# hey-yahei/Quantization.MXNet

Measured on AMD Instinct MI355X. Metric: images/sec int8-sim MobileNet1.0 (per-layer W8A8, online input quant), higher is better.
Workload: dtype f32

## Files before the change

### include/fakequant.h

```cpp
#ifndef FAKEQUANT_H_
#define FAKEQUANT_H_

#include <stddef.h>
#include <stdint.h>

#ifdef __cplusplus
extern "C" {
#endif

#define FQ_OK 0
#define FQ_ERR_INVALID 1
#define FQ_ERR_HIP 2

typedef void* fqStream_t;

#define FQ_ACT_SIGNED 1u
#define FQ_ACT_LO_NEG_MAX 2u
#define FQ_ACT_NO_ABS 4u
#define FQ_ACT_NO_EPS 8u

#define FQ_CODES_INT8 0
#define FQ_CODES_UINT8 1
#define FQ_CODES_RANGE 2
#define FQ_CODES_SCALE 3
// ... 47 lines not shown
int fq_fake_quant_online_prestat(const float* x, float* y, int64_t n, int64_t inner, const float* stat, int width,
                                 unsigned flags, float* out_current_max, int32_t* codes, fqStream_t stream);

#define FQ_ACT_NONE 0
#define FQ_ACT_RELU 1
#define FQ_ACT_RELU6 2
#define FQ_STAT_PREZEROED 0x100
int fq_bn_act_stat(const float* x, float* y, int64_t n, int64_t c, int64_t hw, const float* scale,
                   const float* shift, int act, float* stat_out, fqStream_t stream);
int fq_bn_act_maxpool_stat(const float* x, float* y, int64_t n, int64_t c, int64_t h, int64_t w, const float* scale,
                           const float* shift, int act, float* stat_out, fqStream_t stream);

int fq_add_act_stat(const float* a, const float* b, float* y, int64_t n, int64_t inner, int act, float* stat_out,
                    fqStream_t stream);

int fq_bn_act_stat_hist(const float* x, float* y, int64_t n, int64_t c, int64_t hw, const float* scale,
                        const float* shift, int act, float* stat_out, const float* hist_max, int bins, uint64_t* hist,
                        uint32_t* neg_count, fqStream_t stream);
int fq_add_act_stat_hist(const float* a, const float* b, float* y, int64_t n, int64_t inner, int act, float* stat_out,
                         const float* hist_max, int bins, uint64_t* hist, uint32_t* neg_count, fqStream_t stream);

int fq_bn_add_act_stat(const float* x, const float* residual, float* y, int64_t n, int64_t c, int64_t hw, const float* scale,
                       const float* shift, int act, float* stat_out, fqStream_t stream);
int fq_bn_add_act_stat_hist(const float* x, const float* residual, float* y, int64_t n, int64_t c, int64_t hw,
                            const float* scale, const float* shift, int act, float* stat_out, const float* hist_max, int bins,
                            uint64_t* hist, uint32_t* neg_count, fqStream_t stream);

int fq_global_avg_pool_stat(const float* x, float* y, int64_t n, int64_t c, int64_t hw, int flags, float* stat_out,
                            fqStream_t stream);

int fq_gemm_i8_codes(const int8_t* xcodes, const int8_t* wcodes, const int32_t* wsum, int32_t* out, int64_t n,
                     int64_t l, int64_t k_pad, int64_t cout, int zoff, fqStream_t stream);

int fq_eval_counters(const float* logits, const int64_t* labels, int64_t n, int64_t classes, float* counters,
                     fqStream_t stream);

int fq_stem_conv3x3s2(const float* x, const float* w_tap_major, const float* bias, float* y, int64_t n, int64_t cin,
                      int64_t cout, int64_t h, int64_t w, const float* bn_scale, const float* bn_shift, int act,
                      float* stat_out, fqStream_t stream);
int fq_stem_conv3x3s2_c16(const float* x, const float* w_tap_major, const float* bias, void* y16, int64_t n, int64_t cin,
                          int64_t cout, int64_t h, int64_t w, const float* bn_scale, const float* bn_shift, int act,
                          float* stat_out, const float* out_thr, int out_width, unsigned out_flags, fqStream_t stream);
int fq_stem_conv7x7s2(const float* x, const float* w_tap_major, const float* bias, float* y, int64_t n, int64_t cin,
                      int64_t cout, int64_t h, int64_t w, const float* bn_scale, const float* bn_shift, int act,
                      float* stat_out, fqStream_t stream);
int fq_stem_conv7x7s2_pool_supported(int64_t h, int64_t w);
int fq_stem_conv7x7s2_pool(const float* x, const float* w_tap_major, const float* bias, float* y, int64_t n, int64_t cin,
                           int64_t cout, int64_t h, int64_t w, const float* bn_scale, const float* bn_shift, int act,
                           float* stat_out, fqStream_t stream);

int fq_dwconv3x3(const float* x, const float* w, const float* bias, float* y, int64_t n, int64_t c, int64_t h,
                 int64_t wdt, int stride, const float* in_stat, const float* in_thr, int in_width, unsigned in_flags,
                 float* out_current_max, const float* bn_scale, const float* bn_shift, int act, float* stat_out,
                 fqStream_t stream);

int fq_weight_codes(const float* w, int64_t rows, int64_t row_len, int rows_per_scale, int width, int64_t row_pad,
                    int64_t rows_pad, int8_t* codes, float* scales, int32_t* rowsum, void* ws, fqStream_t stream);
#define FQ_PW_FORM(f) ((f) << 12)
size_t fq_pwconv_workspace_bytes(int64_t n, int64_t cin_pad, int64_t hw);
int fq_pwconv_i8(const float* x, const int8_t* wcodes, const float* wscale, const int32_t* wsum, const float* bias,
                 float* y, int64_t n, int64_t cin, int64_t cin_pad, int64_t cout, int64_t hw, const float* in_stat,
                 const float* in_thr, int in_width, unsigned in_flags, float* out_current_max,
                 const float* bn_scale, const float* bn_shift, int act, float* stat_out, void* ws,
                 fqStream_t stream);

size_t fq_dense_i8_eval_workspace_bytes(int64_t n, int64_t cout);
int fq_dense_i8_eval(const float* x, const int8_t* wcodes, const float* wscale, const int32_t* wsum, const float* bias,
                     float* y, int64_t n, int64_t cin, int64_t cin_pad, int64_t cout, const float* in_stat,
                     const float* in_thr, int in_width, unsigned in_flags, float* out_current_max,
                     const int64_t* labels, float* counters, void* eval_ws, void* ws, fqStream_t stream);

int fq_pwconv_i8_strided(const float* x, const int8_t* wcodes, const float* wscale, const int32_t* wsum,
                         const float* bias, float* y, int64_t n, int64_t cin, int64_t cin_pad, int64_t cout, int64_t h,
                         int64_t w, int stride, const float* in_stat, const float* in_thr, int in_width,
                         unsigned in_flags, float* out_current_max, const float* bn_scale, const float* bn_shift,
                         int act, float* stat_out, const float* residual, void* ws, fqStream_t stream);

int fq_pwconv_i8_sub2_supported(int64_t cin, int64_t cout);
int fq_pwconv_i8_sub2(const float* x, const int8_t* wcodes, const float* wscale, const int32_t* wsum, const float* bias,
                      float* y, int64_t n, int64_t cin, int64_t cin_pad, int64_t cout, int64_t h, int64_t w,
                      const float* in_stat, const float* in_thr, int in_width, unsigned in_flags, float* out_current_max,
                      const float* bn_scale, const float* bn_shift, int act, float* stat_out, const float* residual, void* ws,
                      fqStream_t stream);

int fq_pwconv_i8_shortcut_supported(int64_t cin, int64_t cin2, int64_t cout);
int fq_pwconv_i8_shortcut(const float* x, const int8_t* wcodes, const float* wscale, const int32_t* wsum, const float* bias,
                          float* y, int64_t n, int64_t cin, int64_t cin_pad, int64_t cout, int64_t hw, const float* in_stat,
                          const float* in_thr, int in_width, unsigned in_flags, float* out_current_max, const float* bn_scale,
                          const float* bn_shift, int act, float* stat_out, const float* x2, const int8_t* wcodes2,
                          const float* wscale2, const int32_t* wsum2, int64_t cin2, int64_t cin2_pad, const float* in_stat2,
                          const float* in_thr2, int in_width2, unsigned in_flags2, float* out_current_max2,
                          const float* bn_scale2, const float* bn_shift2, fqStream_t stream);

int fq_pwconv_i8_shortcut_c16(const void* x, const int8_t* wcodes, const float* wscale, const int32_t* wsum, const float* bias,
                              float* y, void* y16, int64_t n, int64_t cin, int64_t cin_pad, int64_t cout, int64_t hw,
                              const float* in_stat, const float* in_thr, int in_width, unsigned in_flags, float* out_current_max,
                              const float* bn_scale, const float* bn_shift, int act, float* stat_out, const void* x2, int x2_is_c16,
                              const int8_t* wcodes2, const float* wscale2, const int32_t* wsum2, int64_t cin2, int64_t cin2_pad,
                              const float* in_stat2, const float* in_thr2, int in_width2, unsigned in_flags2,
                              float* out_current_max2, const float* bn_scale2, const float* bn_shift2, const float* out_thr,
                              int out_width, unsigned out_flags, fqStream_t stream);

int fq_pwconv_i8_gap_supported(int64_t n, int64_t cin, int64_t cout, int64_t hw, int has_residual);
int fq_pwconv_i8_gap(const float* x, const int8_t* wcodes, const float* wscale, const int32_t* wsum, const float* bias,
                     float* y, int64_t n, int64_t cin, int64_t cin_pad, int64_t cout, int64_t hw, const float* in_stat,
                     const float* in_thr, int in_width, unsigned in_flags, float* out_current_max, const float* bn_scale,
                     const float* bn_shift, int act, float* stat_out, const float* residual, void* ws, fqStream_t stream);

int fq_pwconv_i8_stat_supported(int64_t n, int64_t cin, int64_t cout, int64_t hw);
int fq_pwconv_i8_stat(const float* x, const int8_t* wcodes, const float* wscale, const int32_t* wsum, const float* bias,
                      int64_t n, int64_t cin, int64_t cin_pad, int64_t cout_pad, int64_t cout, int64_t hw,
                      const float* in_stat, const float* in_thr, int in_width, unsigned in_flags, float* out_current_max,
                      const float* bn_scale, const float* bn_shift, int act, float* stat_out, void* x_codes_out,
                      fqStream_t stream);
int fq_pwdw_fused_supported(int64_t n, int64_t cin, int64_t cout, int64_t h, int64_t w, int stride);
int fq_debug_fast_quotient(const float* c, int64_t n, const float* d, float* out, int* took_fast_path, fqStream_t stream);
int fq_pwdw_fused(const float* x, const int8_t* wcodes, const float* wscale, const int32_t* wsum, const float* pw_bias,
                  int64_t n, int64_t cin, int64_t cin_pad, int64_t cout_pad, int64_t cout, int64_t h, int64_t w,
                  const float* in_stat, const float* in_thr, int in_width, unsigned in_flags, const float* pw_bn_scale,
                  const float* pw_bn_shift, int pw_act, const float* mid_stat, const float* mid_thr, int mid_width,
                  unsigned mid_flags, float* mid_current_max, const float* dw_w, const float* dw_bias, int dw_stride,
                  const float* dw_bn_scale, const float* dw_bn_shift, int dw_act, float* y, float* stat_out,
                  const void* x_codes, fqStream_t stream);

int fq_pwconv_i8_c16(const void* x, int x_is_c16, const int8_t* wcodes, const float* wscale, const int32_t* wsum,
                     const float* bias, void* y, int64_t n, int64_t cin, int64_t cin_pad, int64_t cout, int64_t h, int64_t w,
                     int stride, const float* in_stat, const float* in_thr, int in_width, unsigned in_flags,
                     float* out_current_max, const float* bn_scale, const float* bn_shift, int act, float* stat_out,
                     const float* residual, const float* out_thr, int out_width, unsigned out_flags, void* ws,
                     fqStream_t stream);

int fq_pwconv_i8_c16_dual(const void* x, const int8_t* wcodes, const float* wscale, const int32_t* wsum, const float* bias,
                          float* y, void* y16, int64_t n, int64_t cin, int64_t cin_pad, int64_t cout, int64_t h, int64_t w,
                          const float* in_stat, const float* in_thr, int in_width, unsigned in_flags, float* out_current_max,
                          const float* bn_scale, const float* bn_shift, int act, float* stat_out, const float* residual,
                          const float* out_thr, int out_width, unsigned out_flags, void* ws, fqStream_t stream);
int fq_pwconv_i8_c16_dual_sub2(const void* x, const int8_t* wcodes, const float* wscale, const int32_t* wsum, const float* bias,
                               float* y, void* y16, int64_t n, int64_t cin, int64_t cin_pad, int64_t cout, int64_t h, int64_t w,
                               const float* in_stat, const float* in_thr, int in_width, unsigned in_flags,
                               float* out_current_max, const float* bn_scale, const float* bn_shift, int act, float* stat_out,
                               const float* residual, const float* out_thr, int out_width, unsigned out_flags, void* ws,
                               fqStream_t stream);

int fq_conv3x3_i8(const float* x, const int8_t* wcodes, const float* wscale, const int32_t* wsum, const float* bias,
                  float* y, int64_t n, int64_t cin, int64_t cout, int64_t h, int64_t w, const float* in_stat,
                  const float* in_thr, int in_width, unsigned in_flags, float* out_current_max, const float* bn_scale,
                  const float* bn_shift, int act, float* stat_out, fqStream_t stream);

int fq_conv3x3_i8_c16(const void* x, int x_is_c16, const int8_t* wcodes, const float* wscale, const int32_t* wsum,
                      const float* bias, void* y, int64_t n, int64_t cin, int64_t cout, int64_t h, int64_t w,
                      const float* in_stat, const float* in_thr, int in_width, unsigned in_flags, float* out_current_max,
                      const float* bn_scale, const float* bn_shift, int act, float* stat_out, const float* out_thr,
                      int out_width, unsigned out_flags, fqStream_t stream);

int fq_dwconv3x3_c16(const void* x, const float* w, const float* bias, void* y, int64_t n, int64_t c, int64_t h, int64_t wdt,
                     int stride, const float* in_stat, const float* in_thr, int in_width, unsigned in_flags,
                     float* out_current_max, const float* bn_scale, const float* bn_shift, int act, float* stat_out,
                     const float* out_thr, int out_width, unsigned out_flags, fqStream_t stream);

int fq_weight_slices(const float* w, int64_t rows, int64_t row_len, int64_t row_pad, int64_t rows_pad, int8_t* codes,
                     float* pscale, int32_t* rowsum, void* ws, fqStream_t stream);
int fq_conv3x3_i8_sliced(const float* x, const int8_t* wslices, const float* pscale, const int32_t* wsum, const float* bias,
                         float* y, int64_t n, int64_t cin, int64_t cout, int64_t h, int64_t w, const float* in_stat,
                         const float* in_thr, int in_width, unsigned in_flags, float* out_current_max,
                         const float* bn_scale, const float* bn_shift, int act, float* stat_out, fqStream_t stream);

int fq_ste_forward(const float* x, float* y, int64_t rows, int64_t row_len, const float* scales, int has_clip,
// ... 54 lines not shown
```

### quantization/mxnet_amd/_lib.py

```python
import ctypes
import os

__all__ = ["LIB", "check_call", "load", "library_path", "FakeQuantError", "EXPORTS"]

_HERE = os.path.dirname(os.path.abspath(__file__))
_LIB_PATH = os.environ.get("FQ_LIB_PATH") or os.path.join(_HERE, "csrc", "libfakequant.so")

c_f32p = ctypes.POINTER(ctypes.c_float)
c_i32p = ctypes.POINTER(ctypes.c_int32)
c_u32p = ctypes.POINTER(ctypes.c_uint32)
c_u64p = ctypes.POINTER(ctypes.c_uint64)
_vp, _i64, _int, _uint, _f32 = ctypes.c_void_p, ctypes.c_int64, ctypes.c_int, ctypes.c_uint, ctypes.c_float

EXPORTS = {
    "fq_last_error": (ctypes.c_char_p, []),
    "fq_version": (_int, []),
    "fq_build_id": (ctypes.c_char_p, []),
    "fq_device_info": (_int, [ctypes.c_char_p, _int, ctypes.POINTER(_int), ctypes.POINTER(_int)]),
    "fq_profile_enable": (_int, [_int]),
    "fq_profile_reset": (_int, []),
    "fq_profile_read": (_int, [_int, ctypes.POINTER(ctypes.c_double), ctypes.POINTER(_i64),
                               ctypes.POINTER(ctypes.c_double)]),
    "fq_profile_read_moved": (_int, [_int, ctypes.POINTER(ctypes.c_double)]),
    "fq_profile_calibrate": (_int, [_vp, _int, ctypes.POINTER(ctypes.c_double), ctypes.POINTER(ctypes.c_double), _vp]),
    "fq_profile_launch_overhead": (_int, [_vp, _int, ctypes.c_double, ctypes.POINTER(ctypes.c_double),
                                          ctypes.POINTER(ctypes.c_double), _vp]),
    "fq_act_workspace_bytes": (ctypes.c_size_t, [_i64]),
    "fq_absmax_per_sample": (_int, [_vp, _i64, _i64, _uint, _vp, _vp]),
    "fq_batch_mean": (_int, [_vp, _i64, _vp, _vp]),
    "fq_batch_mean_gathered": (_int, [_vp, _int, _i64, _vp, _vp]),
    "fq_stat_rows_sum": (_int, [_vp, _i64, _i64, _i64, _vp, _vp]),
    "fq_mean_from_sums": (_int, [_vp, _i64, _vp, _vp]),
    "fq_batch_mean_rows": (_int, [_vp, _i64, _i64, _i64, _vp, _vp]),
    "fq_fake_quant_online": (_int, [_vp, _vp, _i64, _i64, _int, _uint, _vp, _vp, _vp, _vp]),
    "fq_fake_quant_online_prestat": (_int, [_vp, _vp, _i64, _i64, _vp, _int, _uint, _vp, _vp, _vp]),
    "fq_bn_act_stat": (_int, [_vp, _vp, _i64, _i64, _i64, _vp, _vp, _int, _vp, _vp]),
    "fq_bn_act_maxpool_stat": (_int, [_vp, _vp, _i64, _i64, _i64, _i64, _vp, _vp, _int, _vp, _vp]),
    "fq_add_act_stat": (_int, [_vp, _vp, _vp, _i64, _i64, _int, _vp, _vp]),
    "fq_bn_act_stat_hist": (_int, [_vp, _vp, _i64, _i64, _i64, _vp, _vp, _int, _vp, _vp, _int, _vp, _vp, _vp]),
    "fq_add_act_stat_hist": (_int, [_vp, _vp, _vp, _i64, _i64, _int, _vp, _vp, _int, _vp, _vp, _vp]),
    "fq_bn_add_act_stat": (_int, [_vp, _vp, _vp, _i64, _i64, _i64, _vp, _vp, _int, _vp, _vp]),
    "fq_bn_add_act_stat_hist": (_int, [_vp, _vp, _vp, _i64, _i64, _i64, _vp, _vp, _int, _vp, _vp, _int, _vp, _vp, _vp]),
    "fq_global_avg_pool_stat": (_int, [_vp, _vp, _i64, _i64, _i64, _int, _vp, _vp]),
    "fq_gemm_i8_codes": (_int, [_vp, _vp, _vp, _vp, _i64, _i64, _i64, _i64, _int, _vp]),
    "fq_eval_counters": (_int, [_vp, _vp, _i64, _i64, _vp, _vp]),
    "fq_stem_conv3x3s2": (_int, [_vp, _vp, _vp, _vp, _i64, _i64, _i64, _i64, _i64, _vp, _vp, _int, _vp, _vp]),
    "fq_stem_conv7x7s2": (_int, [_vp, _vp, _vp, _vp, _i64, _i64, _i64, _i64, _i64, _vp, _vp, _int, _vp, _vp]),
    "fq_stem_conv7x7s2_pool": (_int, [_vp, _vp, _vp, _vp, _i64, _i64, _i64, _i64, _i64, _vp, _vp, _int, _vp, _vp]),
    "fq_stem_conv7x7s2_pool_supported": (_int, [_i64, _i64]),
    "fq_stem_conv3x3s2_c16": (_int, [_vp, _vp, _vp, _vp, _i64, _i64, _i64, _i64, _i64, _vp, _vp, _int, _vp, _vp, _int, _uint, _vp]),
    "fq_dwconv3x3": (_int, [_vp, _vp, _vp, _vp, _i64, _i64, _i64, _i64, _int, _vp, _vp, _int, _uint, _vp, _vp, _vp, _int,
                            _vp, _vp]),
    "fq_dwconv3x3_c16": (_int, [_vp, _vp, _vp, _vp, _i64, _i64, _i64, _i64, _int, _vp, _vp, _int, _uint, _vp, _vp, _vp, _int,
                                _vp, _vp, _int, _uint, _vp]),
    "fq_weight_codes": (_int, [_vp, _i64, _i64, _int, _int, _i64, _i64, _vp, _vp, _vp, _vp, _vp]),
    "fq_pwconv_workspace_bytes": (ctypes.c_size_t, [_i64, _i64, _i64]),
    "fq_pwconv_i8": (_int, [_vp, _vp, _vp, _vp, _vp, _vp, _i64, _i64, _i64, _i64, _i64, _vp, _vp, _int, _uint, _vp, _vp,
                            _vp, _int, _vp, _vp, _vp]),
    "fq_pwconv_i8_stat_supported": (_int, [_i64, _i64, _i64, _i64]),
    "fq_pwconv_i8_stat": (_int, [_vp, _vp, _vp, _vp, _vp, _i64, _i64, _i64, _i64, _i64, _i64, _vp, _vp, _int, _uint, _vp, _vp,
                                 _vp, _int, _vp, _vp, _vp]),
    "fq_pwdw_fused_supported": (_int, [_i64, _i64, _i64, _i64, _i64, _int]),
    "fq_pwdw_fused": (_int, [_vp, _vp, _vp, _vp, _vp, _i64, _i64, _i64, _i64, _i64, _i64, _i64, _vp, _vp, _int, _uint, _vp,
                             _vp, _int, _vp, _vp, _int, _uint, _vp, _vp, _vp, _int, _vp, _vp, _int, _vp, _vp, _vp, _vp]),
    "fq_debug_fast_quotient": (_int, [_vp, _i64, _vp, _vp, _vp, _vp]),
    "fq_dense_i8_eval_workspace_bytes": (ctypes.c_size_t, [_i64, _i64]),
    "fq_dense_i8_eval": (_int, [_vp, _vp, _vp, _vp, _vp, _vp, _i64, _i64, _i64, _i64, _vp, _vp, _int, _uint, _vp, _vp, _vp,
                                _vp, _vp, _vp]),
    "fq_pwconv_i8_strided": (_int, [_vp, _vp, _vp, _vp, _vp, _vp, _i64, _i64, _i64, _i64, _i64, _i64, _int, _vp, _vp, _int,
                                    _uint, _vp, _vp, _vp, _int, _vp, _vp, _vp, _vp]),
    "fq_pwconv_i8_shortcut_supported": (_int, [_i64, _i64, _i64]),
    "fq_pwconv_i8_shortcut": (_int, [_vp, _vp, _vp, _vp, _vp, _vp, _i64, _i64, _i64, _i64, _i64, _vp, _vp, _int, _uint, _vp, _vp,
                                     _vp, _int, _vp, _vp, _vp, _vp, _vp, _i64, _i64, _vp, _vp, _int, _uint, _vp, _vp, _vp, _vp]),
    "fq_pwconv_i8_shortcut_c16": (_int, [_vp, _vp, _vp, _vp, _vp, _vp, _vp, _i64, _i64, _i64, _i64, _i64, _vp, _vp, _int, _uint, _vp,
                                         _vp, _vp, _int, _vp, _vp, _int, _vp, _vp, _vp, _i64, _i64, _vp, _vp, _int, _uint, _vp, _vp,
                                         _vp, _vp, _int, _uint, _vp]),
    "fq_pwconv_i8_gap_supported": (_int, [_i64, _i64, _i64, _i64, _int]),
    "fq_pwconv_i8_gap": (_int, [_vp, _vp, _vp, _vp, _vp, _vp, _i64, _i64, _i64, _i64, _i64, _vp, _vp, _int, _uint, _vp, _vp, _vp,
                                _int, _vp, _vp, _vp, _vp]),
    "fq_pwconv_i8_sub2_supported": (_int, [_i64, _i64]),
    "fq_pwconv_i8_sub2": (_int, [_vp, _vp, _vp, _vp, _vp, _vp, _i64, _i64, _i64, _i64, _i64, _i64, _vp, _vp, _int,
                                 _uint, _vp, _vp, _vp, _int, _vp, _vp, _vp, _vp]),
    "fq_pwconv_i8_c16": (_int, [_vp, _int, _vp, _vp, _vp, _vp, _vp, _i64, _i64, _i64, _i64, _i64, _i64, _int, _vp, _vp, _int,
                                _uint, _vp, _vp, _vp, _int, _vp, _vp, _vp, _int, _uint, _vp, _vp]),
    "fq_pwconv_i8_c16_dual": (_int, [_vp, _vp, _vp, _vp, _vp, _vp, _vp, _i64, _i64, _i64, _i64, _i64, _i64, _vp, _vp, _int,
                                     _uint, _vp, _vp, _vp, _int, _vp, _vp, _vp, _int, _uint, _vp, _vp]),
    "fq_pwconv_i8_c16_dual_sub2": (_int, [_vp, _vp, _vp, _vp, _vp, _vp, _vp, _i64, _i64, _i64, _i64, _i64, _i64, _vp, _vp, _int,
                                          _uint, _vp, _vp, _vp, _int, _vp, _vp, _vp, _int, _uint, _vp, _vp]),
    "fq_conv3x3_i8": (_int, [_vp, _vp, _vp, _vp, _vp, _vp, _i64, _i64, _i64, _i64, _i64, _vp, _vp, _int, _uint, _vp, _vp,
                             _vp, _int, _vp, _vp]),
    "fq_conv3x3_i8_c16": (_int, [_vp, _int, _vp, _vp, _vp, _vp, _vp, _i64, _i64, _i64, _i64, _i64, _vp, _vp, _int, _uint, _vp,
                                 _vp, _vp, _int, _vp, _vp, _int, _uint, _vp]),
    "fq_conv3x3_i8_sliced": (_int, [_vp, _vp, _vp, _vp, _vp, _vp, _i64, _i64, _i64, _i64, _i64, _vp, _vp, _int, _uint, _vp,
                                    _vp, _vp, _int, _vp, _vp]),
    "fq_weight_slices": (_int, [_vp, _i64, _i64, _i64, _i64, _vp, _vp, _vp, _vp, _vp]),
    "fq_fake_quant_offline": (_int, [_vp, _vp, _i64, _i64, _vp, _int, _uint, _vp, _vp, _vp, _vp]),
    "fq_ste_forward": (_int, [_vp, _vp, _i64, _i64, _vp, _int, _f32, _f32, _f32, _vp]),
    "fq_weight_workspace_bytes": (ctypes.c_size_t, [_i64]),
    "fq_weight_fake_quant": (_int, [_vp, _vp, _i64, _i64, _int, _vp, _vp, _vp]),
    "fq_wino_weight_fake_quant": (_int, [_vp, _vp, _i64, _i64, _int, c_f32p, c_f32p, c_f32p, _int, _vp, _vp, _vp]),
    "fq_comm_unique_id": (_int, [_vp]),
    "fq_comm_init": (_int, [_int, _int, _vp]),
    "fq_comm_world": (_int, []),
    "fq_allreduce_f32": (_int, [_vp, _i64, _int, _vp]),
    "fq_allreduce_f64": (_int, [_vp, _i64, _int, _vp]),
    "fq_allreduce_i64": (_int, [_vp, _i64, _int, _vp]),
    "fq_comm_destroy": (_int, []),
    "fq_ema_update": (_int, [_vp, _vp, _i64, ctypes.c_double, _vp]),
    "fq_global_max": (_int, [_vp, _i64, _vp, _vp]),
    "fq_histogram_accumulate": (_int, [_vp, _i64, _vp, _int, _vp, _vp, _vp]),
    "fq_hist_to_float": (_int, [_vp, _vp, _i64, _vp]),
    "fq_kl_workspace_bytes": (ctypes.c_size_t, [_i64, _int]),
    "fq_kl_search": (_int, [_vp, _i64, _int, _int, _int, _vp, _vp, _vp]),
    "fq_quantize_codes": (_int, [_vp, _vp, _i64, _int, _vp, _vp, _vp]),
# ... 56 lines not shown
```

### quantization/mxnet_amd/csrc/fq_common.h

```cpp
#ifndef FQ_COMMON_H_
#define FQ_COMMON_H_

#include <hip/hip_runtime.h>
#include <type_traits>

#include <algorithm>
#include <cmath>
#include <cstdarg>
#include <cstdint>
#include <cstdio>
#include <cstdlib>
#include <cstring>
#include <mutex>
#include <vector>

#include "fakequant.h"

namespace fqi {

int fail(int code, const char* fmt, ...);
int num_cu();
int max_lds_bytes();
int env_int(const char* name, int dflt);
int stream_policy(int kernel_id, int64_t numel);
// ... 492 lines not shown
    f.sh = k - 32;
  }
  return f;
}

template <bool NT>
__device__ __forceinline__ f4 ld4(const f4* p) {
  if (NT) return __builtin_nontemporal_load(p);
  return *p;
}
template <bool NT>
__device__ __forceinline__ void st4(f4* p, f4 v) {
  if (NT)
    __builtin_nontemporal_store(v, p);
  else
    *p = v;
}
__device__ __forceinline__ f4 fq_code4(f4 v, const QParams& q) {
  f4 k;
  k.x = fq_code(v.x, q);
  k.y = fq_code(v.y, q);
  k.z = fq_code(v.z, q);
  k.w = fq_code(v.w, q);
  return k;
}

template <bool USE_ABS>
__device__ __forceinline__ float stat4(f4 v) {
  return fmaxf(fmaxf(stat_of<USE_ABS>(v.x), stat_of<USE_ABS>(v.y)), fmaxf(stat_of<USE_ABS>(v.z), stat_of<USE_ABS>(v.w)));
}

struct ChunkRange {
  int64_t begin, end;
};
__device__ __forceinline__ ChunkRange block_range(int64_t total_chunks) {
  const int64_t per = (total_chunks + gridDim.x - 1) / gridDim.x;
  ChunkRange r;
  r.begin = (int64_t)blockIdx.x * per;
  r.end = r.begin + per < total_chunks ? r.begin + per : total_chunks;
  return r;
}

__device__ __forceinline__ float act_rt(float v, int act) {
  if (act == FQ_ACT_RELU) v = fmaxf(v, 0.0f);
  if (act == FQ_ACT_RELU6) v = fminf(fmaxf(v, 0.0f), 6.0f);
  return v;
}

__device__ __forceinline__ float lane_prev(float v) {
  return __builtin_bit_cast(float, __builtin_amdgcn_update_dpp(0, __builtin_bit_cast(int, v), 0x138, 0xF, 0xF, false));
}
__device__ __forceinline__ float lane_next(float v) {
  return __builtin_bit_cast(float, __builtin_amdgcn_update_dpp(0, __builtin_bit_cast(int, v), 0x130, 0xF, 0xF, false));
}

constexpr int kEpiRuntime = 0, kEpiBnRelu = 1, kEpiBnRelu6 = 2;
constexpr int kActBiasMul = 0x10;
template <int EPI, bool ACT = true>
__device__ __forceinline__ float dw_finish(float acc, bool has_bias, float bch, bool has_bn, float bsc, float bsh, int act) {
  if (EPI == kEpiRuntime) {
    if (has_bias) acc = (act & kActBiasMul) ? acc * bch : acc + bch;
    if (has_bn) {
      acc = acc * bsc;
      acc = acc + bsh;
    }
    return act_rt(acc, act & 15);
  }
  acc = acc * bsc;
  acc = acc + bsh;
  if (!ACT) return acc;
  acc = fmaxf(acc, 0.0f);
  return EPI == kEpiBnRelu6 ? fminf(acc, 6.0f) : acc;
}

#ifdef FQ_PW_TRACE
__device__ unsigned long long* g_pw_trace = nullptr;
__device__ int g_pw_dbg = 0;
#define PW_STAMP(i)                                                                       \
  do {                                                                                    \
    if (threadIdx.x == 0 && g_pw_trace != nullptr) g_pw_trace[(size_t)blockIdx.x * 8 + (i)] = wall_clock64(); \
  } while (0)
#else
#define PW_STAMP(i) do { } while (0)
#endif

template <bool WANT_MIN, bool USE_ABS>
__global__ __launch_bounds__(kBlock) void minmax_kernel(const float* __restrict__ x, int64_t numel, int vec_ok,
                                                        float* __restrict__ out_min, float* __restrict__ out_max) {
  __shared__ float red[4];
  float mx = USE_ABS ? 0.0f : -INFINITY, mn = INFINITY;
  auto take = [&](float v) {
    mx = fmaxf(mx, stat_of<USE_ABS>(v));
    if (WANT_MIN) mn = fminf(mn, v);
  };
  const int64_t chunks = (numel + kChunk - 1) / kChunk;
  const ChunkRange rg = block_range(chunks);
  for (int64_t c = rg.begin; c < rg.end; ++c) {
    const int64_t base = c * (int64_t)kChunk;
    const int64_t rem = numel - base;
    if (vec_ok && rem >= kChunk) {
      const f4* p = reinterpret_cast<const f4*>(x + base);
      f4 v[kUnroll];
#pragma unroll
      for (int u = 0; u < kUnroll; ++u) v[u] = p[threadIdx.x + u * kBlock];
#pragma unroll
      for (int u = 0; u < kUnroll; ++u) {
// ... 22 lines not shown
```

### quantization/mxnet_amd/csrc/fq_dwconv.hip

```cpp
#include "fq_common.h"

namespace {

typedef float f2 __attribute__((ext_vector_type(2)));
__device__ __forceinline__ f2 splat2(float v) { return (f2){v, v}; }

__device__ __forceinline__ float dw_taps(float w00, float w01, float w02, float w10, float w11, float w12, float w20,
                                         float w21, float w22, float a0, float a1, float a2, float b0, float b1, float b2,
                                         float c0, float c1, float c2) {
  float acc = 0.0f;
  acc = fmaf(w00, a0, acc);
  acc = fmaf(w01, a1, acc);
  acc = fmaf(w02, a2, acc);
  acc = fmaf(w10, b0, acc);
  acc = fmaf(w11, b1, acc);
  acc = fmaf(w12, b2, acc);
  acc = fmaf(w20, c0, acc);
  acc = fmaf(w21, c1, acc);
  acc = fmaf(w22, c2, acc);
  return acc;
}
__device__ __forceinline__ f2 dw_taps2(float w00, float w01, float w02, float w10, float w11, float w12, float w20, float w21,
                                       float w22, f2 a0, f2 a1, f2 a2, f2 b0, f2 b1, f2 b2, f2 c0, f2 c1, f2 c2) {
  f2 acc = {0.f, 0.f};
  acc = __builtin_elementwise_fma(splat2(w00), a0, acc);
  acc = __builtin_elementwise_fma(splat2(w01), a1, acc);
  acc = __builtin_elementwise_fma(splat2(w02), a2, acc);
  acc = __builtin_elementwise_fma(splat2(w10), b0, acc);
  acc = __builtin_elementwise_fma(splat2(w11), b1, acc);
  acc = __builtin_elementwise_fma(splat2(w12), b2, acc);
  acc = __builtin_elementwise_fma(splat2(w20), c0, acc);
  acc = __builtin_elementwise_fma(splat2(w21), c1, acc);
  acc = __builtin_elementwise_fma(splat2(w22), c2, acc);
  return acc;
}

template <bool ONLINE>
__device__ __forceinline__ QParams dw_qparams(const float* in_stat, int n, const float* in_thr,
                                              float levels, int lo_neg_max, float eps, float* cur_max_out) {
  const float max_ = input_threshold(in_stat, n, ONLINE ? nullptr : in_thr, cur_max_out, blockIdx.x == 0);
  return make_qparams_rt(max_, levels, lo_neg_max, eps, in_thr);
}
template <bool ONLINE>
__device__ __forceinline__ QParams dw_qparams_finish(const ThresholdReq& treq, const float* in_stat, int n,
                                                     const float* in_thr, float levels, int lo_neg_max, float eps,
                                                     float* cur_max_out) {
  const float max_ = threshold_finish(treq, in_stat, n, ONLINE ? nullptr : in_thr, cur_max_out, blockIdx.x == 0);
  return make_qparams_rt(max_, levels, lo_neg_max, eps, in_thr);
}

struct DwBlkRange {
  unsigned begin, end;
  unsigned n_samples;
  unsigned s_base;
};
__device__ __forceinline__ DwBlkRange dw_block_range(unsigned nblk, unsigned tsegs, unsigned segs_per_block, unsigned nsegx,
                                                     unsigned C) {
  DwBlkRange r;
  r.begin = (unsigned)((uint64_t)nblk * blockIdx.x / gridDim.x);
  r.end = (unsigned)((uint64_t)nblk * (blockIdx.x + 1) / gridDim.x);
  r.n_samples = tsegs / nsegx / C;
  const unsigned seg0 = r.begin * segs_per_block;
  r.s_base = (seg0 < tsegs ? seg0 : tsegs - 1) / nsegx / C;
  return r;
}

constexpr int kStatSlots = 16;
template <class SampleT>
__device__ __forceinline__ void dw_stat_update(unsigned* k_stat, unsigned s_base, SampleT sample, bool is_out, float m,
                                               int lane, float* stat_out) {
  const unsigned s0 = (unsigned)__builtin_amdgcn_readfirstlane((int)sample);
  const bool wave_uniform = __all(!is_out || (unsigned)sample == s0);
  if (wave_uniform) {
    const float wm = wave_max_nonneg(is_out ? m : 0.0f);
// ... 705 lines not shown
          for (int r = 0; r < H; ++r) {
            float c0 = 0.f, c1 = 0.f, c2 = 0.f;
            if (r + 1 < H) {
              c1 = lp[(r + 1) * W];
              c0 = left_of(c1, first);
              c2 = right_of(c1, last);
            }
            lp[r * W] = window(a0, a1, a2, b0, b1, b2, c0, c1, c2);
            a0 = b0; a1 = b1; a2 = b2;
            b0 = c0; b1 = c1; b2 = c2;
          }
        } else {
          const float* lp = my_tile + j * IN + pos * 2;
          float* op = my_out + j * OUT + pos;
          float a0 = 0.f, a1 = 0.f, a2 = 0.f;
#pragma unroll
          for (int r = 0; r < HO; ++r) {
            const f2 vb = *reinterpret_cast<const f2*>(lp + (2 * r) * W);
            const float b0 = left_of(vb.y, first);
            float c0 = 0.f, c1 = 0.f, c2 = 0.f;
            if (2 * r + 1 < H) {
              const f2 vc = *reinterpret_cast<const f2*>(lp + (2 * r + 1) * W);
              c1 = vc.x;
              c2 = vc.y;
              c0 = left_of(vc.y, first);
            }
            op[r * WO] = window(a0, a1, a2, b0, vb.x, vb.y, c0, c1, c2);
            a0 = c0; a1 = c1; a2 = c2;
          }
        }
      }
    }
    FQ_DWF_PHASE();
    {
      f4 ov[NLO];
#pragma unroll
      for (int i = 0; i < NLO; ++i) ov[i] = DOWN ? otile[wave][lane + 64 * i] : tile[wave][lane + 64 * i];
#pragma unroll
      for (int i = 0; i < NLO; ++i)
        buf_st_v4f_unguarded(ry, (lane + 64u * i) < lim_out ? lane * 16u : kOob, base * (OUT * 4u) + 1024u * i, ov[i]);
      hold_store_data(ov);
    }
    if (has_stat) {
      const unsigned sample = fast_div(base + (is_out ? j : 0u), g.by_c);
      dw_stat_update(k_stat, s_base, sample, is_out, m, (int)lane, stat_out);
    }
    __builtin_amdgcn_wave_barrier();
  }
  PW_STAMP(3);
  if (has_stat) dw_stat_flush(k_stat, s_base, n_samples, stat_out);
  PW_STAMP(5);
}

template <int S, bool QUANT, bool ONLINE, bool NT, int EPI>
__global__ __launch_bounds__(kBlock) void dwconv3x3_cols4_kernel(
    const float* __restrict__ x, const float* __restrict__ wgt, const float* __restrict__ bias,
    float* __restrict__ y, DwColGeom g, int64_t total_segs, const float* __restrict__ in_stat, int n,
    const float* __restrict__ in_thr, float levels, int lo_neg_max, float eps, float* __restrict__ cur_max_out,
    const float* __restrict__ bn_scale, const float* __restrict__ bn_shift, int act, float* __restrict__ stat_out) {
  constexpr int D = (S == 1) ? 4 : 2;
  __shared__ unsigned k_stat[kStatSlots];
  if (threadIdx.x < kStatSlots) k_stat[threadIdx.x] = 0u;
  QParams q = {};
  if (QUANT) q = dw_qparams<ONLINE>(in_stat, n, in_thr, levels, lo_neg_max, eps, cur_max_out);
  const int lane = threadIdx.x & 63, wave = threadIdx.x >> 6;
  const int seg_in_wave = lane / g.SEG;
  const int pos = lane - seg_in_wave * g.SEG;
  const bool lane_used = seg_in_wave < g.segs;
  const int64_t segs_per_block = (int64_t)g.segs * (kBlock / 64);
  const int64_t nblk = (total_segs + segs_per_block - 1) / segs_per_block;
  const bool has_bn = bn_scale != nullptr, has_stat = stat_out != nullptr;
  const int plane_in = g.H * g.W, plane_out = g.Ho * g.Wo;
  const int last_row = g.H - 1;
  const unsigned tsegs = (unsigned)total_segs, nsegx = (unsigned)g.nsegx, C_u = (unsigned)g.C;
  const DwBlkRange rg = dw_block_range((unsigned)nblk, tsegs, (unsigned)segs_per_block, nsegx, C_u);
  __syncthreads();
  for (unsigned blk = rg.begin; blk < rg.end; ++blk) {
    const unsigned seg = blk * (unsigned)segs_per_block + (unsigned)wave * (unsigned)g.segs + (unsigned)seg_in_wave;
    const bool seg_ok = lane_used && seg < tsegs;
    const unsigned plane = seg_ok ? seg / nsegx : 0u;
    const int sx = seg_ok ? (int)(seg - plane * nsegx) : 0;
    const unsigned sample_u = plane / C_u;
    const int ch = (int)(plane - sample_u * C_u);
    const int sample = (int)sample_u;
    const int ic0 = (sx * g.sw + pos - 1) * 4;
    const bool ld_ok = seg_ok && ic0 >= 0 && ic0 < g.W;
    const int oc = S == 1 ? ic0 : ic0 / 2;
    const bool is_out = seg_ok && pos >= 1 && pos <= g.sw && oc < g.Wo;
    const f4* xs = reinterpret_cast<const f4*>(ld_ok ? x + plane * (int64_t)plane_in + ic0 : x);
    float* yp = y + plane * (int64_t)plane_out + oc;
    const int rowq = g.W / 4;
    const float* wk = wgt + ch * 9;
    const float w00 = wk[0], w01 = wk[1], w02 = wk[2], w10 = wk[3], w11 = wk[4], w12 = wk[5], w20 = wk[6],
                w21 = wk[7], w22 = wk[8];
    const float bch = bias != nullptr ? bias[ch] : 0.0f;
    const float bsc = has_bn ? bn_scale[ch] : 1.0f, bsh = has_bn ? bn_shift[ch] : 0.0f;
    float m = 0.0f;
    auto ldrow = [&](int row) -> f4 {
      const int rc = row < last_row ? row : last_row;
      return keep4(ld4<NT>(xs + (int64_t)rc * rowq), ld_ok && row <= last_row);
    };
    auto quant4 = [&](f4 v) -> f4 { return QUANT ? fq_code4(v, q) * q.scale : v; };
    auto finish = [&](float acc) -> float { return dw_finish<EPI>(acc, bias != nullptr, bch, has_bn, bsc, bsh, act); };

    if (S == 1) {
      float a[6] = {0.f, 0.f, 0.f, 0.f, 0.f, 0.f}, b[6];
      f4 raw[D];
#pragma unroll
      for (int k = 0; k < D; ++k) raw[k] = ldrow(1 + k);
      {
        const f4 v = quant4(ldrow(0));
        b[0] = lane_prev(v.w);
        b[1] = v.x; b[2] = v.y; b[3] = v.z; b[4] = v.w;
        b[5] = lane_next(v.x);
      }
      auto emit = [&](int r, f4 craw) {
        const f4 v = quant4(craw);
        float c[6];
        c[0] = lane_prev(v.w);
        c[1] = v.x; c[2] = v.y; c[3] = v.z; c[4] = v.w;
        c[5] = lane_next(v.x);
        float o[4];
#pragma unroll
        for (int k = 0; k < 4; ++k) {
          o[k] = finish(dw_taps(w00, w01, w02, w10, w11, w12, w20, w21, w22, a[k], a[k + 1], a[k + 2], b[k], b[k + 1],
                                b[k + 2], c[k], c[k + 1], c[k + 2]));
        }
        const float mm = fmaxf(fmaxf(fabsf(o[0]), fabsf(o[1])), fmaxf(fabsf(o[2]), fabsf(o[3])));
        m = fmaxf(m, keep(mm, is_out));
        if (is_out) {
          if (g.nts) __builtin_nontemporal_store((f4){o[0], o[1], o[2], o[3]}, reinterpret_cast<f4*>(yp + (int64_t)r * g.Wo));
          else *reinterpret_cast<f4*>(yp + (int64_t)r * g.Wo) = (f4){o[0], o[1], o[2], o[3]};
        }
#pragma unroll
        for (int k = 0; k < 6; ++k) {
          a[k] = b[k];
          b[k] = c[k];
        }
      };
      int r0 = 0;
      for (; r0 + D <= g.Ho; r0 += D) {
        f4 nxt[D];
#pragma unroll
        for (int k = 0; k < D; ++k) nxt[k] = ldrow(r0 + k + 1 + D);
#pragma unroll
        for (int k = 0; k < D; ++k) emit(r0 + k, raw[k]);
#pragma unroll
        for (int k = 0; k < D; ++k) raw[k] = nxt[k];
      }
#pragma unroll
      for (int k = 0; k < D; ++k)
        if (r0 + k < g.Ho) emit(r0 + k, raw[k]);
    } else {
      float a[5] = {0.f, 0.f, 0.f, 0.f, 0.f};
      f4 rb[D], rc[D];
#pragma unroll
      for (int k = 0; k < D; ++k) {
        rb[k] = ldrow(2 * k);
        rc[k] = ldrow(2 * k + 1);
      }
      auto emit2 = [&](int r, f4 braw, f4 craw) {
        const f4 vb = quant4(braw), vc = quant4(craw);
        const float b[5] = {lane_prev(vb.w), vb.x, vb.y, vb.z, vb.w};
        const float c[5] = {lane_prev(vc.w), vc.x, vc.y, vc.z, vc.w};
        float o[2];
#pragma unroll
        for (int k = 0; k < 2; ++k) {
          o[k] = finish(dw_taps(w00, w01, w02, w10, w11, w12, w20, w21, w22, a[2 * k], a[2 * k + 1], a[2 * k + 2], b[2 * k],
                                b[2 * k + 1], b[2 * k + 2], c[2 * k], c[2 * k + 1], c[2 * k + 2]));
        }
        m = fmaxf(m, keep(fmaxf(fabsf(o[0]), fabsf(o[1])), is_out));
        if (is_out) {
          typedef float f2v __attribute__((ext_vector_type(2)));
          if (g.nts) __builtin_nontemporal_store((f2v){o[0], o[1]}, reinterpret_cast<f2v*>(yp + (int64_t)r * g.Wo));
          else *reinterpret_cast<float2*>(yp + (int64_t)r * g.Wo) = make_float2(o[0], o[1]);
        }
#pragma unroll
        for (int k = 0; k < 5; ++k) a[k] = c[k];
      };
      int r0 = 0;
      for (; r0 + D <= g.Ho; r0 += D) {
        f4 nb[D], nc[D];
#pragma unroll
        for (int k = 0; k < D; ++k) {
          nb[k] = ldrow(2 * (r0 + k + D));
          nc[k] = ldrow(2 * (r0 + k + D) + 1);
        }
#pragma unroll
        for (int k = 0; k < D; ++k) emit2(r0 + k, rb[k], rc[k]);
#pragma unroll
        for (int k = 0; k < D; ++k) {
          rb[k] = nb[k];
          rc[k] = nc[k];
        }
      }
#pragma unroll
      for (int k = 0; k < D; ++k)
        if (r0 + k < g.Ho) emit2(r0 + k, rb[k], rc[k]);
    }
    if (has_stat) dw_stat_update(k_stat, rg.s_base, sample, is_out, m, lane, stat_out);
  }
  if (has_stat) dw_stat_flush(k_stat, rg.s_base, rg.n_samples, stat_out);
}

}

constexpr unsigned kFlagRangeRecord = 0x100u;
constexpr unsigned kFlagBiasMultiplies = 0x200u;

namespace {

struct DwCall {
  const float *x, *w, *bias;
  float* y;
  int64_t n, c, h, wdt;
  int stride;
  const float *in_stat, *in_thr;
  float* out_current_max;
  const float *bn_scale, *bn_shift;
  int act;
  float* stat_out;
  hipStream_t st;
  bool quant, online, prezeroed;
  int epi;
  float levels, eps;
  int lo_neg;
  int64_t ho, wo;
};

template <class KernelFor, class... Geom>
int dw_launch(const DwCall& d, int grid, size_t lds, KernelFor kernel_for, Geom... geom) {
  using std::integral_constant;
  if (d.stat_out && !d.prezeroed) FQ_HIP(hipMemsetAsync(d.stat_out, 0, d.n * sizeof(float), d.st));
  ProfScope prof(FQ_KERNEL_DWCONV, 4.0 * ((double)d.n * d.c * d.h * d.wdt + (double)d.n * d.c * d.ho * d.wo), d.st);
  auto launch = [&](auto kernel) {
    hipLaunchKernelGGL(kernel, dim3(grid), dim3(kBlock), lds, d.st, d.x, d.w, d.bias, d.y, geom..., d.in_stat, (int)d.n,
                       d.in_thr, d.levels, d.lo_neg, d.eps, d.out_current_max, d.bn_scale, d.bn_shift, d.act, d.stat_out);
  };
  auto with_epi = [&](auto quant_c, auto online_c) {
    if (d.epi == kEpiBnRelu) launch(kernel_for(quant_c, online_c, integral_constant<int, kEpiBnRelu>{}));
    else if (d.epi == kEpiBnRelu6) launch(kernel_for(quant_c, online_c, integral_constant<int, kEpiBnRelu6>{}));
    else launch(kernel_for(quant_c, online_c, integral_constant<int, kEpiRuntime>{}));
  };
  if (!d.quant) with_epi(std::false_type{}, std::false_type{});
  else if (d.online) with_epi(std::true_type{}, std::true_type{});
  else with_epi(std::true_type{}, std::false_type{});
  FQ_LAUNCH_CHECK();
  return FQ_OK;
}
template <int V>
using dw_int = std::integral_constant<int, V>;

int64_t dw_blocks(int64_t total_segs, int segs) {
  const int64_t per_block = (int64_t)segs * (kBlock / 64);
  return (total_segs + per_block - 1) / per_block;
}
int dw_grid(int64_t nblk, int wg_per_cu) {
  const int64_t cap = (int64_t)num_cu() * wg_per_cu;
  return (int)(nblk < cap ? nblk : cap);
}

DwColGeom dw_col_geom(const DwCall& d, int units, int halo) {
  DwColGeom cg = {};
  cg.C = (int)d.c;
  cg.H = (int)d.h;
  cg.W = (int)d.wdt;
  cg.Ho = (int)d.ho;
  cg.Wo = (int)d.wo;
  const int max_sw = 64 - halo;
  cg.nsegx = (units + max_sw - 1) / max_sw;
  cg.sw = (units + cg.nsegx - 1) / cg.nsegx;
  cg.SEG = cg.sw + halo;
  cg.segs = 64 / cg.SEG;
  return cg;
}

int dw_flat_kind(const DwCall& d) {
  return (d.h == 14 && d.wdt == 14) ? (d.stride == 1 ? 0 : 1)
         : (d.h == 7 && d.wdt == 7 && d.stride == 1) ? 2
         : (d.h == 28 && d.wdt == 28) ? (d.stride == 1 ? 3 : 4) : -1;
}
int dw_flat_planes(int kind) { return kind == 0 ? 9 : kind >= 3 ? 4 : 8; }
bool dw_flat_applies(const DwCall& d, int form) {
  static const int flat_on = env_int("FQ_DW_FLAT", 31) & 31;
  const int kind = dw_flat_kind(d);
  const bool whole = kind == 0 || kind >= 3 || (d.n * d.c) % dw_flat_planes(kind) == 0;
  return kind >= 0 && (form == 5 || (form == 0 && ((flat_on >> kind) & 1))) && whole && aligned16(d.x) && aligned16(d.y) &&
         d.n * d.c * d.h * d.wdt * 4 < (1ll << 31);
}
// ... 1 lines not shown
  const int kind = dw_flat_kind(d);
  DwFlatGeom fg;
  fg.C = (int)d.c;
  fg.planes = (unsigned)(d.n * d.c);
  fg.by_c = fast_div_for((unsigned)d.c);
  const int64_t nblk = dw_blocks(d.n * d.c, dw_flat_planes(kind));
  static const int fl_tune = env_int("FQ_DW_FLAT_WG_PER_CU", 0);
  const int grid = dw_grid(nblk, fl_tune > 0 ? fl_tune : 3);
  fg.per = (unsigned)(nblk / grid);
  fg.rem = (unsigned)(nblk % grid);
  auto go = [&](auto s, auto hw) {
    return dw_launch(d, grid, 0, [](auto q, auto o, auto e) {
      return dwconv3x3_flat_kernel<decltype(s)::value, q(), o(), decltype(hw)::value, decltype(hw)::value, e()>;
    }, fg);
  };
  return kind == 0 ? go(dw_int<1>{}, dw_int<14>{}) : kind == 1 ? go(dw_int<2>{}, dw_int<14>{})
         : kind == 2 ? go(dw_int<1>{}, dw_int<7>{}) : kind == 4 ? go(dw_int<2>{}, dw_int<28>{})
                     : go(dw_int<1>{}, dw_int<28>{});
}

bool dw_planes_two_cols(const DwCall& d) {
  static const int planes_cpl = env_int("FQ_DW_PLANES_CPL", 2);
  const bool al8 = ((((uintptr_t)d.x) | ((uintptr_t)d.y)) & 7) == 0;
  return d.wdt % 2 == 0 && al8 && (d.stride == 2 || planes_cpl == 2);
}
bool dw_planes_applies(const DwCall& d, int form) {
  static const int planes_on = env_int("FQ_DW_PLANES", 1);
  const bool can_planes = (d.h == 14 || d.h == 7) && d.wdt <= 64 && (d.stride == 1 || (dw_planes_two_cols(d) && d.h == 14)) &&
                          d.n * d.c * d.h * d.wdt * 4 < (1ll << 31);
  return (form == 4 || (form == 0 && planes_on)) && can_planes;
}
int dw_run_planes(const DwCall& d) {
  const bool two_cols = dw_planes_two_cols(d);
  DwColGeom cg = dw_col_geom(d, (int)(d.stride == 2 ? d.wo : (two_cols ? d.wdt / 2 : d.wdt)), 0);
  cg.sw = cg.Wo;
  const int64_t total_segs = d.n * d.c;
  static const int pl_wg_per_cu = env_int("FQ_DW_PLANES_WG_PER_CU", 5);
  const int grid = dw_grid(dw_blocks(total_segs, cg.segs), pl_wg_per_cu);
  auto go = [&](auto s, auto h, auto cpl) {
    return dw_launch(d, grid, 0, [](auto q, auto o, auto e) {
      return dwconv3x3_planes_kernel<decltype(s)::value, q(), o(), decltype(h)::value, decltype(cpl)::value, e()>;
    }, cg, total_segs);
  };
  if (d.stride == 2) return go(dw_int<2>{}, dw_int<14>{}, dw_int<2>{});
  if (d.h == 14) return two_cols ? go(dw_int<1>{}, dw_int<14>{}, dw_int<2>{}) : go(dw_int<1>{}, dw_int<14>{}, dw_int<1>{});
  return two_cols ? go(dw_int<1>{}, dw_int<7>{}, dw_int<2>{}) : go(dw_int<1>{}, dw_int<7>{}, dw_int<1>{});
}

int dw_cols_grid(int64_t total_segs, const DwColGeom& cg) {
  static const int dw_wg_per_cu = env_int("FQ_DW_WG_PER_CU", 6);
  return dw_grid(dw_blocks(total_segs, cg.segs), dw_wg_per_cu);
}
bool dw_cols4_applies(const DwCall& d, int form) {
  const bool can4 = (d.wdt % 4 == 0) && aligned16(d.x) && aligned16(d.y) && ((d.h * d.wdt) % 4 == 0) &&
                    (d.stride == 1 || ((d.wdt / 2) % 2 == 0));
  return (form == 3 || form == 0) && can4;
}
int dw_run_cols4(const DwCall& d) {
  DwColGeom cg = dw_col_geom(d, (int)(d.wdt / 4), d.stride == 1 ? 2 : 1);
  const int64_t total_segs = d.n * d.c * cg.nsegx;
  FQ_REQUIRE(total_segs < (1ll << 31) - 1024, "fq_dwconv3x3: tensor too large for 32-bit segment indices");
  const int grid = dw_cols_grid(total_segs, cg);
  static const int dw_nt_mb = env_int("FQ_DW_NT_MB", 200);
  const bool nt = 4.0 * (double)d.n * d.c * d.h * d.wdt > 1e6 * dw_nt_mb;
  static const int dw_nts_mb = env_int("FQ_DW_NTS_MB", 1 << 30);
  cg.nts = 4.0 * (double)d.n * d.c * cg.Ho * cg.Wo >= 1e6 * dw_nts_mb ? 1 : 0;
  auto go = [&](auto s, auto nt_c) {
    return dw_launch(d, grid, 0, [](auto q, auto o, auto e) {
      return dwconv3x3_cols4_kernel<decltype(s)::value, q(), o(), decltype(nt_c)::value, e()>;
    }, cg, total_segs);
  };
  if (d.stride == 1) return nt ? go(dw_int<1>{}, std::true_type{}) : go(dw_int<1>{}, std::false_type{});
  return nt ? go(dw_int<2>{}, std::true_type{}) : go(dw_int<2>{}, std::false_type{});
}
bool dw_cols_applies(const DwCall& d, int form) {
  return form == 2 || ((form == 0 || form == 3) && d.wdt >= 14);
}
int dw_run_cols(const DwCall& d) {
  const DwColGeom cg = dw_col_geom(d, (int)d.wo, d.stride == 1 ? 2 : 1);
  const int64_t total_segs = d.n * d.c * cg.nsegx;
  FQ_REQUIRE(total_segs < (1ll << 31) - 1024, "fq_dwconv3x3: tensor too large for 32-bit segment indices");
  const int grid = dw_cols_grid(total_segs, cg);
  auto go = [&](auto s) {
    return dw_launch(d, grid, 0, [](auto q, auto o, auto e) {
      return dwconv3x3_cols_kernel<decltype(s)::value, q(), o(), e()>;
    }, cg, total_segs);
  };
  return d.stride == 1 ? go(dw_int<1>{}) : go(dw_int<2>{});
}

int dw_run_tiles(const DwCall& d) {
  const int stride = d.stride;
  DwGeom g;
  g.C = (int)d.c;
  g.H = (int)d.h;
  g.W = (int)d.wdt;
  g.Ho = (int)d.ho;
  g.Wo = (int)d.wo;
  g.WS = g.W + 2;
  if ((g.WS & 1) == 0) g.WS += 1;
  const int lds_budget = 8192;
  const int plane_in = g.H * g.W;
  if (plane_in <= 4096 && (g.H + 2) * g.WS <= lds_budget) {
    g.TR = g.Ho;
    g.strips = 1;
    g.IR = g.H + 2;
    g.P = 1;
    for (int p = (int)(d.c < 64 ? d.c : 64); p >= 1; --p)
      if (d.c % p == 0 && p * g.IR * g.WS <= lds_budget) {
        g.P = p;
        break;
      }
  } else {
    g.P = 1;
    int tr = (lds_budget / g.WS - 2) / stride;
    FQ_REQUIRE(tr >= 1, "fq_dwconv3x3: rows of %d floats do not fit the LDS tile", g.W);
    g.strips = (g.Ho + tr - 1) / tr;
    g.TR = (g.Ho + g.strips - 1) / g.strips;
    g.IR = g.TR * stride + 2;
  }
  {
    const int per_seg = g.P * g.Wo;
    int nseg = (2 * kBlock + per_seg - 1) / per_seg;
    if (nseg < 1) nseg = 1;
    if (nseg > g.TR) nseg = g.TR;
    g.RS = (g.TR + nseg - 1) / nseg;
    g.nseg = (g.TR + g.RS - 1) / g.RS;
  }
  const bool base_ok = aligned16(d.x);
  if (g.P > 1 || g.strips == 1)
    g.vec_in = base_ok && (((int64_t)g.P * plane_in) % 4 == 0) && (plane_in % 4 == 0 || g.P % 4 == 0);
  else
    g.vec_in = base_ok && (g.W % 4 == 0) && (plane_in % 4 == 0);
  const int64_t tiles = (d.n * d.c / g.P) * g.strips;
  const size_t lds = (size_t)((g.P * g.IR * g.WS + 3) / 4 * 4 + 16) * sizeof(float);
  auto go = [&](auto s) {
    return dw_launch(d, grid_for(tiles), lds, [](auto q, auto o, auto) {
      return dwconv3x3_kernel<decltype(s)::value, q(), o()>;
    }, g, tiles);
  };
  return stride == 1 ? go(dw_int<1>{}) : go(dw_int<2>{});
}

}

static int dwconv3x3_impl(const float* x, const float* w, const float* bias, float* y, int64_t n, int64_t c, int64_t h,
                          int64_t wdt, int stride, const float* in_stat, const float* in_thr, int in_width, unsigned in_flags,
                          float* out_current_max, const float* bn_scale, const float* bn_shift, int act, float* stat_out,
                          fqStream_t stream) {
  FQ_REQUIRE(x && w && y, "fq_dwconv3x3: null pointer");
  FQ_REQUIRE(n > 0 && c > 0 && h > 0 && wdt > 0 && n * c < (1ll << 31) && h * wdt < (1ll << 28),
             "fq_dwconv3x3: bad shape (n=%lld c=%lld h=%lld w=%lld)", (long long)n, (long long)c, (long long)h,
             (long long)wdt);
  FQ_REQUIRE(stride == 1 || stride == 2, "fq_dwconv3x3: stride must be 1 or 2, got %d", stride);
  FQ_REQUIRE((bn_scale == nullptr) == (bn_shift == nullptr), "fq_dwconv3x3: bn_scale and bn_shift go together");
  const bool prezeroed = (act & FQ_STAT_PREZEROED) != 0;
  act &= ~FQ_STAT_PREZEROED;
  FQ_REQUIRE(act >= FQ_ACT_NONE && act <= FQ_ACT_RELU6, "fq_dwconv3x3: unknown activation %d", act);
  const bool quant = in_stat != nullptr || in_thr != nullptr;
  if (quant) FQ_REQUIRE(in_width >= 2 && in_width <= 16, "fq_dwconv3x3: width %d out of range", in_width);
  if (in_flags & kFlagBiasMultiplies) act |= kActBiasMul;
  static const int epi_on = env_int("FQ_DW_EPI", 1);

  DwCall d = {};
  d.x = x; d.w = w; d.bias = bias; d.y = y;
  d.n = n, d.c = c, d.h = h, d.wdt = wdt, d.stride = stride;
  d.in_stat = in_stat, d.in_thr = in_thr, d.out_current_max = out_current_max;
  d.bn_scale = bn_scale, d.bn_shift = bn_shift, d.act = act, d.stat_out = stat_out;
  d.st = (hipStream_t)stream;
  d.quant = quant, d.online = quant && in_thr == nullptr, d.prezeroed = prezeroed;
  d.epi = (epi_on && bn_scale != nullptr && bias == nullptr)
              ? (act == FQ_ACT_RELU ? kEpiBnRelu : act == FQ_ACT_RELU6 ? kEpiBnRelu6 : kEpiRuntime)
              : kEpiRuntime;
  d.levels = act_levels(in_width, in_flags);
  d.lo_neg = (in_flags & kFlagRangeRecord) ? kRangeMode : ((in_flags & FQ_ACT_LO_NEG_MAX) ? 1 : 0);
  d.eps = (in_flags & FQ_ACT_NO_EPS) ? 0.0f : kEps;
  d.ho = (h - 1) / stride + 1, d.wo = (wdt - 1) / stride + 1;

  static const int form = env_int("FQ_DW_FORM", 0);
  if (dw_flat_applies(d, form)) return dw_run_flat(d);
  if (dw_planes_applies(d, form)) return dw_run_planes(d);
  if (dw_cols4_applies(d, form)) return dw_run_cols4(d);
  if (dw_cols_applies(d, form)) return dw_run_cols(d);
  return dw_run_tiles(d);
}

namespace fqi {
int dw_range_call(const float* x, const float* wcodes_f32, float* y, int64_t n, int64_t c, int64_t h, int64_t wdt, int stride,
                  const float* rec, const float* svec, const float* bn_scale, const float* bn_shift, int act,
                  float* stat_out, hipStream_t st) {
  return dwconv3x3_impl(x, wcodes_f32, svec, y, n, c, h, wdt, stride, nullptr, rec, 8, kFlagRangeRecord | kFlagBiasMultiplies,
                        nullptr, bn_scale, bn_shift, act, stat_out, (fqStream_t)st);
}
}

extern "C" {

int fq_dwconv3x3(const float* x, const float* w, const float* bias, float* y, int64_t n, int64_t c, int64_t h,
                 int64_t wdt, int stride, const float* in_stat, const float* in_thr, int in_width, unsigned in_flags,
                 float* out_current_max, const float* bn_scale, const float* bn_shift, int act, float* stat_out,
                 fqStream_t stream) {
  FQ_REQUIRE(!(in_flags & ~(FQ_ACT_SIGNED | FQ_ACT_LO_NEG_MAX | FQ_ACT_NO_ABS | FQ_ACT_NO_EPS)), "fq_dwconv3x3: unknown flags");
  return dwconv3x3_impl(x, w, bias, y, n, c, h, wdt, stride, in_stat, in_thr, in_width, in_flags, out_current_max, bn_scale,
                        bn_shift, act, stat_out, stream);
}

}
```

### quantization/mxnet_amd/csrc/fq_pw.h

```cpp
#ifndef FQ_PW_H_
#define FQ_PW_H_

#include "fq_common.h"

namespace fqi {

struct PwCall {
  const float* x;
  const int8_t* wcodes;
  const float* wscale;
  const int32_t* wsum;
  const float* bias;
  float* y;
  int64_t n, cin, cin_pad, cout, hw;
  int stride;
  int64_t h_in, w_in, w_out;
  const float* in_stat;
  const float* in_thr;
  float levels;
  int lo_neg, zoff;
  float* out_current_max;
  const float* bn_scale;
  const float* bn_shift;
  int act;
  float* stat_out;
  const float* residual;
  bool prezeroed;
  void* ws;
  hipStream_t st;
  int form;
  bool in_c16 = false;
  const float* out_thr = nullptr;
  float out_levels = 0.0f;
  int out_lo_neg = 0, out_zoff = 0;
  void* y16 = nullptr;
  const float* dual_thr = nullptr;
  bool sub = false;
  bool gap = false;
  const long long* eval_labels = nullptr;
  float* eval_counters = nullptr;
  void* eval_ws = nullptr;
  void* x_codes_out = nullptr;
};

bool pw_stat_shape_ok(int64_t n, int64_t cin, int64_t cout, int64_t hw);
int pw_stat_launch(const PwCall& c);
bool pw_short_shape_ok(int64_t cin, int64_t cin2, int64_t cout);
int pw_short_launch(const PwCall& a, const PwCall& b);
int pw_try_stream(const PwCall& c, bool* taken);
bool pw_stream_shape_ok(const PwCall& c);
bool pw_stream_thin_takes(const PwCall& c);
int pw_try_split(const PwCall& c, bool* taken);
int pw_split16_launch(const PwCall& a, const void* geom, int kt, int cw, int64_t grid, size_t lds, const int8_t* wfrag,
                      bool* launched, int nw = 4);
bool pw_split_sub_shape_ok(int64_t cin_pad, int64_t cout);
int pw_split_sub_launch(const PwCall& a, const void* geom, int kt, int64_t grid, size_t lds, const int8_t* wfrag, bool* launched);
int pw_try_sample(const PwCall& c, bool* taken);
bool pw_sample_gap_shape_ok(int64_t n, int64_t cin, int64_t cout, int64_t hw, bool residual);
int pw_try_rows(const PwCall& c, bool* taken);
size_t pw_rows_eval_ws_bytes(int64_t n, int64_t cout);
int pw_two_kernels(const PwCall& c);

inline int pw_zero_stat(const PwCall& c) {
  if (c.stat_out && !c.prezeroed) {
    hipError_t e = hipMemsetAsync(c.stat_out, 0, c.n * sizeof(float), c.st);
    if (e != hipSuccess) return fail(FQ_ERR_HIP, "hipMemsetAsync(stat_out): %s", hipGetErrorString(e));
  }
  return FQ_OK;
}

}

#endif
```

### quantization/mxnet_amd/csrc/fq_pwconv.hip

```cpp
#include "fq_pw.h"

namespace {

__global__ __launch_bounds__(kBlock) void weight_codes_kernel(const float* __restrict__ w, int rows, int row_len,
                                                              int rows_per_scale, float levels, int row_pad,
                                                              const float* __restrict__ gmax,
                                                              int8_t* __restrict__ codes, float* __restrict__ scales,
                                                              int* __restrict__ rowsum, int8_t* __restrict__ frag) {
  __shared__ int red[4];
  const int r = blockIdx.x;
  int8_t* dst = codes + (int64_t)r * row_pad;
  const int kts = row_pad >> 5;
  auto frag_at = [&](int i) -> int8_t* {
    const int kt = i >> 5, hs = (i >> 4) & 1, b = i & 15;
    return frag + ((((int64_t)(r >> 5) * kts + kt) << 6) + (r & 31) + 32 * hs) * 16 + b;
  };
  if (r >= rows) {
    for (int i = threadIdx.x; i < row_pad; i += kBlock) {
      dst[i] = 0;
      *frag_at(i) = 0;
    }
    return;
  }
  const float s = gmax[r / rows_per_scale] / levels;
// ... 141 lines not shown
    FQ_REQUIRE(c.form == 0 || c.form == 7, "fq_pwconv_i8_gap: only the sample form pools");
    if (int rc = pw_try_sample(c, &taken)) return rc;
    FQ_REQUIRE(taken, "fq_pwconv_i8_gap: shape not taken (see fq_pwconv_i8_gap_supported)");
    return FQ_OK;
  }
  if (sub) {
    FQ_REQUIRE(c.form == 0 || c.form == 6, "fq_pwconv_i8_sub2: only the split form stores a subsampled output");
    if (int rc = pw_try_split(c, &taken)) return rc;
    FQ_REQUIRE(taken, "fq_pwconv_i8_sub2: shape not taken (see fq_pwconv_i8_sub2_supported)");
    return FQ_OK;
  }
  if (hw == 1 && !(in_c16 || out_thr) && !range) {
    if (int rc = pw_try_rows(c, &taken)) return rc;
    if (taken) return FQ_OK;
  }
  FQ_REQUIRE(c.form != 8, "fq_pwconv_i8: the rows form takes planes of one pixel");
  if (!(in_c16 || out_thr)) {
    if (int rc = pw_try_sample(c, &taken)) return rc;
    if (taken) return FQ_OK;
  } else if (out_thr && !in_c16) {
    if (int rc = pw_try_stream(c, &taken)) return rc;
    if (taken) return FQ_OK;
  }
  if (!taken && pw_stream_thin_takes(c)) {
    if (int rc = pw_try_stream(c, &taken)) return rc;
    if (taken) return FQ_OK;
  }
  FQ_REQUIRE(c.form != 7, "fq_pwconv_i8: the sample form takes stride 1, no residual, Cout a multiple of 256 and planes that "
             "cut into blocks of 96..128 pixels (Cin 128 ... 1024; a residual operand with 512 channels per workgroup) or whole planes "
             "of 45..64 pixels (Cin 512 / 1024, no residual)");
  if (int rc = pw_try_split(c, &taken)) return rc;
  if (taken) return FQ_OK;
  if (int rc = pw_try_stream(c, &taken)) return rc;
  if (taken) return FQ_OK;
  FQ_REQUIRE(residual == nullptr, "fq_pwconv_i8_strided: a residual operand needs a shape the split or the streaming "
             "form takes");
  if (range) {
    *range_taken = false;
    prof.cancel();
    return FQ_OK;
  }
  return pw_two_kernels(c);
}

int fq_pwconv_i8(const float* x, const int8_t* wcodes, const float* wscale, const int32_t* wsum, const float* bias,
                 float* y, int64_t n, int64_t cin, int64_t cin_pad, int64_t cout, int64_t hw, const float* in_stat,
                 const float* in_thr, int in_width, unsigned in_flags, float* out_current_max,
                 const float* bn_scale, const float* bn_shift, int act, float* stat_out, void* ws,
                 fqStream_t stream) {
  return pwconv_dispatch(x, wcodes, wscale, wsum, bias, y, n, cin, cin_pad, cout, hw, 1, 0, 0, 0, in_stat, in_thr,
                         in_width, in_flags, out_current_max, bn_scale, bn_shift, act, stat_out, nullptr, ws, stream);
}

int fq_pwconv_i8_stat_supported(int64_t n, int64_t cin, int64_t cout, int64_t hw) {
  return pw_stat_shape_ok(n, cin, cout, hw) ? 1 : 0;
}

int fq_pwconv_i8_stat(const float* x, const int8_t* wcodes, const float* wscale, const int32_t* wsum, const float* bias,
                      int64_t n, int64_t cin, int64_t cin_pad, int64_t cout_pad, int64_t cout, int64_t hw,
                      const float* in_stat, const float* in_thr, int in_width, unsigned in_flags, float* out_current_max,
                      const float* bn_scale, const float* bn_shift, int act, float* stat_out, void* x_codes_out,
                      fqStream_t stream) {
  FQ_REQUIRE(x && wcodes && wscale && wsum && stat_out, "fq_pwconv_i8_stat: null pointer");
  FQ_REQUIRE(pw_stat_shape_ok(n, cin, cout, hw), "fq_pwconv_i8_stat: shape not taken (n=%lld cin=%lld cout=%lld hw=%lld): see "
             "fq_pwconv_i8_stat_supported", (long long)n, (long long)cin, (long long)cout, (long long)hw);
  FQ_REQUIRE(cin_pad >= cin && cin_pad % 64 == 0 && cin_pad <= 8192 && cout_pad >= cout && cout_pad % 32 == 0,
             "fq_pwconv_i8_stat: cin_pad / cout_pad must be those of fq_weight_codes");
  FQ_REQUIRE(in_stat != nullptr || in_thr != nullptr, "fq_pwconv_i8_stat: give in_stat (online), in_thr (offline) or both");
  FQ_REQUIRE(in_width >= 2 && in_width <= 8, "fq_pwconv_i8_stat: input width %d does not fit int8 codes", in_width);
  FQ_REQUIRE(!(in_flags & (FQ_ACT_NO_ABS | FQ_ACT_NO_EPS)), "fq_pwconv_i8_stat: unsupported activation flags");
  FQ_REQUIRE((bn_scale == nullptr) == (bn_shift == nullptr), "fq_pwconv_i8_stat: bn_scale and bn_shift go together");
  PwCall c;
  c.prezeroed = (act & FQ_STAT_PREZEROED) != 0;
  act &= ~FQ_STAT_PREZEROED;
  FQ_REQUIRE(act >= FQ_ACT_NONE && act <= FQ_ACT_RELU6, "fq_pwconv_i8_stat: unknown activation %d", act);
  FQ_REQUIRE(aligned16(wcodes) && aligned16(x) && aligned16(x_codes_out),
             "fq_pwconv_i8_stat: x, wcodes and x_codes_out must be 16-byte aligned");
  c.x = x; c.wcodes = wcodes + cout_pad * cin_pad; c.wscale = wscale; c.wsum = wsum; c.bias = bias; c.y = nullptr;
  c.n = n; c.cin = cin; c.cin_pad = cin_pad; c.cout = cout; c.hw = hw; c.stride = 1; c.h_in = c.w_in = c.w_out = 0;
  c.in_stat = in_stat; c.in_thr = in_thr;
  c.levels = act_levels(in_width, in_flags);
  c.lo_neg = (in_flags & FQ_ACT_LO_NEG_MAX) ? 1 : 0;
  c.zoff = (in_flags & FQ_ACT_SIGNED) ? 0 : 128;
  c.out_current_max = out_current_max; c.bn_scale = bn_scale; c.bn_shift = bn_shift; c.act = act;
  c.stat_out = stat_out; c.residual = nullptr; c.ws = nullptr; c.st = (hipStream_t)stream; c.form = 0;
  c.x_codes_out = x_codes_out;
  const double in_elems = (double)n * cin * hw, out_elems = (double)n * cout * hw;
  const double code_bytes = x_codes_out ? 32.0 * (double)((cin + 31) / 32) * n * hw : 0.0;
  ProfScope prof(FQ_KERNEL_PWCONV, 4.0 * (in_elems + out_elems), c.st, 4.0 * in_elems + code_bytes);
  return pw_stat_launch(c);
}

int fq_pwconv_i8_strided(const float* x, const int8_t* wcodes, const float* wscale, const int32_t* wsum,
                         const float* bias, float* y, int64_t n, int64_t cin, int64_t cin_pad, int64_t cout, int64_t h,
                         int64_t w, int stride, const float* in_stat, const float* in_thr, int in_width,
                         unsigned in_flags, float* out_current_max, const float* bn_scale, const float* bn_shift,
                         int act, float* stat_out, const float* residual, void* ws, fqStream_t stream) {
  FQ_REQUIRE(h > 0 && w > 0 && (stride == 1 || stride == 2), "fq_pwconv_i8_strided: bad plane %lld x %lld or stride %d",
             (long long)h, (long long)w, stride);
  const int64_t ho = (h - 1) / stride + 1, wo = (w - 1) / stride + 1;
  return pwconv_dispatch(x, wcodes, wscale, wsum, bias, y, n, cin, cin_pad, cout, ho * wo, stride, h, w, wo, in_stat,
                         in_thr, in_width, in_flags, out_current_max, bn_scale, bn_shift, act, stat_out, residual, ws,
                         stream);
}

int fq_pwconv_i8_sub2_supported(int64_t cin, int64_t cout) {
  return pw_split_sub_shape_ok((cin + 63) / 64 * 64, cout) ? 1 : 0;
}

int fq_pwconv_i8_sub2(const float* x, const int8_t* wcodes, const float* wscale, const int32_t* wsum, const float* bias,
                      float* y, int64_t n, int64_t cin, int64_t cin_pad, int64_t cout, int64_t h, int64_t w,
                      const float* in_stat, const float* in_thr, int in_width, unsigned in_flags, float* out_current_max,
                      const float* bn_scale, const float* bn_shift, int act, float* stat_out, const float* residual, void* ws,
                      fqStream_t stream) {
  FQ_REQUIRE(h > 0 && w > 0, "fq_pwconv_i8_sub2: bad plane %lld x %lld", (long long)h, (long long)w);
  FQ_REQUIRE(pw_split_sub_shape_ok(cin_pad, cout), "fq_pwconv_i8_sub2: built for 64 / 128 / 256 / 512 (padded) input channels "
             "and more than 128 output channels (got cin_pad=%lld cout=%lld)", (long long)cin_pad, (long long)cout);
  return pwconv_dispatch(x, wcodes, wscale, wsum, bias, y, n, cin, cin_pad, cout, h * w, 1, h, w, w, in_stat, in_thr,
                         in_width, in_flags, out_current_max, bn_scale, bn_shift, act, stat_out, residual, ws, stream, false,
                         nullptr, 8, 0, nullptr, nullptr, nullptr, nullptr, nullptr, true);
}

int fq_pwconv_i8_gap_supported(int64_t n, int64_t cin, int64_t cout, int64_t hw, int has_residual) {
  return pw_sample_gap_shape_ok(n, cin, cout, hw, has_residual != 0) ? 1 : 0;
}

int fq_pwconv_i8_gap(const float* x, const int8_t* wcodes, const float* wscale, const int32_t* wsum, const float* bias,
                     float* y, int64_t n, int64_t cin, int64_t cin_pad, int64_t cout, int64_t hw, const float* in_stat,
                     const float* in_thr, int in_width, unsigned in_flags, float* out_current_max, const float* bn_scale,
                     const float* bn_shift, int act, float* stat_out, const float* residual, void* ws, fqStream_t stream) {
  FQ_REQUIRE(cin == cin_pad && pw_sample_gap_shape_ok(n, cin, cout, hw, residual != nullptr),
             "fq_pwconv_i8_gap: shape not taken (n=%lld cin=%lld cout=%lld hw=%lld%s): see fq_pwconv_i8_gap_supported",
             (long long)n, (long long)cin, (long long)cout, (long long)hw, residual ? ", residual" : "");
  return pwconv_dispatch(x, wcodes, wscale, wsum, bias, y, n, cin, cin_pad, cout, hw, 1, 0, 0, 0, in_stat, in_thr, in_width,
                         in_flags, out_current_max, bn_scale, bn_shift, act, stat_out, residual, ws, stream, false, nullptr, 8, 0,
                         nullptr, nullptr, nullptr, nullptr, nullptr, false, true);
}

int fq_pwconv_i8_shortcut_supported(int64_t cin, int64_t cin2, int64_t cout) {
  return pw_short_shape_ok(cin, cin2, cout) ? 1 : 0;
}

// ... 194 lines not shown
```

### quantization/mxnet_amd/csrc/fq_pwdw.hip

```cpp
#include "fq_pw.h"

#include <climits>

namespace {

struct PwDwGeom {
  int Cin, KTS, Cout, H, W, Ho, Wo;
  int strips, ctg, bands, RB;
  int zoff, pitch;
  int vw;
  FastDiv qv;
};

constexpr int kRowSlack = 8;

template <int KT, int S> struct PwDwRing {
  static constexpr int NB = S == 1 ? 2 : (KT <= 2 ? 3 : 4);
  static constexpr int NR = 2;
};

template <int KT, int CW, int S, int LZ, int FAST, int CODES>
__global__ __launch_bounds__(512) void pwdw_kernel(
    const float* __restrict__ x, const int8_t* __restrict__ xc, const int8_t* __restrict__ wfrag, const float* __restrict__ wscale,
    const int* __restrict__ wsum, const float* __restrict__ bias1, PwDwGeom g, const float* __restrict__ in_stat, int n,
// ... 324 lines not shown
            const float* src = rbuf + c * g.pitch + 2 * qd;
            const float2 v = make_float2(src[0], src[1]);
            m = fmaxf(m, fmaxf(fabsf(v.x), fabsf(v.y)));
            *reinterpret_cast<float2*>(yr + (int64_t)c * g.Ho * g.Wo + 2 * qd) = v;
          } else {
            const float v = rbuf[c * g.pitch + qd];
            m = fmaxf(m, fabsf(v));
            yr[(int64_t)c * g.Ho * g.Wo + qd] = v;
          }
        }
      }
    };
    constexpr int U = CODES ? NR : ((KT % NB == 0) ? 1 : ((2 * KT) % NB == 0 ? 2 : NB));
    static_assert(U <= 3, "the row loop below unrolls at most three phases");
    using std::integral_constant;
    for (int t = t_first; t <= t_last; t += U) {
      row(t, integral_constant<int, 0>{});
      if (U > 1 && t + 1 <= t_last) row(t + 1, integral_constant<int, 1 % U>{});
      if (U > 2 && t + 2 <= t_last) row(t + 2, integral_constant<int, 2 % U>{});
    }
  };
  using std::false_type;
  using std::true_type;
  if (fq_nonneg(q1) && fq_nonneg(q2) && fq1.ok && fq2.ok) body(true_type{});
  else body(false_type{});

  if (stat_out != nullptr) {
    m = wave_max_nonneg(m);
    __syncthreads();
    if (lane == 0) red[wave] = m;
    __syncthreads();
    if (threadIdx.x == 0) {
      float mm = 0.0f;
      for (int w = 0; w < (int)(blockDim.x >> 6); ++w) mm = fmaxf(mm, red[w]);
      if (__float_as_uint(mm) != 0u) FQ_STAT_FLUSH_MAX(reinterpret_cast<unsigned*>(stat_out) + smp, __float_as_uint(mm));
    }
  }
}

__device__ __forceinline__ void buf_st_v4i(fq_rsrc r, unsigned voff, v4i v) {
  typedef unsigned v4u __attribute__((ext_vector_type(4)));
  __builtin_amdgcn_raw_buffer_store_b128(__builtin_bit_cast(v4u, v), r, (int)voff, 0, 0);
  asm volatile("s_nop 1" : : "v"(v));
}

struct PwStatGeom {
  int Cin, KTS, Cout, CT, HW;
  int64_t cols, tiles;
  int zoff;
  int table;
  FastDiv hw;
};

template <int KT>
__global__ __launch_bounds__(kBlock, 3) void pw_stat_kernel(
    const float* __restrict__ x, const int8_t* __restrict__ wfrag, const float* __restrict__ wscale,
    const int* __restrict__ wsum, const float* __restrict__ bias, PwStatGeom g, const float* __restrict__ in_stat, int n,
    const float* __restrict__ in_thr, float levels, int lo_neg, float eps, float* __restrict__ cur_max_out,
    const float* __restrict__ bn_scale, const float* __restrict__ bn_shift, int act, float* __restrict__ stat_out,
    int8_t* __restrict__ x_codes_out) {
  extern __shared__ __attribute__((aligned(16))) unsigned char pst_smem[];
  v4i* ldsW = reinterpret_cast<v4i*>(pst_smem);
  int* c_zs = reinterpret_cast<int*>(pst_smem + (size_t)g.CT * KT * 1024);
  float* c_k = reinterpret_cast<float*>(c_zs + g.CT * 32);
  int* accs = reinterpret_cast<int*>(c_k + 4 * g.CT * 32);
  const int lane = threadIdx.x & 63, wave = threadIdx.x >> 6;
  const int h = lane >> 5, i32 = lane & 31;
  const unsigned HW = (unsigned)g.HW, cols = (unsigned)g.cols;
  const int64_t nwaves = (int64_t)gridDim.x * 4, wid = (int64_t)blockIdx.x * 4 + wave;
  const int64_t t_begin = g.tiles * wid / nwaves, t_end = g.tiles * (wid + 1) / nwaves;
  const int pl = 16 * ((i32 >> 2) & 1) + 4 * (i32 >> 3) + (i32 & 3);
  int* my = accs + (size_t)wave * g.CT * 128;
  constexpr int kSlots = 8;
  __shared__ unsigned k_stat[kSlots];
  if (threadIdx.x < kSlots) k_stat[threadIdx.x] = 0u;
  unsigned s_base;
  {
    const int64_t t0 = g.tiles * ((int64_t)blockIdx.x * 4) / nwaves;
    const unsigned j0 = (unsigned)(t0 < g.tiles ? t0 : g.tiles - 1) * 32u;
    s_base = fast_div(j0 < cols ? j0 : cols - 1, g.hw);
  }

  struct Pix { unsigned smp, p; };
  auto pix_of = [&](int64_t t) __attribute__((always_inline)) {
    unsigned j = (unsigned)t * 32u + (unsigned)pl;
    j = j < cols ? j : cols - 1;
    Pix r;
    r.smp = fast_div(j, g.hw);
    r.p = j - r.smp * HW;
    return r;
  };
  constexpr int NB = 3;
  const fq_rsrc rs = make_rsrc(x, (int64_t)(cols / HW) * g.Cin * HW * 4);
  auto issue = [&](int64_t t, int kt, float (&v)[16]) __attribute__((always_inline)) {
    if (t >= t_end) return;
    const Pix px = pix_of(t);
    const bool ok = kt * 32 + 16 * h < g.Cin;
    const unsigned vo = ok ? (unsigned)(((px.smp * (unsigned)g.Cin + 16u * h) * HW + px.p) * 4u) : 0x80000000u;
    const unsigned so = (unsigned)kt * 32u * HW * 4u;
#pragma unroll
    for (int i = 0; i < 16; ++i) v[i] = buf_ld_f32(rs, vo, so + (unsigned)i * HW * 4u);
  };
  float raw[NB][16];
#pragma unroll
  for (int b2 = 0; b2 < NB; ++b2)
#pragma unroll
    for (int i = 0; i < 16; ++i) raw[b2][i] = 0.0f;
#pragma unroll
  for (int qq = 0; qq < NB - 1; ++qq) issue(t_begin + qq / KT, qq % KT, raw[qq]);
  FQ_PIN();
  const float max_ = input_threshold(in_stat, n, in_thr, cur_max_out, blockIdx.x == 0);
  const QParams q = make_qparams(max_, levels, lo_neg != 0, eps);
  const int ubias = 128 - g.zoff;
  const unsigned nn_xor = fq_nonneg_xor(ubias);
  const bool wr_codes = x_codes_out != nullptr;
  const fq_rsrc rcodes = make_rsrc(x_codes_out, wr_codes ? (int64_t)(cols / HW) * 2 * KT * HW * 16 : 0);
  for (int idx = threadIdx.x; idx < g.CT * KT * 64; idx += kBlock) {
    const int f = idx >> 6, ct = f / KT, kt = f - ct * KT;
    ldsW[idx] = *reinterpret_cast<const v4i*>(wfrag + (((int64_t)ct * g.KTS + kt) << 10) + ((idx & 63) << 4));
  }
  const int nchs = g.CT * 32;
  for (int i = threadIdx.x; i < nchs; i += kBlock) {
    const bool okc = i < g.Cout;
    c_zs[i] = okc ? g.zoff * wsum[i] : 0;
    c_k[i] = okc ? wscale[i] : 0.0f;
    c_k[nchs + i] = (okc && bias != nullptr) ? bias[i] : 0.0f;
    c_k[2 * nchs + i] = (okc && bn_scale != nullptr) ? bn_scale[i] : 1.0f;
    c_k[3 * nchs + i] = (okc && bn_scale != nullptr) ? bn_shift[i] : 0.0f;
  }
  auto reset = [&]() __attribute__((always_inline)) {
    for (int ct = 0; ct < g.CT; ++ct) {
      my[ct * 128 + lane] = INT_MIN;
      my[ct * 128 + 64 + lane] = INT_MAX;
    }
  };
  reset();
  __syncthreads();
  const bool has_bn = bn_scale != nullptr;
  auto flush = [&](unsigned smp) __attribute__((always_inline)) {
    float m = 0.0f;
    for (int ct = 0; ct < g.CT; ++ct) {
      const int c = ct * 32 + i32;
      int hi = my[ct * 128 + lane], lo = my[ct * 128 + 64 + lane];
      const int ohi = __shfl_xor(hi, 32, 64), olo = __shfl_xor(lo, 32, 64);
      hi = hi > ohi ? hi : ohi;
      lo = lo < olo ? lo : olo;
      if (c < g.Cout && hi >= lo) {
        hi += c_zs[c];
        lo += c_zs[c];
        const float sxw = q.scale * c_k[c];
        const float bch = c_k[nchs + c];
        const float bsc = c_k[2 * nchs + c], bsh = c_k[3 * nchs + c];
        auto f = [&](int a) {
          float v = (float)a * sxw;
          if (bias != nullptr) v = v + bch;
          if (has_bn) {
            v = v * bsc;
            v = v + bsh;
          }
          return fabsf(act_rt(v, act));
        };
        m = fmaxf(m, fmaxf(f(hi), f(lo)));
      }
    }
    m = wave_max_nonneg(m);
    if (lane == 0 && __float_as_uint(m) != 0u) {
      const unsigned slot = smp - s_base;
      if (g.table && slot < (unsigned)kSlots) atomicMax(&k_stat[slot], __float_as_uint(m));
      else FQ_STAT_FLUSH_MAX(reinterpret_cast<unsigned*>(stat_out) + smp, __float_as_uint(m));
    }
    reset();
  };
  v4i afrag[KT];
  const FastQuot fqx = make_fast_quot(q.denom);
  auto quant = [&](int kt, const float (&v)[16], auto nn_c) __attribute__((always_inline)) {
    v4i f;
#pragma unroll
    for (int d = 0; d < 4; ++d) {
      if constexpr (decltype(nn_c)::value) {
        unsigned u = 0u;
#pragma unroll
        for (int b = 0; b < 4; ++b) {
          int r;
          const float Q = fast_quot(fq_clip(v[4 * d + b], q), fqx);
          asm("v_cvt_rpi_i32_f32 %0, %1" : "=v"(r) : "v"(Q));
          u |= (unsigned)r << (8 * b);
        }
        f[d] = (int)(u ^ nn_xor);
      } else {
        f[d] = fq_pack4<false>(v[4 * d + 0], v[4 * d + 1], v[4 * d + 2], v[4 * d + 3], q, ubias, nn_xor);
      }
    }
    asm volatile("" : "+v"(f[0]), "+v"(f[1]), "+v"(f[2]), "+v"(f[3]));
    afrag[kt] = f;
  };
  auto reduce_tile = [&](int plo, int phi) __attribute__((always_inline)) {
    const bool whole = plo <= 0 && phi >= 32;
#pragma unroll 1
    for (int ct = 0; ct < g.CT; ++ct) {
      v16i acc = {0, 0, 0, 0, 0, 0, 0, 0, 0, 0, 0, 0, 0, 0, 0, 0};
#pragma unroll
      for (int kt = 0; kt < KT; ++kt)
        acc = __builtin_amdgcn_mfma_i32_32x32x32_i8(afrag[kt], ldsW[((ct * KT + kt) << 6) + lane], acc, 0, 0, 0);
      int hi = INT_MIN, lo = INT_MAX;
      if (whole) {
#pragma unroll
        for (int k = 0; k < 16; k += 2) {
          hi = max(max(acc[k], acc[k + 1]), hi);
          lo = min(min(acc[k], acc[k + 1]), lo);
        }
      } else {
#pragma unroll
        for (int k = 0; k < 16; ++k) {
          const int p = 16 * h + k;
          const bool in = p >= plo && p < phi;
          hi = in && acc[k] > hi ? acc[k] : hi;
          lo = in && acc[k] < lo ? acc[k] : lo;
        }
      }
      atomicMax(&my[ct * 128 + lane], hi);
      atomicMin(&my[ct * 128 + 64 + lane], lo);
    }
  };
  unsigned cur = fast_div((unsigned)((t_begin < g.tiles ? t_begin : g.tiles - 1) * 32), g.hw);
  auto run_tile = [&](int64_t t, auto ph_c, auto nn_c) __attribute__((always_inline)) {
    constexpr int PH = decltype(ph_c)::value;
    const Pix px = pix_of(t);
    const unsigned cvo = ((px.smp * (unsigned)(2 * KT) + (unsigned)h) * HW + px.p) * 16u;
#pragma unroll
    for (int kt = 0; kt < KT; ++kt) {
      const int qn = kt + NB - 1;
      issue(t + qn / KT, qn % KT, raw[(PH * KT + kt + NB - 1) % NB]);
      FQ_PIN();
      quant(kt, raw[(PH * KT + kt) % NB], nn_c);
      if (wr_codes) buf_st_v4i(rcodes, cvo + (unsigned)(2 * kt) * HW * 16u, afrag[kt]);
      FQ_PIN();
    }
    const unsigned j0 = (unsigned)t * 32u, j1 = j0 + 31u < cols ? j0 + 31u : cols - 1;
    const unsigned s0 = fast_div(j0, g.hw), s1 = fast_div(j1, g.hw);
    if (s0 != cur) {
      flush(cur);
      cur = s0;
    }
    if (s0 == s1) {
      reduce_tile(0, 32);
    } else {
      const int pb = (int)(s1 * HW - j0);
      reduce_tile(0, pb);
      flush(cur);
      cur = s1;
      reduce_tile(pb, 32);
    }
    FQ_PIN();
  };
  auto run_all = [&](auto nn_c) __attribute__((always_inline)) {
    constexpr int U = (KT % NB == 0) ? 1 : NB;
    using std::integral_constant;
    for (int64_t t = t_begin; t < t_end; t += U) {
      run_tile(t, integral_constant<int, 0>{}, nn_c);
      if (U > 1 && t + 1 < t_end) run_tile(t + 1, integral_constant<int, 1 % U>{}, nn_c);
      if (U > 2 && t + 2 < t_end) run_tile(t + 2, integral_constant<int, 2 % U>{}, nn_c);
      if (U > 3 && t + 3 < t_end) run_tile(t + 3, integral_constant<int, 3 % U>{}, nn_c);
    }
  };
  if (fq_nonneg(q) && fqx.ok) run_all(std::true_type{});
  else run_all(std::false_type{});
  if (t_begin < t_end) flush(cur);
  __syncthreads();
  if (threadIdx.x < kSlots && k_stat[threadIdx.x] != 0u && s_base + threadIdx.x < cols / HW)
    FQ_STAT_FLUSH_MAX(reinterpret_cast<unsigned*>(stat_out) + s_base + threadIdx.x, k_stat[threadIdx.x]);
}

__global__ void fast_quotient_kernel(const float* __restrict__ c, int64_t n, const float* __restrict__ d, float* __restrict__ out,
                                     int* __restrict__ ok_out) {
  const FastQuot f = make_fast_quot(d[0]);
  const double rden = 1.0 / (double)d[0];
  const int64_t i = (int64_t)blockIdx.x * blockDim.x + threadIdx.x;
  if (i == 0) ok_out[0] = f.ok ? 1 : 0;
  if (i < n) out[i] = f.ok ? fast_quot(c[i], f) : ieee_div_by(c[i], rden);
}

struct PwDwPlan {
  int kt, cw, lz, strips, ctg, bands, rb, pitch, threads;
  size_t lds;
  bool ok;
};

PwDwPlan pwdw_plan(int64_t n, int64_t cin, int64_t cout, int64_t h, int64_t w, int stride) {
  PwDwPlan p;
  memset(&p, 0, sizeof(p));
  if (n <= 0 || cin <= 0 || cout <= 0 || h < 3 || w < 8 || (stride != 1 && stride != 2)) return p;
  if (cout % 32 != 0 || (stride == 2 && (w % 2 != 0 || h % 2 != 0))) return p;
  const int kt = (int)((cin + 31) / 32), ct = (int)(cout / 32);
  if (!(kt == 1 || kt == 2 || kt == 4 || kt == 8)) return p;
  const int wo = (int)((w - 1) / stride + 1), ho = (int)((h - 1) / stride + 1);
  p.kt = kt;
  p.cw = ct % 2 == 0 ? 2 : 1;
  p.strips = (int)((w + 29) / 30);
  p.lz = (stride == 1 && p.strips == 1) ? (int)(30 - w) : 0;
  if (!(p.lz == 0 || p.lz == 2)) return p;
  p.ctg = ct / p.cw;
  p.threads = 64 * p.strips * p.ctg;
  if (p.threads > 512) return p;
  const int reach = stride == 1 ? (int)w + 2 + p.lz : 15 * p.strips + 1;
  p.pitch = (reach > wo ? reach : wo) + p.lz;
  p.pitch |= 1;
  p.lds = (size_t)ct * kt * 1024 + 2 * ((size_t)cout * p.pitch + kRowSlack) * 4 + kRowSlack * 4 + (stride == 1 ? (size_t)cout * 13 * 4 : 0);
  if (p.lds + 10 * 1024 > (size_t)max_lds_bytes()) return p;
  static const int rb_env = env_int("FQ_PWDW_RB", 0);
  {
    const int waves = p.threads / 64;
    int occ = (int)((160 * 1024) / (p.lds + 512));
    const int by_regs = 8 / waves > 0 ? 8 / waves : 1;
    occ = occ < by_regs ? occ : by_regs;
    occ = occ < 1 ? 1 : occ;
    const double slots = (double)num_cu() * occ;
    double best = 1e30;
    int best_rb = ho;
    for (int b = 1; b <= ho; ++b) {
      const int rb = (ho + b - 1) / b, bands = (ho + rb - 1) / rb;
      const double wgs = (double)n * bands, rounds = ceil(wgs / slots), fill = wgs < slots ? wgs / slots : 1.0;
      const double cost = rounds * (stride * rb + 2) / fill;
      if (cost < best - 1e-9) {
        best = cost;
        best_rb = rb;
      }
    }
    p.rb = rb_env > 0 ? (rb_env < ho ? rb_env : ho) : best_rb;
  }
  p.bands = (ho + p.rb - 1) / p.rb;
  if (n * cin * h * w * 4 >= (1ll << 32) || n * cout * ho * wo >= (1ll << 31)) return p;
  p.ok = true;
  return p;
}

}

namespace fqi {

bool pw_stat_shape_ok(int64_t n, int64_t cin, int64_t cout, int64_t hw) {
  if (n <= 0 || cin <= 0 || cout <= 0 || hw < 32 || hw >= (1ll << 30) || n * hw >= (1ll << 31) - 512) return false;
  const int kt = (int)((cin + 31) / 32), ct = (int)((cout + 31) / 32);
  if (!(kt == 1 || kt == 2 || kt == 4 || kt == 8) || cin % 16 != 0) return false;
  const size_t lds = (size_t)ct * kt * 1024 + 5 * (size_t)ct * 32 * 4 + 4 * (size_t)ct * 128 * 4;
  return lds <= 120 * 1024 && n * cin * hw * 4 < (1ll << 32);
}

int pw_stat_launch(const PwCall& c) {
  const int kt = (int)((c.cin + 31) / 32), ct = (int)((c.cout + 31) / 32);
  const size_t lds = (size_t)ct * kt * 1024 + 5 * (size_t)ct * 32 * 4 + 4 * (size_t)ct * 128 * 4;
  PwStatGeom g;
  g.Cin = (int)c.cin; g.KTS = (int)(c.cin_pad / 32); g.Cout = (int)c.cout; g.CT = ct; g.HW = (int)c.hw;
  g.cols = c.n * c.hw; g.tiles = (g.cols + 31) / 32; g.zoff = c.zoff;
  g.hw = fast_div_for((unsigned)c.hw);
  if (int rc = pw_zero_stat(c)) return rc;
  int per_cu = (int)((160 * 1024) / (lds + 1024));
  per_cu = per_cu > 3 ? 3 : per_cu;
  static const int wg_env = env_int("FQ_PWSTAT_WG_PER_CU", 0);
  if (wg_env > 0) per_cu = wg_env;
  int64_t grid = (int64_t)num_cu() * per_cu;
  const int64_t need = (g.tiles + 3) / 4;
  if (grid > need) grid = need;
  static const int table_env = env_int("FQ_PWSTAT_TABLE", -1);
  g.table = table_env >= 0 ? table_env : (g.tiles < grid * 4 * 10 ? 1 : 0);
#define FQ_PST_GO(KT_)                                                                                                     \
  case KT_: {                                                                                                              \
    static const bool attr_ok = hipFuncSetAttribute(reinterpret_cast<const void*>(&pw_stat_kernel<KT_>),                   \
                                                    hipFuncAttributeMaxDynamicSharedMemorySize, 120 * 1024) == hipSuccess; \
    FQ_REQUIRE(attr_ok, "fq_pwconv_i8_stat: cannot raise the dynamic LDS limit");                                          \
    hipLaunchKernelGGL((pw_stat_kernel<KT_>), dim3((unsigned)grid), dim3(kBlock), lds, c.st, c.x, c.wcodes, c.wscale,       \
                       (const int*)c.wsum, c.bias, g, c.in_stat, (int)c.n, c.in_thr, c.levels, c.lo_neg, kEps,              \
                       c.out_current_max, c.bn_scale, c.bn_shift, c.act, c.stat_out, (int8_t*)c.x_codes_out);              \
  } break;
  switch (kt) {
    FQ_PST_GO(1) FQ_PST_GO(2) FQ_PST_GO(4) FQ_PST_GO(8)
    default: return fail(FQ_ERR_INVALID, "fq_pwconv_i8_stat: K / 32 = %d is not instantiated", kt);
  }
#undef FQ_PST_GO
  FQ_LAUNCH_CHECK();
  return FQ_OK;
}

}

using namespace fqi;

extern "C" {

int fq_debug_fast_quotient(const float* c, int64_t n, const float* d, float* out, int* took_fast_path, fqStream_t stream) {
  FQ_REQUIRE(c && d && out && took_fast_path && n > 0, "fq_debug_fast_quotient: null pointer");
  hipLaunchKernelGGL(fast_quotient_kernel, dim3((unsigned)((n + 255) / 256)), dim3(256), 0, (hipStream_t)stream, c, n, d, out,
                     took_fast_path);
  FQ_LAUNCH_CHECK();
  return FQ_OK;
}

int fq_pwdw_fused_supported(int64_t n, int64_t cin, int64_t cout, int64_t h, int64_t w, int stride) {
  return pwdw_plan(n, cin, cout, h, w, stride).ok ? 1 : 0;
}

int fq_pwdw_fused(const float* x, const int8_t* wcodes, const float* wscale, const int32_t* wsum, const float* pw_bias,
                  int64_t n, int64_t cin, int64_t cin_pad, int64_t cout_pad, int64_t cout, int64_t h, int64_t w,
                  const float* in_stat, const float* in_thr, int in_width, unsigned in_flags, const float* pw_bn_scale,
                  const float* pw_bn_shift, int pw_act, const float* mid_stat, const float* mid_thr, int mid_width,
                  unsigned mid_flags, float* mid_current_max, const float* dw_w, const float* dw_bias, int dw_stride,
                  const float* dw_bn_scale, const float* dw_bn_shift, int dw_act, float* y, float* stat_out,
                  const void* x_codes, fqStream_t stream) {
  FQ_REQUIRE((x || x_codes) && wcodes && wscale && wsum && dw_w && y, "fq_pwdw_fused: null pointer");
  FQ_REQUIRE(in_stat != nullptr || in_thr != nullptr, "fq_pwdw_fused: give in_stat (online) or in_thr (offline)");
  FQ_REQUIRE(mid_stat != nullptr || mid_thr != nullptr, "fq_pwdw_fused: give mid_stat (the per-sample maxima of the pointwise "
             "output, from fq_pwconv_i8_stat) or mid_thr (a stored threshold)");
  FQ_REQUIRE(in_width >= 2 && in_width <= 8, "fq_pwdw_fused: input width %d does not fit int8 codes", in_width);
  FQ_REQUIRE(mid_width >= 2 && mid_width <= 16, "fq_pwdw_fused: bad width %d of the depthwise input", mid_width);
  FQ_REQUIRE(!((in_flags | mid_flags) & (FQ_ACT_NO_ABS | FQ_ACT_NO_EPS)), "fq_pwdw_fused: unsupported activation flags");
  FQ_REQUIRE((pw_bn_scale == nullptr) == (pw_bn_shift == nullptr) && (dw_bn_scale == nullptr) == (dw_bn_shift == nullptr),
             "fq_pwdw_fused: a BatchNorm's scale and shift go together");
  FQ_REQUIRE(cin_pad >= cin && cin_pad % 64 == 0 && cout_pad >= cout && cout_pad % 32 == 0,
             "fq_pwdw_fused: cin_pad / cout_pad must be those of fq_weight_codes");
  const bool prezeroed = (dw_act & FQ_STAT_PREZEROED) != 0;
  dw_act &= ~FQ_STAT_PREZEROED;
  FQ_REQUIRE(pw_act >= FQ_ACT_NONE && pw_act <= FQ_ACT_RELU6 && dw_act >= FQ_ACT_NONE && dw_act <= FQ_ACT_RELU6,
             "fq_pwdw_fused: unknown activation");
  FQ_REQUIRE(aligned16(wcodes) && (x_codes ? aligned16(x_codes) : aligned16(x)) && aligned16(y),
             "fq_pwdw_fused: x (x_codes when given), wcodes and y must be 16-byte aligned");
  const PwDwPlan p = pwdw_plan(n, cin, cout, h, w, dw_stride);
  FQ_REQUIRE(p.ok, "fq_pwdw_fused: shape not taken (n=%lld cin=%lld cout=%lld %lldx%lld stride %d): see fq_pwdw_fused_supported",
             (long long)n, (long long)cin, (long long)cout, (long long)h, (long long)w, dw_stride);
  hipStream_t st = (hipStream_t)stream;
  const int64_t ho = (h - 1) / dw_stride + 1, wo = (w - 1) / dw_stride + 1;
  if (stat_out && !prezeroed) FQ_HIP(hipMemsetAsync(stat_out, 0, n * sizeof(float), st));
// ... 63 lines not shown
```

### quantization/mxnet_amd/ops.py

```python
import ctypes
import threading

import numpy as np
import torch

from . import _lib
from ._lib import FakeQuantError

__all__ = ["comm_unique_id", "comm_init", "comm_world", "comm_allreduce", "comm_destroy", "add_act_stat", "bn_act_maxpool_stat", "stat_rows_sum", "mean_from_sums", "fake_quant_online_prestat", "bn_act_stat", "stem_conv3x3s2", "stem_conv_s2", "stem_conv_supported", "eval_counters", "dense_i8_eval", "gemm_i8_codes", "global_avg_pool_stat", "dwconv3x3", "dwconv3x3_c16", "weight_codes", "pwconv_i8", "pwconv_strided_supported", "weight_codes_3x3", "weight_slices_3x3", "conv3x3_i8", "Codes16", "batch_mean_rows", "batch_mean_gathered", "ste_forward", "absmax_per_sample", "batch_mean", "fake_quant_online", "fake_quant_offline", "weight_fake_quant",
           "wino_weight_fake_quant", "ema_update", "global_max", "histogram_accumulate", "hist_to_float",
           "kl_search", "quantize_codes", "dequantize", "qconv_kind", "qconv_weights", "qconv_workspace", "qconv2d",
           "batches_in_flight", "in_flight", "winograd_matrices", "device_info", "act_flags"]

_WS = {}


def _lib_():
    return _lib.LIB


_DEVICE_TLS = threading.local()


def _stream(t):
# ... 447 lines not shown
    if x.dim() != 4 or w.dim() != 4 or w.shape[2] != w.shape[3] or w.shape[2] not in (3, 7) or w.shape[1] != x.shape[1]:
        raise ValueError("stem_conv_s2 wants x (N,C,H,W) and w (Cout,C,K,K), K = 3 or 7; got %s and %s"
                         % (tuple(x.shape), tuple(w.shape)))
    for name, t in (("bias", bias), ("bn_scale", bn_scale), ("bn_shift", bn_shift), ("w_tap_major", w_tap_major)):
        if t is not None:
            _check(t, name)
    act = act or "none"
    if act not in _ACTS:
        raise ValueError("unknown activation %r" % (act,))
    n, cin, h, wd = x.shape
    cout, ks = w.shape[0], w.shape[2]
    pad = ks // 2
    wt = w_tap_major if w_tap_major is not None else w.permute(1, 2, 3, 0).contiguous()
    y = torch.empty((n, cout, (h + 2 * pad - ks) // 2 + 1, (wd + 2 * pad - ks) // 2 + 1), dtype=torch.float32,
                    device=x.device)
    stat, zflag = _stat_target(n, x.device, want_stat)
    if out_codes is not None:
        if ks != 3:
            raise ValueError("the first convolution hands codes over in its 3x3 form only")
        othr = _check(out_codes["thr"], "out_codes['thr']")
        yc = Codes16.empty(tuple(y.shape), x.device, othr, out_codes.get("width", 8), out_codes.get("flags", 0))
        check_call(_lib_().fq_stem_conv3x3s2_c16(_ptr(x), _ptr(wt), _ptr(bias), _ptr(yc.t), n, cin, cout, h, wd, _ptr(bn_scale),
                                                 _ptr(bn_shift), _ACTS[act] | zflag, _ptr(stat), _ptr(othr), int(yc.width),
                                                 int(yc.flags), _stream(x)))
        return yc, stat
    if pool:
        if ks != 7 or not stem_pool_supported(h, wd):
            raise ValueError("the pooled form is built for the 7x7 first convolution on planes whose output rows cut into four "
                             "tiles of at most 32 columns; got K = %d on %d x %d" % (ks, h, wd))
        ho, wo = y.shape[2], y.shape[3]
        yp = torch.empty((n, cout, (ho - 1) // 2 + 1, (wo - 1) // 2 + 1), dtype=torch.float32, device=x.device)
        check_call(_lib_().fq_stem_conv7x7s2_pool(_ptr(x), _ptr(wt), _ptr(bias), _ptr(yp), n, cin, cout, h, wd, _ptr(bn_scale),
                                                  _ptr(bn_shift), _ACTS[act] | zflag, _ptr(stat), _stream(x)))
        return yp, stat
    entry = _lib_().fq_stem_conv3x3s2 if ks == 3 else _lib_().fq_stem_conv7x7s2
    check_call(entry(_ptr(x), _ptr(wt), _ptr(bias), _ptr(y), n, cin, cout, h, wd, _ptr(bn_scale), _ptr(bn_shift),
                     _ACTS[act] | zflag, _ptr(stat), _stream(x)))
    return y, stat


stem_conv3x3s2 = stem_conv_s2


def stem_pool_supported(h, w):
    return bool(_lib_().fq_stem_conv7x7s2_pool_supported(int(h), int(w)))


def stem_conv_supported(cin, cout, kernel, stride, pad):
    k, s, p = tuple(kernel), tuple(stride), tuple(pad)
    return cin == 3 and s == (2, 2) and ((cout == 32 and k == (3, 3) and p == (1, 1)) or
                                         (cout == 64 and k == (7, 7) and p == (3, 3)))


def dwconv3x3(x, w, bias=None, stride=1, in_stat=None, in_thr=None, width=8, flags=0, cur_out=None, bn_scale=None,
              bn_shift=None, act=None, want_stat=True):
    _check(x, "x")
    _check(w, "w")
    if x.dim() != 4 or w.dim() != 4 or tuple(w.shape[1:]) != (1, 3, 3) or w.shape[0] != x.shape[1]:
        raise ValueError("dwconv3x3 wants x (N,C,H,W) and w (C,1,3,3); got %s and %s" % (tuple(x.shape), tuple(w.shape)))
    for name, t in (("bias", bias), ("in_stat", in_stat), ("in_thr", in_thr), ("bn_scale", bn_scale),
                    ("bn_shift", bn_shift), ("cur_out", cur_out)):
        if t is not None:
            _check(t, name)
    n, c, h, wd = x.shape
    ho, wo = (h - 1) // stride + 1, (wd - 1) // stride + 1
    y = torch.empty((n, c, ho, wo), dtype=torch.float32, device=x.device)
    stat, zflag = _stat_target(n, x.device, want_stat)
    check_call(_lib_().fq_dwconv3x3(_ptr(x), _ptr(w), _ptr(bias), _ptr(y), n, c, h, wd, int(stride), _ptr(in_stat),
                                    _ptr(in_thr), int(width), int(flags), _ptr(cur_out), _ptr(bn_scale),
                                    _ptr(bn_shift), _ACTS[act] | zflag, _ptr(stat), _stream(x)))
    return y, stat


def dwconv3x3_c16(x, w, bias=None, stride=1, in_stat=None, in_thr=None, width=8, flags=0, cur_out=None, bn_scale=None,
                  bn_shift=None, act=None, want_stat=True, out_codes=None):
    if not isinstance(x, Codes16) or in_thr is None or not x.matches(in_thr, width, flags):
        raise ValueError("dwconv3x3_c16 wants a Codes16 input quantised with this call's in_thr / width / signedness")
    if out_codes is None:
        raise ValueError("dwconv3x3_c16 writes codes: give out_codes")
    _check(x.t, "x", torch.int8)
    _check(w, "w")
    n, c, h, wd = x.shape
    if w.dim() != 4 or tuple(w.shape[1:]) != (1, 3, 3) or w.shape[0] != c:
        raise ValueError("dwconv3x3_c16 wants w (C,1,3,3); got %s for C = %d" % (tuple(w.shape), c))
    for name, t in (("bias", bias), ("in_stat", in_stat), ("in_thr", in_thr), ("bn_scale", bn_scale),
                    ("bn_shift", bn_shift), ("cur_out", cur_out)):
        if t is not None:
            _check(t, name)
    dev = x.t.device
    ho, wo = (h - 1) // stride + 1, (wd - 1) // stride + 1
    othr = _check(out_codes["thr"], "out_codes['thr']")
    y = Codes16.empty((n, c, ho, wo), dev, othr, out_codes.get("width", 8), out_codes.get("flags", 0))
    if in_stat is not None and cur_out is None:
        cur_out = torch.empty(1, dtype=torch.float32, device=dev)
    stat, zflag = _stat_target(n, dev, want_stat)
    check_call(_lib_().fq_dwconv3x3_c16(_ptr(x.t), _ptr(w), _ptr(bias), _ptr(y.t), n, c, h, wd, int(stride), _ptr(in_stat),
                                        _ptr(in_thr), int(width), int(flags), _ptr(cur_out), _ptr(bn_scale), _ptr(bn_shift),
                                        _ACTS[act] | zflag, _ptr(stat), _ptr(othr), y.width, y.flags, _stream(w)))
    return y, stat


def pwdw_supported(xshape, cout, stride):
    n, cin, h, w = (int(v) for v in xshape)
    lib = _lib_()
    return bool(lib.fq_pwconv_i8_stat_supported(n, cin, int(cout), h * w)) and \
        bool(lib.fq_pwdw_fused_supported(n, cin, int(cout), h, w, int(stride)))


def pair_codes_shape(xshape):
    n, cin, h, w = (int(v) for v in xshape)
    return (n, 2 * ((cin + 31) // 32), h * w, 16)


def _check_pair_codes(t, name, x):
    _check(t, name, torch.int8)
    if x.dim() != 4 or tuple(t.shape) != pair_codes_shape(x.shape):
        raise ValueError("%s must be int8 %s for x %s; got %s" % (name, pair_codes_shape(x.shape) if x.dim() == 4 else "(4-d x)",
                                                                  tuple(x.shape), tuple(t.shape)))
    if t.device != x.device:
        raise ValueError("%s lives on %s, x on %s" % (name, t.device, x.device))
    return t


def pwconv_i8_stat(x, wcodes, wscale, wsum, bias=None, in_stat=None, in_thr=None, width=8, flags=0, cur_out=None,
                   bn_scale=None, bn_shift=None, act=None, x_codes_out=None):
    _check(x, "x")
    _check(wcodes, "wcodes", torch.int8)
    _check(wscale, "wscale")
    _check(wsum, "wsum", torch.int32)
    for name, t in (("bias", bias), ("in_stat", in_stat), ("in_thr", in_thr), ("bn_scale", bn_scale),
                    ("bn_shift", bn_shift), ("cur_out", cur_out)):
        if t is not None:
            _check(t, name)
    n, cin = x.shape[0], x.shape[1]
    cout = wscale.numel()
    cin_pad = wcodes.shape[1]
    if (cin + 63) // 64 * 64 != cin_pad:
        raise ValueError("x has %d channels but the weight codes were made for a row length that pads to %d" % (cin, cin_pad))
    if in_stat is not None and cur_out is None:
        cur_out = torch.empty(1, dtype=torch.float32, device=x.device)
    if x_codes_out is not None:
        _check_pair_codes(x_codes_out, "x_codes_out", x)
    stat, zflag = _stat_target(n, x.device, True)
    hw = x.numel() // (n * cin)
    check_call(_lib_().fq_pwconv_i8_stat(_ptr(x), _ptr(wcodes), _ptr(wscale), _ptr(wsum), _ptr(bias), n, cin, cin_pad,
                                         wcodes.shape[0], cout, hw, _ptr(in_stat), _ptr(in_thr), int(width), int(flags), _ptr(cur_out),
                                         _ptr(bn_scale), _ptr(bn_shift), _ACTS[act] | zflag, _ptr(stat), _ptr(x_codes_out),
                                         _stream(x)))
    return stat


def pwdw_fused(x, wcodes, wscale, wsum, dw_w, pw_bias=None, in_stat=None, in_thr=None, width=8, flags=0, pw_bn_scale=None,
               pw_bn_shift=None, pw_act=None, mid_stat=None, mid_thr=None, mid_width=8, mid_flags=0, mid_cur_out=None,
               dw_bias=None, stride=1, dw_bn_scale=None, dw_bn_shift=None, dw_act=None, want_stat=True, x_codes=None):
    _check(x, "x")
    _check(wcodes, "wcodes", torch.int8)
    _check(wscale, "wscale")
    _check(wsum, "wsum", torch.int32)
    _check(dw_w, "dw_w")
    for name, t in (("pw_bias", pw_bias), ("in_stat", in_stat), ("in_thr", in_thr), ("pw_bn_scale", pw_bn_scale),
                    ("pw_bn_shift", pw_bn_shift), ("mid_stat", mid_stat), ("mid_thr", mid_thr), ("mid_cur_out", mid_cur_out),
                    ("dw_bias", dw_bias), ("dw_bn_scale", dw_bn_scale), ("dw_bn_shift", dw_bn_shift)):
        if t is not None:
            _check(t, name)
    if x.dim() != 4:
        raise ValueError("pwdw_fused wants x (N, Cin, H, W); got %s" % (tuple(x.shape),))
    n, cin, h, w = x.shape
    cout = wscale.numel()
    if dw_w.dim() != 4 or tuple(dw_w.shape) != (cout, 1, 3, 3):
        raise ValueError("pwdw_fused wants dw_w (%d,1,3,3); got %s" % (cout, tuple(dw_w.shape)))
    cout_pad, cin_pad = wcodes.shape
    if (cin + 63) // 64 * 64 != cin_pad:
        raise ValueError("x has %d channels but the weight codes were made for a row length that pads to %d" % (cin, cin_pad))
    if x_codes is not None:
        _check_pair_codes(x_codes, "x_codes", x)
    ho, wo = (h - 1) // stride + 1, (w - 1) // stride + 1
    y = torch.empty((n, cout, ho, wo), dtype=torch.float32, device=x.device)
    stat, zflag = _stat_target(n, x.device, want_stat)
    check_call(_lib_().fq_pwdw_fused(_ptr(x), _ptr(wcodes), _ptr(wscale), _ptr(wsum), _ptr(pw_bias), n, cin, cin_pad, cout_pad,
                                     cout, h, w, _ptr(in_stat), _ptr(in_thr), int(width), int(flags), _ptr(pw_bn_scale),
                                     _ptr(pw_bn_shift), _ACTS[pw_act], _ptr(mid_stat), _ptr(mid_thr), int(mid_width),
                                     int(mid_flags), _ptr(mid_cur_out), _ptr(dw_w), _ptr(dw_bias), int(stride),
                                     _ptr(dw_bn_scale), _ptr(dw_bn_shift), _ACTS[dw_act] | zflag, _ptr(y), _ptr(stat),
                                     _ptr(x_codes), _stream(x)))
    return y, stat


def weight_codes(w, rows_per_scale, width=8):
    _check(w, "w")
    rows = w.shape[0]
    row_len = w.numel() // rows
    row_pad = (row_len + 63) // 64 * 64
    rows_pad = (rows + 63) // 64 * 64
    buf = torch.empty(2 * rows_pad * row_pad, dtype=torch.int8, device=w.device)
    codes = buf[:rows_pad * row_pad].view(rows_pad, row_pad)
    scales = torch.empty(rows, dtype=torch.float32, device=w.device)
    rowsum = torch.empty(rows, dtype=torch.int32, device=w.device)
    ws = _workspace(w.device, _lib_().fq_weight_workspace_bytes(rows))
    check_call(_lib_().fq_weight_codes(_ptr(w), rows, row_len, int(rows_per_scale), int(width), row_pad, rows_pad,
                                       _ptr(codes), _ptr(scales), _ptr(rowsum), _ptr(ws), _stream(w)))
    return codes, scales, rowsum
# ... 618 lines not shown
```

### quantization/mxnet_amd/quantize/convert/convert_conv2d.py

```python
from collections import namedtuple

import os

import torch

from ...mx import nd
from ...mx import autograd
from ...mx.ndarray import NDArray
from ...mx.gluon.nn import Conv2D
from ... import ops
from .._state import DeviceScalar
from ._blocks import INPUT_RANGE, BatchNormTerms, contiguous, rebind_forward, scalar_slot

__all__ = ['gen_conv2d_converter']

QuantizedArgs = namedtuple("ConvQuantizedArgs",
                           "quantize_input in_signed in_width "
                           "wt_width quant_type "
                           "fake_bn wino_quantize")

WINOGRAD_VARIANTS = ("F23", "F43", "F63")


def current_slot(block, like):
    return scalar_slot(block, like)[0]


class _InputView(object):

    def __init__(self, block, x):
        self.t = contiguous(x._t)
        self.n = self.t.shape[0]
        self.cur, self.side = scalar_slot(block, self.t)
        rows = getattr(block, "_fq_stat_ws", None)
        if rows is not None and (rows.device != self.t.device or rows.numel() < self.n):
            rows = None
        self.rows = rows
        self.exchange = getattr(block, "_fq_global_stat", None)
        hint = x._fq_stat if x._t is self.t else None
        if hint is not None and (hint.numel() != self.n or hint.device != self.t.device):
            hint = None
        self.hint = hint

    def per_sample(self):
        if self.hint is None:
            return ops.absmax_per_sample(self.t, out=None if self.rows is None else self.rows[:self.n])
        if self.rows is not None:
            self.rows[:self.n].copy_(self.hint)
            return self.rows[:self.n]
        return self.hint

    def finish(self, block):
        if self.side:
            return
        block._fq_last_n = self.n
        block.current_input_max = DeviceScalar(self.cur)


def fake_quant_block_input(block, x, input_max, flags, width):
    v = _InputView(block, x)
    wanted = block.quantize_input
    offline = block.quantize_input_offline
    y = None
    if v.exchange is not None and v.rows is not None:
        v.exchange(v.per_sample(), v.n, v.cur)
        if wanted:
            y = ops.fake_quant_offline(v.t, input_max._t if offline else v.cur, width, flags, want_stat=False)[0]
    elif v.hint is not None or (v.rows is not None and getattr(block, "_fq_keep_rows", False)):
        stat = v.per_sample()
        if wanted and not offline:
            y = ops.fake_quant_online_prestat(v.t, stat, width, flags, cur_out=v.cur)[0]
        else:
            ops.batch_mean(stat, out=v.cur)
            if wanted:
                y = ops.fake_quant_offline(v.t, input_max._t, width, flags, want_stat=False)[0]
    elif not wanted:
        ops.batch_mean(v.per_sample(), out=v.cur)
    elif offline:
        y = ops.fake_quant_offline(v.t, input_max._t, width, flags, cur_out=v.cur, stat_ws=v.rows,
                                   want_stat=getattr(block, "track_input_stat", True))[0]
    else:
        y = ops.fake_quant_online(v.t, width, flags, cur_out=v.cur, stat_ws=v.rows)[0]
    v.finish(block)
    if y is None:
        return x
    return NDArray(autograd.ste_link(v.t, y))


def fused_input_plan(block, x, input_max, flags, width):
    v = _InputView(block, x)
    wanted = block.quantize_input
    online = wanted and not block.quantize_input_offline
    stat = None
    if online or v.exchange is not None or getattr(block, "track_input_stat", True):
        stat = v.per_sample()
    plan = {}
    if v.exchange is not None and v.rows is not None:
        v.exchange(stat, v.n, v.cur)
        if wanted:
            plan = dict(in_thr=input_max._t if block.quantize_input_offline else v.cur, width=width, flags=flags)
    elif online:
        plan = dict(in_stat=stat, width=width, flags=flags, cur_out=v.cur)
    elif wanted:
        plan = dict(in_thr=input_max._t, width=width, flags=flags)
        if stat is not None:
            plan.update(in_stat=stat, cur_out=v.cur)
    elif stat is not None:
        ops.batch_mean(stat, out=v.cur)
    v.finish(block)
    return plan


def depthwise_fused(block, x, weight_q, bias, plan):
    fz = block._fq_dw_fused
    scale, shift = fz["constants"]() if fz["bn"] is not None else (None, None)
    c16_in = getattr(x, "_fq_c16", None)
    if c16_in is not None:
        out_codes = handover_target(block, fz) if "in_thr" in plan else None
        if out_codes is not None:
            yc, stat = ops.dwconv3x3_c16(c16_in, contiguous(weight_q._t), None if bias is None else bias._t,
                                         stride=block._kwargs["stride"][0], bn_scale=scale, bn_shift=shift, act=fz["act"],
                                         out_codes=out_codes, **plan)
            out = NDArray(yc.t)
            out._fq_c16 = yc
            out._fq_stat = stat
            return out
        x = NDArray(codes16_to_fake_quant(c16_in))
        plan = {}
    y, stat = ops.dwconv3x3(contiguous(x._t), contiguous(weight_q._t), None if bias is None else bias._t,
                            stride=block._kwargs["stride"][0], bn_scale=scale, bn_shift=shift, act=fz["act"], **plan)
    out = NDArray(y)
    out._fq_stat = stat
    return out


def _weight_rows_per_scale(block, args):
    cout = block._kwargs["num_filter"]
    per_channel = args.quant_type == "channel" or (args.quant_type == "group" and block._kwargs["num_group"] == cout)
    return 1 if per_channel else cout


def _pointwise_weight_codes(block, args, weight_raw, weight_q):
    param_t = block.weight.data()._t
    key = (param_t.data_ptr(), param_t._version)
    held = getattr(block, "_fq_pw_cache", None)
    if block.fixed_params == 1 and held is not None and held[3] == key:
        return held[:3]
    three = block._fq_pw_fused.get("kind") == "3x3"
    if block._fq_pw_fused.get("sliced"):
        codes = ops.weight_slices_3x3(contiguous(weight_q._t))
        if block.fixed_params == 1:
            block._fq_pw_cache = tuple(codes) + (key,)
        return codes
    make = ops.weight_codes_3x3 if three else ops.weight_codes
    rederived = block.fixed_params == 1 and held is not None
    src = contiguous((weight_q if rederived else weight_raw)._t)
    live = None if rederived else block.__dict__.get("_fq_pw_live")
    if live is not None and live[0] is weight_raw._t and live[1] == weight_raw._t._version:
        codes = live[2]
    else:
        codes = make(src, _weight_rows_per_scale(block, args), args.wt_width)
        if not rederived and block.fixed_params != 1 and weight_raw._t is param_t:
            block.__dict__["_fq_pw_live"] = (weight_raw._t, weight_raw._t._version, codes)
    if block.fixed_params == 1:
        block.__dict__.pop("_fq_pw_live", None)
    if rederived:
        ref = src.permute(0, 2, 3, 1).contiguous() if three else src
        if not ops.weight_codes_reproduce(ref, codes[0], codes[1]):
            block._fq_no_int8 = True
            block.__dict__.pop("_fq_pw_cache", None)
            return None
    if block.fixed_params == 1:
        block._fq_pw_cache = tuple(codes) + (key,)
    return codes


_DW_C16_MIN_PIXELS = int(os.environ.get("FQ_DW_C16_MIN_PIXELS", "1"))


def _consumer_takes_codes(nxt):
    a = nxt.quantize_args
    return (nxt.enable_quantize and a.quantize_input and nxt.quantize_input and nxt.quantize_input_offline
            and a.in_width <= 8 and a.wt_width <= 8 and not getattr(nxt, "_fq_no_int8", False)
            and getattr(nxt, "input_max", None) is not None and getattr(nxt, "_fq_global_stat", None) is None)


# ... 109 lines not shown


def materialise_shortcut_record(d):
    return ops.pwconv_i8(d["x"], *d["codes"], None, bn_scale=d["bn"][0], bn_shift=d["bn"][1], act=None, want_stat=False,
                         **d["plan"])[0]


def materialise_shortcut(s):
    return NDArray(materialise_shortcut_record(s._fq_short))


def _convolve(block, F, x, weight, bias):
    if getattr(x, "_fq_sub2", None) is None:
        return block.origin_forward(F, x, weight, bias)
    out = F.Convolution(x, weight, bias, name="fwd", **dict(block._kwargs, stride=(1, 1)))
    return out if block.act is None else block.act(out)


_PLACEHOLDERS = {}


def _placeholder(shape, device):
    one = _PLACEHOLDERS.get(device)
    if one is None:
        one = _PLACEHOLDERS[device] = torch.zeros(1, dtype=torch.int8, device=device)
    return one.expand(*shape)


def recompute_target(block, fz, x, plan, c16_in):
    from .. import fuse as _fuse
    nxt = fz.get("pair_dw")
    if nxt is None or not _fuse.RECOMPUTE or c16_in is not None or autograd.is_recording() or _fuse._collection is not None:
        return None
    if getattr(ops.StatArena._tls, "current", None) is None:
        return None
    if "in_stat" not in plan or "in_thr" in plan or getattr(block, "_fq_residual", None) is not None:
        return None
    a = nxt.quantize_args
    if not (nxt.enable_quantize and a.quantize_input and nxt.quantize_input and not nxt.quantize_input_offline
            and getattr(nxt, "_fq_global_stat", None) is None and not a.fake_bn and nxt._kwargs["num_group"] == block._kwargs["num_filter"]):
        return None
    if any(_hooked(b) for b in (block, nxt, fz.get("bn"), fz.get("act_block"))):
        return None
    t = x._t
    if t.dim() != 4 or t.shape[2] * t.shape[3] < _fuse.RECOMPUTE_MIN_PIXELS or t.shape[1] > _fuse.RECOMPUTE_MAX_CIN:
        return None
    if not ops.pwdw_supported(tuple(t.shape), block._kwargs["num_filter"], nxt._kwargs["stride"][0]):
        return None
    return nxt


def _materialise(x):
    d = x._fq_deferred
    y, stat = ops.pwconv_i8(d["x"], *d["codes"], d["bias"], bn_scale=d["bn"][0], bn_shift=d["bn"][1], act=d["act"], **d["plan"])
    out = NDArray(y)
    out._fq_stat = stat
    return out


def depthwise_recompute(block, x, weight_q, bias, flags, width):
    d = x._fq_deferred
    fz = block._fq_dw_fused
    scale, shift = fz["constants"]() if fz["bn"] is not None else (None, None)
    src = d["x"]
    n = src.shape[0]
    cur, side = scalar_slot(block, src)
    stat = x._fq_stat
    rows = getattr(block, "_fq_stat_ws", None)
    if rows is not None and rows.device == src.device and rows.numel() >= n:
        rows[:n].copy_(stat)
    p = d["plan"]
    z, zstat = ops.pwdw_fused(src, *d["codes"], contiguous(weight_q._t), pw_bias=d["bias"], in_stat=p["in_stat"],
                              width=p["width"], flags=p["flags"], pw_bn_scale=d["bn"][0], pw_bn_shift=d["bn"][1],
                              pw_act=d["act"], mid_stat=stat, mid_width=width, mid_flags=flags, mid_cur_out=cur,
                              dw_bias=None if bias is None else bias._t, stride=block._kwargs["stride"][0],
                              dw_bn_scale=scale, dw_bn_shift=shift, dw_act=fz["act"], x_codes=d.get("x_codes"))
    if not side:
        block._fq_last_n = n
        block.current_input_max = DeviceScalar(cur)
    out = NDArray(z)
    out._fq_stat = zstat
    return out


def _handed_over(x):
    return getattr(x, "_fq_c16", None)


def codes16_to_fake_quant(c16):
    n, c, h, w = c16.shape
    signed = bool(c16.flags & 1)
    b = (c16.t.to(torch.int16) & 255) ^ 0x80
    codes = (b - 128).to(torch.int8).to(torch.float32) if signed else b.to(torch.float32)
    levels = float((1 << (c16.width - 1)) - 1) if signed else float((1 << c16.width) - 1)
    scale = c16.thr.reshape(()) / levels
    t = codes.reshape(n, -1, h * w, 16).permute(0, 1, 3, 2).reshape(n, -1, h, w)[:, :c]
    return (t * scale).contiguous()


def pointwise_fused(block, F, x, weight_raw, weight_q, bias, plan, weights_quantised):
    fz = block._fq_pw_fused
    args = block.quantize_args
    scale, shift = fz["constants"]() if fz["bn"] is not None else (None, None)
    on_codes = bool(plan) and weights_quantised and args.in_width <= 8 and args.wt_width <= 8 \
        and not getattr(block, "_fq_no_int8", False)
    held = _pointwise_weight_codes(block, args, weight_raw, weight_q) if on_codes else None
    on_codes = held is not None
    res0 = getattr(block, "_fq_residual", None)
    if res0 is not None and res0.get("short") is not None and not (on_codes and fz.get("kind") == "1x1"):
        res0["t"], res0["short"] = materialise_shortcut_record(res0["short"]), None
    c16_in = _handed_over(x)
    stride_ = 1 if getattr(x, "_fq_sub2", None) is not None else block._kwargs["stride"][0]
    if c16_in is None and on_codes and "in_thr" in plan:
        side = getattr(x, "_fq_side", None)
        if side is not None and not autograd.is_recording():
            if side[0] is block and side[1].matches(plan["in_thr"], plan["width"], plan["flags"]):
                c16_in = side[1]
            elif side[0] is not block and _same_quantiser(block, side[0], plan, side[1]):
                c16_in = ops.Codes16(side[1].t, side[1].shape, plan["in_thr"], plan["width"], plan["flags"])
    if c16_in is not None and not (on_codes and "in_thr" in plan):
        x = NDArray(codes16_to_fake_quant(c16_in))
        plan, c16_in = {}, None
    if on_codes:
        codes, scales, rowsum = held
        x_arg = c16_in if c16_in is not None else contiguous(x._t)
        if fz.get("kind") == "3x3":
            out_codes = None if fz.get("sliced") else handover_target(block)
            y, stat = ops.conv3x3_i8(x_arg, codes, scales, rowsum, None if bias is None else bias._t,
                                     bn_scale=scale, bn_shift=shift, act=fz["act"],
                                     **({} if fz.get("sliced") or out_codes is None else dict(out_codes=out_codes)), **plan)
        else:
            res = getattr(block, "_fq_residual", None)
            extra = {}
            xshape = c16_in.shape if c16_in is not None else tuple(x._t.shape)
            side_blk = sub_link = None
            if res is not None and res.get("short") is not None:
                d = res["short"]
                side_s = side_target(block, c16_in) if c16_in is not None else None
                d16 = isinstance(d["x"], ops.Codes16)
                if (block._kwargs["stride"][0] == 1 and scale is not None and not _hooked(block)
                        and (c16_in is None and not d16 or (side_s is not None and "in_thr" in plan))
                        and tuple(d["x"].shape[2:]) == tuple(xshape[2:]) and d["x"].shape[0] == xshape[0]
                        and ops.pwconv_shortcut_supported(xshape[1], d["x"].shape[1], block._kwargs["num_filter"])
                        and (c16_in is None or block._kwargs["num_filter"] % 512 == 0 or xshape[1] == 64)
                        and not autograd.is_recording()):
                    p2 = d["plan"]
                    kw2 = dict(x2=d["x"], wcodes2=d["codes"][0], wscale2=d["codes"][1], wsum2=d["codes"][2], in_stat2=p2.get("in_stat"),
                               in_thr2=p2.get("in_thr"), width2=p2["width"], flags2=p2["flags"], cur_out2=p2.get("cur_out"),
                               bn_scale2=d["bn"][0], bn_shift2=d["bn"][1])
                    if side_s is not None:
                        a_ = side_s.quantize_args
                        kw2["side_codes"] = dict(thr=side_s.input_max.data()._t, width=a_.in_width, flags=ops.act_flags(signed=a_.in_signed))
                    out = ops.pwconv_i8_shortcut(x_arg, codes, scales, rowsum, None if bias is None else bias._t, bn_scale=scale,
                                                 bn_shift=shift, act=res["act"], **kw2, **plan)
                    res["used"] = True
                    folded = NDArray(out[0])
                    folded._fq_stat = out[1]
                    if side_s is not None:
                        folded._fq_side = (side_s, out[2])
                    return folded
                res["t"] = materialise_shortcut_record(d)
                res["short"] = None
            if res is not None and block._kwargs["stride"][0] == 1 and tuple(res["t"].shape[2:]) == tuple(xshape[2:]) \
                    and res["t"].shape[1] == block._kwargs["num_filter"] and ops.pwconv_residual_supported(xshape[1]):
                extra = dict(residual=res["t"])
                res["used"] = True
                side_blk = side_target(block, c16_in)
                if side_blk is not None:
                    a_ = side_blk.quantize_args
                    extra["side_codes"] = dict(thr=side_blk.input_max.data()._t, width=a_.in_width,
                                               flags=ops.act_flags(signed=a_.in_signed))
                if side_blk is not None or c16_in is None:
                    sub_link = sub_target(block, fz, xshape)
                    if sub_link is not None:
                        extra["subsample"] = True
            if not extra and (c16_in is None or xshape[1] >= 256 or
                              (xshape[1] <= 32 and xshape[0] * xshape[2] * xshape[3] > 32 * 4096 and _THIN_FORMS)):
                xs = c16_in.shape if c16_in is not None else tuple(x._t.shape)
                s_ = stride_
                fz["c16_pays"] = len(xs) == 4 and ((xs[2] - 1) // s_ + 1) * ((xs[3] - 1) // s_ + 1) >= _DW_C16_MIN_PIXELS
                out_codes = handover_target(block)
                if out_codes is not None and fz.get("via") is not None:
                    co = block._kwargs["num_filter"]
                    if not (co >= 256 or (co <= 32 and xs[0] * ((xs[2] - 1) // s_ + 1) * ((xs[3] - 1) // s_ + 1) > 32 * 4096
                                          and _THIN_FORMS)):
                        out_codes = None
                if out_codes is not None:
                    extra = dict(out_codes=out_codes)
            if not extra or (set(extra) == {"residual"} and side_blk is None):
                gap = gap_target(block, fz, c16_in, xshape, "residual" in extra)
                if gap is not None:
                    y, stat = ops.pwconv_i8_gap(x_arg, codes, scales, rowsum, None if bias is None else bias._t, bn_scale=scale,
                                                bn_shift=shift, act=res["act"] if "residual" in extra else fz["act"],
                                                residual=extra.get("residual"), **plan)
                    pooled = NDArray(y)
                    pooled._fq_stat = stat
                    pooled._fq_pooled_by = gap
                    return pooled
            short = defer_shortcut(block, fz, x, x_arg, c16_in, (codes, scales, rowsum), bias, scale, shift, plan, stride_, extra)
            if short is not None:
                return short
            pair = recompute_target(block, fz, x, plan, c16_in) if not extra else None
            if pair is not None:
                b_ = None if bias is None else bias._t
                from .. import fuse as _fuse
                xcodes = torch.empty(ops.pair_codes_shape(x_arg.shape), dtype=torch.int8, device=x_arg.device) \
                    if _fuse.PAIR_CODES else None
                stat = ops.pwconv_i8_stat(x_arg, codes, scales, rowsum, b_, bn_scale=scale, bn_shift=shift, act=fz["act"],
                                          x_codes_out=xcodes, **plan)
                xs = tuple(x_arg.shape)
                res_ = NDArray(_placeholder((xs[0], block._kwargs["num_filter"], xs[2], xs[3]), x_arg.device))
                res_._fq_stat = stat
                res_._fq_deferred = dict(x=x_arg, codes=(codes, scales, rowsum), bias=b_, bn=(scale, shift), act=fz["act"],
                                         plan=dict(in_stat=plan["in_stat"], width=plan["width"], flags=plan["flags"],
                                                   cur_out=plan.get("cur_out")), consumer=pair, x_codes=xcodes)
                return res_
            out = ops.pwconv_i8(x_arg, codes, scales, rowsum, None if bias is None else bias._t,
                                bn_scale=scale, bn_shift=shift,
                                act=res["act"] if "residual" in extra else fz["act"],
                                stride=stride_, **extra, **plan)
            y, stat = out[0], out[1]
            if sub_link is not None and side_blk is None:
                trunk = NDArray(y)
                trunk._fq_stat = stat
                trunk._fq_sub2 = {"hw": tuple(xshape[2:]), "readers": sub_link["readers"], "unit": sub_link["unit"]}
                return trunk
            if side_blk is not None:
                trunk = NDArray(y)
                trunk._fq_stat = stat
                trunk._fq_side = (side_blk, out[2])
                if sub_link is not None:
                    trunk._fq_sub2 = {"hw": tuple(xshape[2:]), "readers": sub_link["readers"], "unit": sub_link["unit"]}
                return trunk
    else:
        if plan:
            t = contiguous(x._t)
            if "in_thr" not in plan:
                xq = ops.fake_quant_online_prestat(t, plan["in_stat"], plan["width"], plan["flags"],
                                                   cur_out=plan.get("cur_out"))[0]
            else:
                if "in_stat" in plan:
                    ops.batch_mean(plan["in_stat"], out=plan["cur_out"])
                xq = ops.fake_quant_offline(t, plan["in_thr"], plan["width"], plan["flags"], want_stat=False)[0]
            xq_ = NDArray(xq)
            xq_._fq_sub2 = x._fq_sub2
            x = xq_
        out = _convolve(block, F, x, weight_q, bias)
        from .. import fuse as _fuse
        res = getattr(block, "_fq_residual", None)
        if (res is not None and scale is not None and fz["act"] == "none" and res.get("owner") is not None and _fuse.BN_ADD
                and tuple(res["t"].shape) == tuple(out._t.shape) and out._t.is_cuda):
            owner = res["owner"]
            sink = _fuse._kl_sink(owner)
            y, stat = ops.bn_act_stat(contiguous(out._t), scale, shift, res["act"], hist=sink, residual=res["t"])
            res["used"] = True
            r_ = NDArray(y)
            r_._fq_stat = stat
            if _fuse._collection is not None:
                r_._fq_kl = (owner, sink)
            return r_
        if fz["bn"] is None and fz["act"] == "none":
            return out
        if scale is None:
            c = out.shape[1]
            scale = torch.ones(c, dtype=torch.float32, device=out._t.device)
            shift = torch.zeros(c, dtype=torch.float32, device=out._t.device)
        sink = _fuse._kl_sink(block)
        y, stat = ops.bn_act_stat(out._t.contiguous(), scale, shift, fz["act"], hist=sink)
# ... 11 lines not shown
    return res


def _fake_quant_weight(block, args, weight):
    keep = not args.fake_bn and not autograd.is_recording()
    if keep:
        held = block.__dict__.get("_fq_wq_cache")
        if held is not None and held[0] is weight._t and held[1] == weight._t._version:
            return held[2]
    out = _fake_quant_weight_now(block, args, weight)
    if keep:
        block.__dict__["_fq_wq_cache"] = (weight._t, weight._t._version, out)
    return out


def _fake_quant_weight_now(block, args, weight):
    w = contiguous(weight._t)
    if args.quant_type == 'channel' and args.wino_quantize != 'none' and block._kwargs['kernel'] == (3, 3):
        wq = ops.wino_weight_fake_quant(w, args.wino_quantize, args.wt_width)
        return NDArray(autograd.wino_link(w, wq, *ops.winograd_matrices(args.wino_quantize)))
    if args.quant_type == 'channel':
        rows = block._kwargs['num_filter']
    elif args.quant_type == 'group':
        rows = block._kwargs['num_group']
        if rows not in (1, w.shape[0]):
            raise ValueError("group-wise weight quantisation needs num_group in {1, num_filter} "
                             "(got num_group=%d, num_filter=%d): operands could not be broadcast" % (rows, w.shape[0]))
    else:
        rows = 1
    return NDArray(autograd.ste_link(w, ops.weight_fake_quant(w, rows, args.wt_width)))


def _quantised_conv(self, F, x, weight, bias=None, input_max=None,
                    gamma=None, beta=None, running_mean=None, running_var=None):
    args = self.quantize_args
    dw = getattr(self, "_fq_dw_fused", None)
    pw = getattr(self, "_fq_pw_fused", None)
    taken_over = dw is not None or pw is not None
    if taken_over and autograd.is_recording():
        raise RuntimeError("this net was rewired by quantize.fuse.fuse_inference (inference only): call "
                           "quantize.fuse.unfuse(net) before recording gradients")
    frozen = self.fixed_params == 1
    weight_raw, plan = weight, {}

    if args.fake_bn and not frozen:
        terms = BatchNormTerms(gamma, beta, running_mean, running_var)
        weight, bias = terms.fold_weight(F, weight), terms.fold_bias(F, bias)

    sub = getattr(x, "_fq_sub2", None)
    if sub is not None and not any(self is r for r in sub["readers"]):
        raise RuntimeError("a subsampled trunk (fq_pwconv_i8_sub2) reached a block that is not one of its two readers")

    deferred = getattr(x, "_fq_deferred", None)
    if deferred is not None and not (deferred["consumer"] is self and dw is not None and self.enable_quantize
                                     and args.quantize_input and self.quantize_input and not self.quantize_input_offline):
        x, deferred = _materialise(x), None

    weight_q = weight
    if self.enable_quantize:
        if args.quantize_input and deferred is not None:
            flags = ops.act_flags(signed=args.in_signed)
        elif args.quantize_input:
            flags = ops.act_flags(signed=args.in_signed)
            if taken_over:
                plan = fused_input_plan(self, x, input_max, flags, args.in_width)
            else:
                xq = fake_quant_block_input(self, x, input_max, flags, args.in_width)
                if sub is not None and xq is not x:
                    xq._fq_sub2 = sub
                x = xq
        if not frozen:
            weight_q = _fake_quant_weight(self, args, weight)

    if self.fixed_params == 0:
        self.fixed_params = 1
        self.weight.set_data(weight_q)
        if bias is not None:
            self.bias.set_data(bias)

    if deferred is not None:
        return depthwise_recompute(self, x, weight_q, bias, flags, args.in_width)
    if dw is not None:
        return depthwise_fused(self, x, weight_q, bias, plan)
    if pw is not None:
        return pointwise_fused(self, F, x, weight_raw, weight_q, bias, plan, bool(self.enable_quantize))
    return _convolve(self, F, x, weight_q, bias)


_FAKE_BN_PARAMS = (("gamma", "ones", True), ("beta", "zeros", True),
                   ("running_mean", "zeros", False), ("running_var", "ones", False))


def _attach_fake_bn(block):
    channels = block._kwargs['num_filter']
    for name, init, trainable in _FAKE_BN_PARAMS:
        setattr(block, name, block.params.get(name, shape=(channels,), init=init, differentiable=trainable,
                                              allow_deferred_init=True))

    @torch.no_grad()
    def record_batch_stats(blk, inputs):
        w = blk.weight.data()
        b = blk.bias.data() if blk.bias is not None else nd.zeros(shape=w.shape[0], ctx=w.context)
        y = nd.Convolution(inputs[0], w, b, **blk._kwargs)
        count = y.shape[0] * y.shape[2] * y.shape[3]
        blk.current_mean = y.sum(axis=(0, 2, 3)) / count
        centred = (y - blk.current_mean.reshape(1, -1, 1, 1)) ** 2
        blk.current_var = centred.sum(axis=(0, 2, 3)) / count
    block.register_forward_pre_hook(record_batch_stats)
# ... 25 lines not shown
```

### quantization/mxnet_amd/quantize/fuse.py

```python
import types

import torch

from ..mx.gluon import nn
from ..mx.ndarray import NDArray
from .. import ops

__all__ = ["fuse_inference", "unfuse", "refresh", "eval_head", "EvalHead"]


def _is_relu6_block(b):
    return type(b).__name__ == "RELU6"


def _act_kind(b):
    if isinstance(b, nn.Activation) and b._act_type == "relu" and not hasattr(b, "quantize_args") \
            and b.hybrid_forward.__func__ is nn.Activation.hybrid_forward:
        return "relu"
    if _is_relu6_block(b):
        return "relu6"
    return None


def _tensors_key(*tensors):
# ... 53 lines not shown
        sink = _kl_sink(self)
        y, stat = ops.bn_act_stat(t, st["scale"], st["shift"], st["act"], want_stat=True, hist=sink)
        out = NDArray(y)
        out._fq_stat = stat
        if _collection is not None:
            out._fq_kl = (self, sink)
        return out


def _pool_after_bn_forward(self, F, x):
    if getattr(x, "_fq_pooled_by", None) is self:
        x._fq_pooled_by = None
        return x
    return self._fq_pool_fused["orig"](F, x)


def _pool_stat_forward(self, F, x):
    if getattr(x, "_fq_pooled_by", None) is self:
        x._fq_pooled_by = None
        return x
    t = x._t if x._t.is_contiguous() else x._t.contiguous()
    if t.dim() != 4 or t.shape[3] % 4 or not t.is_cuda:
        return self._fq_pool_fused["orig"](F, x)
    st = self._fq_pool_fused
    c = t.shape[1]
    if st.get("ones") is None or st["ones"].numel() != c or st["ones"].device != t.device:
        st["ones"] = torch.ones(c, dtype=torch.float32, device=t.device)
        st["zeros"] = torch.zeros(c, dtype=torch.float32, device=t.device)
    y, stat = ops.bn_act_maxpool_stat(t, st["ones"], st["zeros"], "none", want_stat=True)
    out = NDArray(y)
    out._fq_stat = stat
    return out


def _is_maxpool_3x3s2p1(b):
    if type(b) is not nn.MaxPool2D or b.hybrid_forward.__func__ is not nn.MaxPool2D.hybrid_forward:
        return False
    k = b._kwargs
    return (k["kernel"] == (3, 3) and k["stride"] == (2, 2) and k["pad"] == (1, 1) and not k["global_pool"]
            and k["pooling_convention"] == "valid")


import os as _os

HANDOVER = _os.environ.get("FQ_HANDOVER", "1") != "0"
SIDE_CODES = _os.environ.get("FQ_HANDOVER_SIDE", "1") != "0"
STEM_CODES = _os.environ.get("FQ_HANDOVER_STEM", "1") != "0"
WINO_SLICED = _os.environ.get("FQ_WINO_SLICED", "1") != "0"
BN_ADD = _os.environ.get("FQ_BN_ADD", "1") != "0"
RECOMPUTE = _os.environ.get("FQ_RECOMPUTE", "1") != "0"
RECOMPUTE_MIN_PIXELS = int(_os.environ.get("FQ_RECOMPUTE_MIN_PIXELS", "3136"))
RECOMPUTE_MAX_CIN = int(_os.environ.get("FQ_RECOMPUTE_MAX_CIN", "128"))
PAIR_CODES = _os.environ.get("FQ_PWDW_CODES", "1") != "0"
SUBSAMPLE = _os.environ.get("FQ_SUBSAMPLE", "1") != "0"
GAP_FUSE = _os.environ.get("FQ_GAP_FUSE", "1") != "0"
SHORTCUT_FUSE = _os.environ.get("FQ_SHORTCUT_FUSE", "1") != "0"
UNIT_LINKS = _os.environ.get("FQ_HANDOVER_UNITS", "1") != "0"


def _identity_forward(self, F, x, *args, **kwargs):
    return x


def _is_dw3x3(b):
    if type(b) is not nn.Conv2D:
        return False
    k = b._kwargs
    cin = b.weight.shape[1] if b.weight.shape else 0
    return (k["kernel"] == (3, 3) and k["pad"] == (1, 1) and k["dilate"] == (1, 1) and k["stride"] in ((1, 1), (2, 2))
            and k["num_group"] == k["num_filter"] and cin == 1 and k["layout"] == "NCHW" and b.act is None
            and not getattr(getattr(b, "quantize_args", None), "fake_bn", False))


def _is_pw1x1(b):
    if type(b) is not nn.Conv2D or not hasattr(b, "quantize_args"):
        return False
    k = b._kwargs
    if not (k["kernel"] == (1, 1) and k["pad"] == (0, 0) and k["dilate"] == (1, 1) and k["num_group"] == 1
            and k["layout"] == "NCHW" and b.act is None and not b.quantize_args.fake_bn):
        return False
    if k["stride"] == (1, 1):
        return True
    cin = b.weight.shape[1] if b.weight.shape is not None and len(b.weight.shape) == 4 else 0
    return k["stride"] == (2, 2) and cin > 0 and ops.pwconv_strided_supported(cin)


def _is_dense3x3(b):
    if type(b) is not nn.Conv2D or not hasattr(b, "quantize_args"):
        return False
    k = b._kwargs
    a = b.quantize_args
    cin = b.weight.shape[1] if b.weight.shape is not None and len(b.weight.shape) == 4 else 0
    return (k["kernel"] == (3, 3) and k["pad"] == (1, 1) and k["dilate"] == (1, 1) and k["stride"] == (1, 1)
            and k["num_group"] == 1 and k["layout"] == "NCHW" and b.act is None and not a.fake_bn
            and cin in (64, 128, 256, 512) and k["num_filter"] >= 32
            and (not _wino_sliced(b) or (k["num_filter"] % 32 == 0 and WINO_SLICED)))


def _wino_sliced(b):
    a = b.quantize_args
    return a.quant_type == "channel" and a.wino_quantize != "none"


def _is_stem3x3s2(b):
    if type(b) is not nn.Conv2D or hasattr(b, "quantize_args"):
        return False
# ... 288 lines not shown
                    if fz is not None and fz.get("kind") == "1x1" and type(c) is nn.Conv2D and hasattr(c, "quantize_args") and \
                            k + 1 + (1 if fz["bn"] is not None else 0) + (1 if fz["act_block"] is not None else 0) == i:
                        fz["gap_next"] = {"gap": b, "via": ()}
                prev = own[i - 1] if i > 0 else None
                if type(prev) in (nn.Sequential, nn.HybridSequential) and "forward" not in prev.__dict__ and len(prev._children):
                    unit = list(prev._children.values())[-1]
                    if _is_residual_unit(unit):
                        tail = _tail_conv(unit.body)
                        if tail is not None and hasattr(tail, "quantize_args"):
                            tail._fq_pw_fused["gap_next"] = {"gap": b, "via": (unit, prev)}
            if flat is not None:
                flat.hybrid_forward = types.MethodType(_flatten_keep_stat_forward, flat)
            fused[0] += 1

    def visit_pw(container):
        if not isinstance(container, (nn.Sequential, nn.HybridSequential)):
            return
        kids = list(container._children.values())
        for i, b in enumerate(kids):
            dense3 = _is_dense3x3(b)
            if not (_is_pw1x1(b) or dense3) or hasattr(b, "_fq_pw_fused") or hasattr(b, "_fq_dw_fused"):
                continue
            bn = kids[i + 1] if i + 1 < len(kids) else None
            if not (type(bn) is nn.BatchNorm and not hasattr(bn, "_fq_fused") and bn._kwargs.get("axis", 1) == 1
                    and bn.hybrid_forward.__func__ is nn.BatchNorm.hybrid_forward):
                bn = None
            nxt = kids[i + 2] if bn is not None and i + 2 < len(kids) else (kids[i + 1] if bn is None and i + 1 < len(kids) else None)
            act = _act_kind(nxt) if nxt is not None else None
            b._fq_pw_fused = {"bn": bn, "act": act or "none", "act_block": nxt if act else None,
                              "constants": _bn_constants_getter(bn) if bn is not None else None,
                              "kind": "3x3" if dense3 else "1x1", "sliced": bool(dense3 and _wino_sliced(b))}
            if bn is not None:
                bn._fq_fused = {"taken_by_conv": True, "orig": bn.hybrid_forward, "act_block": None}
                bn.hybrid_forward = types.MethodType(_identity_forward, bn)
            if act:
                bypass(nxt)
            fused[0] += 1
        kids = list(container._children.values())

        def after(i, fz):
            j = i + 1 + (1 if fz["bn"] is not None else 0) + (1 if fz["act_block"] is not None else 0)
            return kids[j] if j < len(kids) else None

        for i, b in enumerate(kids):
            fz = getattr(b, "_fq_pw_fused", None) or getattr(b, "_fq_dw_fused", None)
            if fz is None or fz.get("sliced") or not hasattr(b, "quantize_args"):
                continue
            nxt = after(i, fz)
            if type(nxt) is not nn.Conv2D or not hasattr(nxt, "quantize_args"):
                continue
            if hasattr(b, "_fq_dw_fused"):
                if getattr(nxt, "_fq_pw_fused", None) is not None and nxt._fq_pw_fused.get("kind") == "1x1":
                    fz["next"] = nxt
            elif getattr(nxt, "_fq_pw_fused", None) is not None and not nxt._fq_pw_fused.get("sliced"):
                fz["next"] = nxt
            elif getattr(nxt, "_fq_dw_fused", None) is not None and fz.get("kind") == "1x1":
                fz["next"] = nxt
                if b._kwargs["stride"] == (1, 1) and b._kwargs["num_group"] == 1:
                    fz["pair_dw"] = nxt

    def visit(container):
        kids = list(container._children.values())
        for i, b in enumerate(kids):
            if type(b) is not nn.BatchNorm or hasattr(b, "_fq_fused") or b._kwargs.get("axis", 1) != 1:
                continue
            if b.hybrid_forward.__func__ is not nn.BatchNorm.hybrid_forward:
                continue
            nxt = kids[i + 1] if i + 1 < len(kids) and isinstance(container, (nn.Sequential, nn.HybridSequential)) \
                else None
            act = _act_kind(nxt) if nxt is not None else None
            if act and hasattr(nxt, "_fq_bypassed_orig"):
                act = None
            pool = kids[i + 2] if act and i + 2 < len(kids) and _is_maxpool_3x3s2p1(kids[i + 2]) \
                and not hasattr(kids[i + 2], "_fq_pool_fused") else None
            b._fq_fused = {"act": act or "none", "key": None, "scale": None, "shift": None,
                           "orig": b.hybrid_forward, "act_block": nxt if act else None, "pool": pool}
            b.hybrid_forward = types.MethodType(_fused_bn_forward, b)
            if act:
                bypass(nxt)
            if pool is not None:
                pool._fq_pool_fused = {"orig": pool.hybrid_forward}
                pool.hybrid_forward = types.MethodType(_pool_after_bn_forward, pool)
            fused[0] += 1

    after_features = {}
    feats, head = getattr(net, "features", None), getattr(net, "output", None)
    if isinstance(feats, (nn.Sequential, nn.HybridSequential)) and head is not None:
        after_features[id(feats)] = list(head._children.values()) \
            if isinstance(head, (nn.Sequential, nn.HybridSequential)) else [head]
    def visit_residual(b):
        if _is_residual_unit(b) and not hasattr(b, "_fq_residual_fused"):
            b._fq_residual_fused = True
            b.forward = types.MethodType(_residual_unit_forward, b)
            fused[0] += 1
        elif _is_linear_bottleneck(b) and b.use_shortcut and not hasattr(b, "_fq_residual_fused"):
            b._fq_residual_fused = True
            b.forward = types.MethodType(_linear_bottleneck_forward, b)
            fused[0] += 1

    def visit_side_links(container):
        if not isinstance(container, (nn.Sequential, nn.HybridSequential)):
            return
        kids = list(container._children.values())

        def unit(b, last):
            if getattr(b, "_fq_residual_fused", False) and hasattr(b, "body") and hasattr(b, "downsample"):
# ... 214 lines not shown
```

Before: 145,700.

## Defer stride-1 depthwise output and recompute it inside the following pointwise stat pass

A stride-1 depthwise conv that feeds a 1x1 pointwise conv now runs a statistics-only pass. That pass keeps the byte input codes and skips storing the float output. The pointwise stat kernel then recomputes the depthwise result from those codes as its front stage, so the full float dw activation is never written to or read back from memory. This adds a new kernel mode, extra Python deferral and materialisation logic, and repeated depthwise arithmetic. The payoff depends on PAIR_FRONT (default 1), which requires ops.in_flight() before the path activates.

After: 152,900 (median of 6 runs). 4.9% higher.

```diff
diff --git a/include/fakequant.h b/include/fakequant.h
--- a/include/fakequant.h
+++ b/include/fakequant.h
@@ -123,7 +123,7 @@
 int fq_dwconv3x3(const float* x, const float* w, const float* bias, float* y, int64_t n, int64_t c, int64_t h,
                  int64_t wdt, int stride, const float* in_stat, const float* in_thr, int in_width, unsigned in_flags,
                  float* out_current_max, const float* bn_scale, const float* bn_shift, int act, float* stat_out,
-                 fqStream_t stream);
+                 fqStream_t stream, void* x_codes_out);
 
 int fq_weight_codes(const float* w, int64_t rows, int64_t row_len, int rows_per_scale, int width, int64_t row_pad,
                     int64_t rows_pad, int8_t* codes, float* scales, int32_t* rowsum, void* ws, fqStream_t stream);
@@ -178,12 +178,14 @@
                      const float* in_thr, int in_width, unsigned in_flags, float* out_current_max, const float* bn_scale,
                      const float* bn_shift, int act, float* stat_out, const float* residual, void* ws, fqStream_t stream);
 
-int fq_pwconv_i8_stat_supported(int64_t n, int64_t cin, int64_t cout, int64_t hw);
+int fq_pwconv_i8_stat_supported(int64_t n, int64_t cin, int64_t cout, int64_t hw, int64_t front_h, int64_t front_wdt);
 int fq_pwconv_i8_stat(const float* x, const int8_t* wcodes, const float* wscale, const int32_t* wsum, const float* bias,
                       int64_t n, int64_t cin, int64_t cin_pad, int64_t cout_pad, int64_t cout, int64_t hw,
                       const float* in_stat, const float* in_thr, int in_width, unsigned in_flags, float* out_current_max,
                       const float* bn_scale, const float* bn_shift, int act, float* stat_out, void* x_codes_out,
-                      fqStream_t stream);
+                      fqStream_t stream, const void* front_codes, const float* front_w, const float* front_bias,
+                      const float* front_bn_scale, const float* front_bn_shift, int front_act, const float* front_in_stat,
+                      const float* front_in_thr, int front_width, unsigned front_flags, int64_t front_h, int64_t front_wdt);
 int fq_pwdw_fused_supported(int64_t n, int64_t cin, int64_t cout, int64_t h, int64_t w, int stride);
 int fq_debug_fast_quotient(const float* c, int64_t n, const float* d, float* out, int* took_fast_path, fqStream_t stream);
 int fq_pwdw_fused(const float* x, const int8_t* wcodes, const float* wscale, const int32_t* wsum, const float* pw_bias,
diff --git a/quantization/mxnet_amd/_lib.py b/quantization/mxnet_amd/_lib.py
--- a/quantization/mxnet_amd/_lib.py
+++ b/quantization/mxnet_amd/_lib.py
@@ -50,16 +50,16 @@
     "fq_stem_conv7x7s2_pool_supported": (_int, [_i64, _i64]),
     "fq_stem_conv3x3s2_c16": (_int, [_vp, _vp, _vp, _vp, _i64, _i64, _i64, _i64, _i64, _vp, _vp, _int, _vp, _vp, _int, _uint, _vp]),
     "fq_dwconv3x3": (_int, [_vp, _vp, _vp, _vp, _i64, _i64, _i64, _i64, _int, _vp, _vp, _int, _uint, _vp, _vp, _vp, _int,
-                            _vp, _vp]),
+                            _vp, _vp, _vp]),
     "fq_dwconv3x3_c16": (_int, [_vp, _vp, _vp, _vp, _i64, _i64, _i64, _i64, _int, _vp, _vp, _int, _uint, _vp, _vp, _vp, _int,
                                 _vp, _vp, _int, _uint, _vp]),
     "fq_weight_codes": (_int, [_vp, _i64, _i64, _int, _int, _i64, _i64, _vp, _vp, _vp, _vp, _vp]),
     "fq_pwconv_workspace_bytes": (ctypes.c_size_t, [_i64, _i64, _i64]),
     "fq_pwconv_i8": (_int, [_vp, _vp, _vp, _vp, _vp, _vp, _i64, _i64, _i64, _i64, _i64, _vp, _vp, _int, _uint, _vp, _vp,
                             _vp, _int, _vp, _vp, _vp]),
-    "fq_pwconv_i8_stat_supported": (_int, [_i64, _i64, _i64, _i64]),
+    "fq_pwconv_i8_stat_supported": (_int, [_i64, _i64, _i64, _i64, _i64, _i64]),
     "fq_pwconv_i8_stat": (_int, [_vp, _vp, _vp, _vp, _vp, _i64, _i64, _i64, _i64, _i64, _i64, _vp, _vp, _int, _uint, _vp, _vp,
-                                 _vp, _int, _vp, _vp, _vp]),
+                                 _vp, _int, _vp, _vp, _vp, _vp, _vp, _vp, _vp, _vp, _int, _vp, _vp, _int, _uint, _i64, _i64]),
     "fq_pwdw_fused_supported": (_int, [_i64, _i64, _i64, _i64, _i64, _int]),
     "fq_pwdw_fused": (_int, [_vp, _vp, _vp, _vp, _vp, _i64, _i64, _i64, _i64, _i64, _i64, _i64, _vp, _vp, _int, _uint, _vp,
                              _vp, _int, _vp, _vp, _int, _uint, _vp, _vp, _vp, _int, _vp, _vp, _int, _vp, _vp, _vp, _vp]),
diff --git a/quantization/mxnet_amd/csrc/fq_common.h b/quantization/mxnet_amd/csrc/fq_common.h
--- a/quantization/mxnet_amd/csrc/fq_common.h
+++ b/quantization/mxnet_amd/csrc/fq_common.h
@@ -568,6 +568,22 @@
 }
 __device__ __forceinline__ float lane_next(float v) {
   return __builtin_bit_cast(float, __builtin_amdgcn_update_dpp(0, __builtin_bit_cast(int, v), 0x130, 0xF, 0xF, false));
+}
+
+__device__ __forceinline__ float dw_taps(float w00, float w01, float w02, float w10, float w11, float w12, float w20,
+                                         float w21, float w22, float a0, float a1, float a2, float b0, float b1, float b2,
+                                         float c0, float c1, float c2) {
+  float acc = 0.0f;
+  acc = fmaf(w00, a0, acc);
+  acc = fmaf(w01, a1, acc);
+  acc = fmaf(w02, a2, acc);
+  acc = fmaf(w10, b0, acc);
+  acc = fmaf(w11, b1, acc);
+  acc = fmaf(w12, b2, acc);
+  acc = fmaf(w20, c0, acc);
+  acc = fmaf(w21, c1, acc);
+  acc = fmaf(w22, c2, acc);
+  return acc;
 }
 
 constexpr int kEpiRuntime = 0, kEpiBnRelu = 1, kEpiBnRelu6 = 2;
diff --git a/quantization/mxnet_amd/csrc/fq_dwconv.hip b/quantization/mxnet_amd/csrc/fq_dwconv.hip
--- a/quantization/mxnet_amd/csrc/fq_dwconv.hip
+++ b/quantization/mxnet_amd/csrc/fq_dwconv.hip
@@ -5,21 +5,6 @@
 typedef float f2 __attribute__((ext_vector_type(2)));
 __device__ __forceinline__ f2 splat2(float v) { return (f2){v, v}; }
 
-__device__ __forceinline__ float dw_taps(float w00, float w01, float w02, float w10, float w11, float w12, float w20,
-                                         float w21, float w22, float a0, float a1, float a2, float b0, float b1, float b2,
-                                         float c0, float c1, float c2) {
-  float acc = 0.0f;
-  acc = fmaf(w00, a0, acc);
-  acc = fmaf(w01, a1, acc);
-  acc = fmaf(w02, a2, acc);
-  acc = fmaf(w10, b0, acc);
-  acc = fmaf(w11, b1, acc);
-  acc = fmaf(w12, b2, acc);
-  acc = fmaf(w20, c0, acc);
-  acc = fmaf(w21, c1, acc);
-  acc = fmaf(w22, c2, acc);
-  return acc;
-}
 __device__ __forceinline__ f2 dw_taps2(float w00, float w01, float w02, float w10, float w11, float w12, float w20, float w21,
                                        float w22, f2 a0, f2 a1, f2 a2, f2 b0, f2 b1, f2 b2, f2 c0, f2 c1, f2 c2) {
   f2 acc = {0.f, 0.f};
@@ -831,13 +816,14 @@
   PW_STAMP(5);
 }
 
-template <int S, bool QUANT, bool ONLINE, bool NT, int EPI>
+template <int S, bool QUANT, bool ONLINE, bool NT, int EPI, bool NOSTORE = false>
 __global__ __launch_bounds__(kBlock) void dwconv3x3_cols4_kernel(
     const float* __restrict__ x, const float* __restrict__ wgt, const float* __restrict__ bias,
     float* __restrict__ y, DwColGeom g, int64_t total_segs, const float* __restrict__ in_stat, int n,
     const float* __restrict__ in_thr, float levels, int lo_neg_max, float eps, float* __restrict__ cur_max_out,
     const float* __restrict__ bn_scale, const float* __restrict__ bn_shift, int act, float* __restrict__ stat_out) {
   constexpr int D = (S == 1) ? 4 : 2;
+  static_assert(!NOSTORE || (S == 1 && QUANT), "the statistic pass exists for stride 1 with a quantised input");
   __shared__ unsigned k_stat[kStatSlots];
   if (threadIdx.x < kStatSlots) k_stat[threadIdx.x] = 0u;
   QParams q = {};
@@ -881,6 +867,16 @@
     };
     auto quant4 = [&](f4 v) -> f4 { return QUANT ? fq_code4(v, q) * q.scale : v; };
     auto finish = [&](float acc) -> float { return dw_finish<EPI>(acc, bias != nullptr, bch, has_bn, bsc, bsh, act); };
+    unsigned* const cp = reinterpret_cast<unsigned*>(y) + (plane * (int64_t)plane_in + (ld_ok ? ic0 : 0)) / 4;
+    auto quant4_keep = [&](f4 v, int row) -> f4 {
+      const f4 k = fq_code4(v, q);
+      if (y != nullptr && is_out && row <= last_row) {
+        const unsigned b0 = (unsigned)(int)k.x & 255u, b1 = (unsigned)(int)k.y & 255u, b2 = (unsigned)(int)k.z & 255u,
+                       b3 = (unsigned)(int)k.w & 255u;
+        cp[(int64_t)row * rowq] = b0 | (b1 << 8) | (b2 << 16) | (b3 << 24);
+      }
+      return k * q.scale;
+    };
 
     if (S == 1) {
       float a[6] = {0.f, 0.f, 0.f, 0.f, 0.f, 0.f}, b[6];
@@ -888,13 +884,13 @@
 #pragma unroll
       for (int k = 0; k < D; ++k) raw[k] = ldrow(1 + k);
       {
-        const f4 v = quant4(ldrow(0));
+        const f4 v = NOSTORE ? quant4_keep(ldrow(0), 0) : quant4(ldrow(0));
         b[0] = lane_prev(v.w);
         b[1] = v.x; b[2] = v.y; b[3] = v.z; b[4] = v.w;
         b[5] = lane_next(v.x);
       }
       auto emit = [&](int r, f4 craw) {
-        const f4 v = quant4(craw);
+        const f4 v = NOSTORE ? quant4_keep(craw, r + 1) : quant4(craw);
         float c[6];
         c[0] = lane_prev(v.w);
         c[1] = v.x; c[2] = v.y; c[3] = v.z; c[4] = v.w;
@@ -907,7 +903,7 @@
         }
         const float mm = fmaxf(fmaxf(fabsf(o[0]), fabsf(o[1])), fmaxf(fabsf(o[2]), fabsf(o[3])));
         m = fmaxf(m, keep(mm, is_out));
-        if (is_out) {
+        if (!NOSTORE && is_out) {
           if (g.nts) __builtin_nontemporal_store((f4){o[0], o[1], o[2], o[3]}, reinterpret_cast<f4*>(yp + (int64_t)r * g.Wo));
           else *reinterpret_cast<f4*>(yp + (int64_t)r * g.Wo) = (f4){o[0], o[1], o[2], o[3]};
         }
@@ -1005,15 +1001,19 @@
   float levels, eps;
   int lo_neg;
   int64_t ho, wo;
+  void* x_codes_out;
 };
 
 template <class KernelFor, class... Geom>
 int dw_launch(const DwCall& d, int grid, size_t lds, KernelFor kernel_for, Geom... geom) {
   using std::integral_constant;
   if (d.stat_out && !d.prezeroed) FQ_HIP(hipMemsetAsync(d.stat_out, 0, d.n * sizeof(float), d.st));
-  ProfScope prof(FQ_KERNEL_DWCONV, 4.0 * ((double)d.n * d.c * d.h * d.wdt + (double)d.n * d.c * d.ho * d.wo), d.st);
+  const double in_bytes = 4.0 * (double)d.n * d.c * d.h * d.wdt, out_bytes = 4.0 * (double)d.n * d.c * d.ho * d.wo;
+  ProfScope prof(FQ_KERNEL_DWCONV, in_bytes + out_bytes, d.st,
+                 d.y ? -1.0 : in_bytes + (d.x_codes_out ? 0.25 * in_bytes : 0.0));
+  float* const y_arg = d.y ? d.y : static_cast<float*>(d.x_codes_out);
   auto launch = [&](auto kernel) {
-    hipLaunchKernelGGL(kernel, dim3(grid), dim3(kBlock), lds, d.st, d.x, d.w, d.bias, d.y, geom..., d.in_stat, (int)d.n,
+    hipLaunchKernelGGL(kernel, dim3(grid), dim3(kBlock), lds, d.st, d.x, d.w, d.bias, y_arg, geom..., d.in_stat, (int)d.n,
                        d.in_thr, d.levels, d.lo_neg, d.eps, d.out_current_max, d.bn_scale, d.bn_shift, d.act, d.stat_out);
   };
   auto with_epi = [&](auto quant_c, auto online_c) {
@@ -1121,7 +1121,7 @@
   return dw_grid(dw_blocks(total_segs, cg.segs), dw_wg_per_cu);
 }
 bool dw_cols4_applies(const DwCall& d, int form) {
-  const bool can4 = (d.wdt % 4 == 0) && aligned16(d.x) && aligned16(d.y) && ((d.h * d.wdt) % 4 == 0) &&
+  const bool can4 = (d.wdt % 4 == 0) && aligned16(d.x) && aligned16(d.y) && aligned16(d.x_codes_out) && ((d.h * d.wdt) % 4 == 0) &&
                     (d.stride == 1 || ((d.wdt / 2) % 2 == 0));
   return (form == 3 || form == 0) && can4;
 }
@@ -1139,6 +1139,14 @@
       return dwconv3x3_cols4_kernel<decltype(s)::value, q(), o(), decltype(nt_c)::value, e()>;
     }, cg, total_segs);
   };
+  if (d.y == nullptr) {
+    auto go_stat = [&](auto nt_c) {
+      return dw_launch(d, grid, 0, [](auto, auto o, auto e) {
+        return dwconv3x3_cols4_kernel<1, true, o(), decltype(nt_c)::value, e(), true>;
+      }, cg, total_segs);
+    };
+    return nt ? go_stat(std::true_type{}) : go_stat(std::false_type{});
+  }
   if (d.stride == 1) return nt ? go(dw_int<1>{}, std::true_type{}) : go(dw_int<1>{}, std::false_type{});
   return nt ? go(dw_int<2>{}, std::true_type{}) : go(dw_int<2>{}, std::false_type{});
 }
@@ -1216,8 +1224,12 @@
 static int dwconv3x3_impl(const float* x, const float* w, const float* bias, float* y, int64_t n, int64_t c, int64_t h,
                           int64_t wdt, int stride, const float* in_stat, const float* in_thr, int in_width, unsigned in_flags,
                           float* out_current_max, const float* bn_scale, const float* bn_shift, int act, float* stat_out,
-                          fqStream_t stream) {
-  FQ_REQUIRE(x && w && y, "fq_dwconv3x3: null pointer");
+                          fqStream_t stream, void* x_codes_out = nullptr) {
+  FQ_REQUIRE(x && w && (y || stat_out), "fq_dwconv3x3: null pointer");
+  FQ_REQUIRE(y || !x_codes_out || (in_width <= 8 && !(in_flags & kFlagRangeRecord) &&
+                                   ((in_flags & FQ_ACT_SIGNED) || !(in_flags & FQ_ACT_LO_NEG_MAX))),
+             "fq_dwconv3x3: x_codes_out keeps codes that fit a byte (at most 8 bits; unsigned levels with a clip range from 0)");
+  FQ_REQUIRE(!(y && x_codes_out), "fq_dwconv3x3: x_codes_out belongs to the statistic pass (y == NULL)");
   FQ_REQUIRE(n > 0 && c > 0 && h > 0 && wdt > 0 && n * c < (1ll << 31) && h * wdt < (1ll << 28),
              "fq_dwconv3x3: bad shape (n=%lld c=%lld h=%lld w=%lld)", (long long)n, (long long)c, (long long)h,
              (long long)wdt);
@@ -1232,7 +1244,7 @@
   static const int epi_on = env_int("FQ_DW_EPI", 1);
 
   DwCall d = {};
-  d.x = x; d.w = w; d.bias = bias; d.y = y;
+  d.x = x; d.w = w; d.bias = bias; d.y = y; d.x_codes_out = x_codes_out;
   d.n = n, d.c = c, d.h = h, d.wdt = wdt, d.stride = stride;
   d.in_stat = in_stat, d.in_thr = in_thr, d.out_current_max = out_current_max;
   d.bn_scale = bn_scale, d.bn_shift = bn_shift, d.act = act, d.stat_out = stat_out;
@@ -1247,6 +1259,13 @@
   d.ho = (h - 1) / stride + 1, d.wo = (wdt - 1) / stride + 1;
 
   static const int form = env_int("FQ_DW_FORM", 0);
+  if (y == nullptr) {
+    FQ_REQUIRE(quant && stride == 1 && dw_cols4_applies(d, 3),
+               "fq_dwconv3x3: without y (statistic pass) only stride 1, a quantised input and rows of a multiple of 4 floats, "
+               "16-byte aligned, are taken (n=%lld c=%lld h=%lld w=%lld stride %d)", (long long)n, (long long)c, (long long)h,
+               (long long)wdt, stride);
+    return dw_run_cols4(d);
+  }
   if (dw_flat_applies(d, form)) return dw_run_flat(d);
   if (dw_planes_applies(d, form)) return dw_run_planes(d);
   if (dw_cols4_applies(d, form)) return dw_run_cols4(d);
@@ -1268,10 +1287,10 @@
 int fq_dwconv3x3(const float* x, const float* w, const float* bias, float* y, int64_t n, int64_t c, int64_t h,
                  int64_t wdt, int stride, const float* in_stat, const float* in_thr, int in_width, unsigned in_flags,
                  float* out_current_max, const float* bn_scale, const float* bn_shift, int act, float* stat_out,
-                 fqStream_t stream) {
+                 fqStream_t stream, void* x_codes_out) {
   FQ_REQUIRE(!(in_flags & ~(FQ_ACT_SIGNED | FQ_ACT_LO_NEG_MAX | FQ_ACT_NO_ABS | FQ_ACT_NO_EPS)), "fq_dwconv3x3: unknown flags");
   return dwconv3x3_impl(x, w, bias, y, n, c, h, wdt, stride, in_stat, in_thr, in_width, in_flags, out_current_max, bn_scale,
-                        bn_shift, act, stat_out, stream);
-}
-
-}
+                        bn_shift, act, stat_out, stream, x_codes_out);
+}
+
+}
diff --git a/quantization/mxnet_amd/csrc/fq_pw.h b/quantization/mxnet_amd/csrc/fq_pw.h
--- a/quantization/mxnet_amd/csrc/fq_pw.h
+++ b/quantization/mxnet_amd/csrc/fq_pw.h
@@ -4,6 +4,16 @@
 #include "fq_common.h"
 
 namespace fqi {
+
+struct PwFront {
+  const void* codes;
+  const float *w, *bias, *bn_scale, *bn_shift;
+  int act, epi;
+  const float *in_stat, *in_thr;
+  float levels;
+  bool is_signed;
+  int64_t h, wdt;
+};
 
 struct PwCall {
   const float* x;
@@ -41,9 +51,11 @@
   float* eval_counters = nullptr;
   void* eval_ws = nullptr;
   void* x_codes_out = nullptr;
+  const PwFront* front = nullptr;
 };
 
 bool pw_stat_shape_ok(int64_t n, int64_t cin, int64_t cout, int64_t hw);
+bool pw_stat_front_shape_ok(int64_t n, int64_t cin, int64_t cout, int64_t h, int64_t w);
 int pw_stat_launch(const PwCall& c);
 bool pw_short_shape_ok(int64_t cin, int64_t cin2, int64_t cout);
 int pw_short_launch(const PwCall& a, const PwCall& b);
diff --git a/quantization/mxnet_amd/csrc/fq_pwconv.hip b/quantization/mxnet_amd/csrc/fq_pwconv.hip
--- a/quantization/mxnet_amd/csrc/fq_pwconv.hip
+++ b/quantization/mxnet_amd/csrc/fq_pwconv.hip
@@ -217,7 +217,9 @@
                          in_width, in_flags, out_current_max, bn_scale, bn_shift, act, stat_out, nullptr, ws, stream);
 }
 
-int fq_pwconv_i8_stat_supported(int64_t n, int64_t cin, int64_t cout, int64_t hw) {
+int fq_pwconv_i8_stat_supported(int64_t n, int64_t cin, int64_t cout, int64_t hw, int64_t front_h, int64_t front_wdt) {
+  if (front_h != 0 || front_wdt != 0)
+    return (front_h > 0 && front_wdt > 0 && front_h * front_wdt == hw && pw_stat_front_shape_ok(n, cin, cout, front_h, front_wdt)) ? 1 : 0;
   return pw_stat_shape_ok(n, cin, cout, hw) ? 1 : 0;
 }
 
@@ -225,8 +227,10 @@
                       int64_t n, int64_t cin, int64_t cin_pad, int64_t cout_pad, int64_t cout, int64_t hw,
                       const float* in_stat, const float* in_thr, int in_width, unsigned in_flags, float* out_current_max,
                       const float* bn_scale, const float* bn_shift, int act, float* stat_out, void* x_codes_out,
-                      fqStream_t stream) {
-  FQ_REQUIRE(x && wcodes && wscale && wsum && stat_out, "fq_pwconv_i8_stat: null pointer");
+                      fqStream_t stream, const void* front_codes, const float* front_w, const float* front_bias,
+                      const float* front_bn_scale, const float* front_bn_shift, int front_act, const float* front_in_stat,
+                      const float* front_in_thr, int front_width, unsigned front_flags, int64_t front_h, int64_t front_wdt) {
+  FQ_REQUIRE((x || front_codes) && wcodes && wscale && wsum && stat_out, "fq_pwconv_i8_stat: null pointer");
   FQ_REQUIRE(pw_stat_shape_ok(n, cin, cout, hw), "fq_pwconv_i8_stat: shape not taken (n=%lld cin=%lld cout=%lld hw=%lld): see "
              "fq_pwconv_i8_stat_supported", (long long)n, (long long)cin, (long long)cout, (long long)hw);
   FQ_REQUIRE(cin_pad >= cin && cin_pad % 64 == 0 && cin_pad <= 8192 && cout_pad >= cout && cout_pad % 32 == 0,
@@ -239,8 +243,30 @@
   c.prezeroed = (act & FQ_STAT_PREZEROED) != 0;
   act &= ~FQ_STAT_PREZEROED;
   FQ_REQUIRE(act >= FQ_ACT_NONE && act <= FQ_ACT_RELU6, "fq_pwconv_i8_stat: unknown activation %d", act);
-  FQ_REQUIRE(aligned16(wcodes) && aligned16(x) && aligned16(x_codes_out),
+  FQ_REQUIRE(aligned16(wcodes) && (front_codes || aligned16(x)) && aligned16(x_codes_out),
              "fq_pwconv_i8_stat: x, wcodes and x_codes_out must be 16-byte aligned");
+  PwFront front = {};
+  if (front_codes != nullptr) {
+    FQ_REQUIRE(front_w && (front_in_stat || front_in_thr) && aligned16(front_codes), "fq_pwconv_i8_stat: the front layer needs "
+               "its weights, in_stat or in_thr, and 16-byte aligned codes");
+    FQ_REQUIRE(front_h * front_wdt == hw && pw_stat_front_shape_ok(n, cin, cout, front_h, front_wdt),
+               "fq_pwconv_i8_stat: front layer not taken (n=%lld cin=%lld cout=%lld %lldx%lld): see fq_pwconv_i8_stat_supported",
+               (long long)n, (long long)cin, (long long)cout, (long long)front_h, (long long)front_wdt);
+    FQ_REQUIRE(front_width >= 2 && front_width <= 8 && !(front_flags & ~(FQ_ACT_SIGNED | FQ_ACT_LO_NEG_MAX)) &&
+                   ((front_flags & FQ_ACT_SIGNED) || !(front_flags & FQ_ACT_LO_NEG_MAX)),
+               "fq_pwconv_i8_stat: the front layer's input codes are at most 8 bits wide, flags signed / lo_neg_max only");
+    FQ_REQUIRE((front_bn_scale == nullptr) == (front_bn_shift == nullptr) && front_act >= FQ_ACT_NONE && front_act <= FQ_ACT_RELU6,
+               "fq_pwconv_i8_stat: bad BatchNorm or activation of the front layer");
+    front.codes = front_codes; front.w = front_w; front.bias = front_bias; front.bn_scale = front_bn_scale;
+    front.bn_shift = front_bn_shift; front.act = front_act; front.in_stat = front_in_stat; front.in_thr = front_in_thr;
+    front.epi = (front_bn_scale != nullptr && front_bias == nullptr)
+                    ? (front_act == FQ_ACT_RELU ? kEpiBnRelu : front_act == FQ_ACT_RELU6 ? kEpiBnRelu6 : kEpiRuntime)
+                    : kEpiRuntime;
+    front.levels = act_levels(front_width, front_flags);
+    front.is_signed = (front_flags & FQ_ACT_SIGNED) != 0;
+    front.h = front_h; front.wdt = front_wdt;
+    c.front = &front;
+  }
   c.x = x; c.wcodes = wcodes + cout_pad * cin_pad; c.wscale = wscale; c.wsum = wsum; c.bias = bias; c.y = nullptr;
   c.n = n; c.cin = cin; c.cin_pad = cin_pad; c.cout = cout; c.hw = hw; c.stride = 1; c.h_in = c.w_in = c.w_out = 0;
   c.in_stat = in_stat; c.in_thr = in_thr;
@@ -252,7 +278,7 @@
   c.x_codes_out = x_codes_out;
   const double in_elems = (double)n * cin * hw, out_elems = (double)n * cout * hw;
   const double code_bytes = x_codes_out ? 32.0 * (double)((cin + 31) / 32) * n * hw : 0.0;
-  ProfScope prof(FQ_KERNEL_PWCONV, 4.0 * (in_elems + out_elems), c.st, 4.0 * in_elems + code_bytes);
+  ProfScope prof(FQ_KERNEL_PWCONV, 4.0 * (in_elems + out_elems), c.st, (front_codes ? 1.0 : 4.0) * in_elems + code_bytes);
   return pw_stat_launch(c);
 }
 
diff --git a/quantization/mxnet_amd/csrc/fq_pwdw.hip b/quantization/mxnet_amd/csrc/fq_pwdw.hip
--- a/quantization/mxnet_amd/csrc/fq_pwdw.hip
+++ b/quantization/mxnet_amd/csrc/fq_pwdw.hip
@@ -400,30 +400,48 @@
   FastDiv hw;
 };
 
-template <int KT>
+constexpr int kFrontRows = 8;
+struct PwFrontArgs {
+  const int8_t* codes;
+  const float *w, *bias, *bn_scale, *bn_shift;
+  const float *in_stat, *in_thr;
+  float levels;
+  int act;
+  int H, W, Q, segs, R, bands;
+};
+
+template <int KT, int FEPI = -1, bool FSIGNED = false>
 __global__ __launch_bounds__(kBlock, 3) void pw_stat_kernel(
     const float* __restrict__ x, const int8_t* __restrict__ wfrag, const float* __restrict__ wscale,
     const int* __restrict__ wsum, const float* __restrict__ bias, PwStatGeom g, const float* __restrict__ in_stat, int n,
     const float* __restrict__ in_thr, float levels, int lo_neg, float eps, float* __restrict__ cur_max_out,
     const float* __restrict__ bn_scale, const float* __restrict__ bn_shift, int act, float* __restrict__ stat_out,
-    int8_t* __restrict__ x_codes_out) {
+    int8_t* __restrict__ x_codes_out, PwFrontArgs fa) {
+  constexpr bool FRONT = FEPI >= 0;
+  static_assert(!FRONT || KT == 1, "the front layer is built for one 32-channel slab");
   extern __shared__ __attribute__((aligned(16))) unsigned char pst_smem[];
   v4i* ldsW = reinterpret_cast<v4i*>(pst_smem);
   int* c_zs = reinterpret_cast<int*>(pst_smem + (size_t)g.CT * KT * 1024);
   float* c_k = reinterpret_cast<float*>(c_zs + g.CT * 32);
   int* accs = reinterpret_cast<int*>(c_k + 4 * g.CT * 32);
+  float* dwk = reinterpret_cast<float*>(accs + 4 * g.CT * 128);
+  unsigned char* zbuf = reinterpret_cast<unsigned char*>(dwk + g.Cin * 12);
   const int lane = threadIdx.x & 63, wave = threadIdx.x >> 6;
   const int h = lane >> 5, i32 = lane & 31;
   const unsigned HW = (unsigned)g.HW, cols = (unsigned)g.cols;
   const int64_t nwaves = (int64_t)gridDim.x * 4, wid = (int64_t)blockIdx.x * 4 + wave;
-  const int64_t t_begin = g.tiles * wid / nwaves, t_end = g.tiles * (wid + 1) / nwaves;
+  const int64_t n_bands = FRONT ? (int64_t)(g.cols / g.HW) * fa.bands : 0;
+  const int64_t t_begin = FRONT ? n_bands * blockIdx.x / gridDim.x : g.tiles * wid / nwaves;
+  const int64_t t_end = FRONT ? n_bands * (blockIdx.x + 1) / gridDim.x : g.tiles * (wid + 1) / nwaves;
   const int pl = 16 * ((i32 >> 2) & 1) + 4 * (i32 >> 3) + (i32 & 3);
   int* my = accs + (size_t)wave * g.CT * 128;
   constexpr int kSlots = 8;
   __shared__ unsigned k_stat[kSlots];
   if (threadIdx.x < kSlots) k_stat[threadIdx.x] = 0u;
   unsigned s_base;
-  {
+  if constexpr (FRONT) {
+    s_base = (unsigned)((t_begin < n_bands ? t_begin : n_bands - 1) / fa.bands);
+  } else {
     const int64_t t0 = g.tiles * ((int64_t)blockIdx.x * 4) / nwaves;
     const unsigned j0 = (unsigned)(t0 < g.tiles ? t0 : g.tiles - 1) * 32u;
     s_base = fast_div(j0 < cols ? j0 : cols - 1, g.hw);
@@ -454,9 +472,13 @@
   for (int b2 = 0; b2 < NB; ++b2)
 #pragma unroll
     for (int i = 0; i < 16; ++i) raw[b2][i] = 0.0f;
-#pragma unroll
-  for (int qq = 0; qq < NB - 1; ++qq) issue(t_begin + qq / KT, qq % KT, raw[qq]);
+  if constexpr (!FRONT) {
+#pragma unroll
+    for (int qq = 0; qq < NB - 1; ++qq) issue(t_begin + qq / KT, qq % KT, raw[qq]);
+  }
   FQ_PIN();
+  float fscale = 0.0f;
+  if constexpr (FRONT) fscale = input_threshold(fa.in_stat, n, fa.in_thr, nullptr, false) / fa.levels;
   const float max_ = input_threshold(in_stat, n, in_thr, cur_max_out, blockIdx.x == 0);
   const QParams q = make_qparams(max_, levels, lo_neg != 0, eps);
   const int ubias = 128 - g.zoff;
@@ -476,6 +498,14 @@
     c_k[2 * nchs + i] = (okc && bn_scale != nullptr) ? bn_scale[i] : 1.0f;
     c_k[3 * nchs + i] = (okc && bn_scale != nullptr) ? bn_shift[i] : 0.0f;
   }
+  if constexpr (FRONT)
+    for (int i = threadIdx.x; i < g.Cin; i += kBlock) {
+#pragma unroll
+      for (int t = 0; t < 9; ++t) dwk[i * 12 + t] = fa.w[i * 9 + t];
+      dwk[i * 12 + 9] = fa.bias != nullptr ? fa.bias[i] : 0.0f;
+      dwk[i * 12 + 10] = fa.bn_scale != nullptr ? fa.bn_scale[i] : 1.0f;
+      dwk[i * 12 + 11] = fa.bn_scale != nullptr ? fa.bn_shift[i] : 0.0f;
+    }
   auto reset = [&]() __attribute__((always_inline)) {
     for (int ct = 0; ct < g.CT; ++ct) {
       my[ct * 128 + lane] = INT_MIN;
@@ -570,7 +600,7 @@
       atomicMin(&my[ct * 128 + 64 + lane], lo);
     }
   };
-  unsigned cur = fast_div((unsigned)((t_begin < g.tiles ? t_begin : g.tiles - 1) * 32), g.hw);
+  unsigned cur = FRONT ? s_base : fast_div((unsigned)((t_begin < g.tiles ? t_begin : g.tiles - 1) * 32), g.hw);
   auto run_tile = [&](int64_t t, auto ph_c, auto nn_c) __attribute__((always_inline)) {
     constexpr int PH = decltype(ph_c)::value;
     const Pix px = pix_of(t);
@@ -611,8 +641,106 @@
       if (U > 3 && t + 3 < t_end) run_tile(t + 3, integral_constant<int, 3 % U>{}, nn_c);
     }
   };
-  if (fq_nonneg(q) && fqx.ok) run_all(std::true_type{});
-  else run_all(std::false_type{});
+  auto run_front = [&](auto nn_c) __attribute__((always_inline)) {
+    constexpr bool NN = decltype(nn_c)::value;
+    constexpr int FE = FRONT ? FEPI : kEpiRuntime;
+    const int Q = fa.Q, W = fa.W, H = fa.H, NP = fa.R * fa.W;
+    const int seg = lane / Q, pos = lane - seg * Q;
+    const bool first = pos == 0, last = pos == Q - 1;
+    const bool has_fb = fa.bias != nullptr, has_fbn = fa.bn_scale != nullptr;
+    QParams qc = q;
+    if (NN && FE != kEpiRuntime) qc.hi = FE == kEpiBnRelu6 ? fminf(q.hi, 6.0f) : q.hi;
+    const unsigned* xc32 = reinterpret_cast<const unsigned*>(fa.codes);
+    const int z4 = stored_zero4(ubias);
+    const v4i zero_frag = (v4i){z4, z4, z4, z4};
+    auto deq = [&](unsigned wd, int b) __attribute__((always_inline)) {
+      const int code = FSIGNED ? (int)(int8_t)(wd >> (8 * b)) : (int)((wd >> (8 * b)) & 255u);
+      return (float)code * fscale;
+    };
+    for (int64_t bt = t_begin; bt < t_end; ++bt) {
+      const unsigned smp = (unsigned)(bt / fa.bands);
+      const int r0 = (int)(bt - (int64_t)smp * fa.bands) * fa.R;
+      const int Rb = H - r0 < fa.R ? H - r0 : fa.R;
+      if (smp != cur) {
+        flush(cur);
+        cur = smp;
+      }
+      for (int c0 = 0; c0 < g.Cin; c0 += 4 * fa.segs) {
+        const int c = c0 + wave * fa.segs + seg;
+        const bool c_ok = seg < fa.segs && c < g.Cin;
+        const int cc = c_ok ? c : 0;
+        const float* kc = dwk + cc * 12;
+        const float w00 = kc[0], w01 = kc[1], w02 = kc[2], w10 = kc[3], w11 = kc[4], w12 = kc[5], w20 = kc[6], w21 = kc[7],
+                    w22 = kc[8], bch = kc[9], bsc = kc[10], bsh = kc[11];
+        const unsigned* src = xc32 + ((int64_t)(smp * (unsigned)g.Cin + (unsigned)cc) * H) * Q + pos;
+        unsigned raw_c[kFrontRows + 2];
+#pragma unroll
+        for (int k = 0; k < kFrontRows + 2; ++k) {
+          const int t = r0 - 1 + k, tc = t < 0 ? 0 : (t > H - 1 ? H - 1 : t);
+          raw_c[k] = src[tc * Q] & ((t >= 0 && t < H) ? 0xFFFFFFFFu : 0u);
+        }
+        auto zcode = [&](float acc) __attribute__((always_inline)) {
+          if constexpr (NN) {
+            const float v = FE == kEpiRuntime ? dw_finish<kEpiRuntime>(acc, has_fb, bch, has_fbn, bsc, bsh, fa.act)
+                                              : dw_finish<FE, false>(acc, false, 0.0f, true, bsc, bsh, 0);
+            int r;
+            const float Qv = fast_quot(fq_clip(v, qc), fqx);
+            asm("v_cvt_rpi_i32_f32 %0, %1" : "=v"(r) : "v"(Qv));
+            return (unsigned)r ^ (nn_xor & 255u);
+          } else {
+            const float v = dw_finish<FE>(acc, has_fb, bch, has_fbn, bsc, bsh, fa.act);
+            return (unsigned)(fq_code_int(v, q) + ubias) ^ 0x80u;
+          }
+        };
+        float a[6] = {0.f, 0.f, 0.f, 0.f, 0.f, 0.f}, b[6] = {0.f, 0.f, 0.f, 0.f, 0.f, 0.f};
+#pragma unroll
+        for (int k = 0; k < kFrontRows + 2; ++k) {
+          if (k <= Rb + 1) {
+            float cv[6];
+#pragma unroll
+            for (int j = 0; j < 4; ++j) cv[j + 1] = deq(raw_c[k], j);
+            const float lp = lane_prev(cv[4]), ln = lane_next(cv[1]);
+            cv[0] = first ? 0.0f : lp;
+            cv[5] = last ? 0.0f : ln;
+            if (k >= 2) {
+              unsigned char* dst = zbuf + ((size_t)((cc >> 4) * NP + (k - 2) * W + 4 * pos) * 16 + (cc & 15));
+#pragma unroll
+              for (int j = 0; j < 4; ++j) {
+                const unsigned code = zcode(dw_taps(w00, w01, w02, w10, w11, w12, w20, w21, w22, a[j], a[j + 1], a[j + 2], b[j],
+                                                    b[j + 1], b[j + 2], cv[j], cv[j + 1], cv[j + 2]));
+                if (c_ok) dst[16 * j] = (unsigned char)code;
+              }
+            }
+#pragma unroll
+            for (int j = 0; j < 6; ++j) {
+              a[j] = b[j];
+              b[j] = cv[j];
+            }
+          }
+        }
+      }
+      __syncthreads();
+      const int npix = Rb * W, ntile = (npix + 31) >> 5;
+      for (int tl = wave; tl < ntile; tl += 4) {
+        int pp = tl * 32 + pl;
+        pp = pp < npix ? pp : npix - 1;
+        v4i f = *reinterpret_cast<const v4i*>(zbuf + ((size_t)(h * NP + pp) << 4));
+        if (g.Cin <= 16 && h == 1) f = zero_frag;
+        if (wr_codes) buf_st_v4i(rcodes, ((smp * 2u + (unsigned)h) * HW + (unsigned)(r0 * W + pp)) * 16u, f);
+        afrag[0] = f;
+        const int valid = npix - tl * 32;
+        reduce_tile(0, valid < 32 ? valid : 32);
+      }
+      __syncthreads();
+    }
+  };
+  if constexpr (FRONT) {
+    if (fq_nonneg(q) && fqx.ok) run_front(std::true_type{});
+    else run_front(std::false_type{});
+  } else {
+    if (fq_nonneg(q) && fqx.ok) run_all(std::true_type{});
+    else run_all(std::false_type{});
+  }
   if (t_begin < t_end) flush(cur);
   __syncthreads();
   if (threadIdx.x < kSlots && k_stat[threadIdx.x] != 0u && s_base + threadIdx.x < cols / HW)
@@ -694,20 +822,46 @@
   return lds <= 120 * 1024 && n * cin * hw * 4 < (1ll << 32);
 }
 
+static int pw_front_rows(int64_t h, int64_t w) {
+  int r = (int)(32768 / (32 * w));
+  r = r > kFrontRows ? kFrontRows : r;
+  r = r > h ? (int)h : r;
+  for (int k = r; k >= 1 && 2 * k > r; --k)
+    if ((k * w) % 32 == 0) return k;
+  return r;
+}
+
+bool pw_stat_front_shape_ok(int64_t n, int64_t cin, int64_t cout, int64_t h, int64_t w) {
+  if (h < 1 || w < 4 || w % 4 != 0 || w / 4 > 64 || !(cin == 16 || cin == 32) || !pw_stat_shape_ok(n, cin, cout, h * w)) return false;
+  return pw_front_rows(h, w) >= 1 && n * cin * ((w / 4 + 61) / 62) < (1ll << 31) - 1024;
+}
+
 int pw_stat_launch(const PwCall& c) {
   const int kt = (int)((c.cin + 31) / 32), ct = (int)((c.cout + 31) / 32);
-  const size_t lds = (size_t)ct * kt * 1024 + 5 * (size_t)ct * 32 * 4 + 4 * (size_t)ct * 128 * 4;
+  size_t lds = (size_t)ct * kt * 1024 + 5 * (size_t)ct * 32 * 4 + 4 * (size_t)ct * 128 * 4;
+  PwFrontArgs fa = {};
+  if (c.front != nullptr) {
+    const PwFront& f = *c.front;
+    fa.codes = static_cast<const int8_t*>(f.codes);
+    fa.w = f.w; fa.bias = f.bias; fa.bn_scale = f.bn_scale; fa.bn_shift = f.bn_shift;
+    fa.in_stat = f.in_stat; fa.in_thr = f.in_thr; fa.levels = f.levels; fa.act = f.act;
+    fa.H = (int)f.h; fa.W = (int)f.wdt; fa.Q = fa.W / 4; fa.segs = 64 / fa.Q;
+    fa.R = pw_front_rows(f.h, f.wdt);
+    fa.bands = (fa.H + fa.R - 1) / fa.R;
+    lds += (size_t)c.cin * 12 * 4 + (size_t)32 * fa.R * fa.W;
+  }
   PwStatGeom g;
   g.Cin = (int)c.cin; g.KTS = (int)(c.cin_pad / 32); g.Cout = (int)c.cout; g.CT = ct; g.HW = (int)c.hw;
   g.cols = c.n * c.hw; g.tiles = (g.cols + 31) / 32; g.zoff = c.zoff;
   g.hw = fast_div_for((unsigned)c.hw);
   if (int rc = pw_zero_stat(c)) return rc;
   int per_cu = (int)((160 * 1024) / (lds + 1024));
-  per_cu = per_cu > 3 ? 3 : per_cu;
+  const int wg_cap = c.front != nullptr ? 4 : 3;
+  per_cu = per_cu > wg_cap ? wg_cap : per_cu;
   static const int wg_env = env_int("FQ_PWSTAT_WG_PER_CU", 0);
   if (wg_env > 0) per_cu = wg_env;
   int64_t grid = (int64_t)num_cu() * per_cu;
-  const int64_t need = (g.tiles + 3) / 4;
+  const int64_t need = c.front != nullptr ? c.n * fa.bands : (g.tiles + 3) / 4;
   if (grid > need) grid = need;
   static const int table_env = env_int("FQ_PWSTAT_TABLE", -1);
   g.table = table_env >= 0 ? table_env : (g.tiles < grid * 4 * 10 ? 1 : 0);
@@ -718,12 +872,34 @@
     FQ_REQUIRE(attr_ok, "fq_pwconv_i8_stat: cannot raise the dynamic LDS limit");                                          \
     hipLaunchKernelGGL((pw_stat_kernel<KT_>), dim3((unsigned)grid), dim3(kBlock), lds, c.st, c.x, c.wcodes, c.wscale,       \
                        (const int*)c.wsum, c.bias, g, c.in_stat, (int)c.n, c.in_thr, c.levels, c.lo_neg, kEps,              \
-                       c.out_current_max, c.bn_scale, c.bn_shift, c.act, c.stat_out, (int8_t*)c.x_codes_out);              \
+                       c.out_current_max, c.bn_scale, c.bn_shift, c.act, c.stat_out, (int8_t*)c.x_codes_out, fa);          \
   } break;
-  switch (kt) {
-    FQ_PST_GO(1) FQ_PST_GO(2) FQ_PST_GO(4) FQ_PST_GO(8)
-    default: return fail(FQ_ERR_INVALID, "fq_pwconv_i8_stat: K / 32 = %d is not instantiated", kt);
-  }
+#define FQ_PST_FRONT(EPI_, SG_)                                                                                            \
+  {                                                                                                                        \
+    static const bool attr_ok = hipFuncSetAttribute(reinterpret_cast<const void*>(&pw_stat_kernel<1, EPI_, SG_>),          \
+                                                    hipFuncAttributeMaxDynamicSharedMemorySize, 120 * 1024) == hipSuccess; \
+    FQ_REQUIRE(attr_ok, "fq_pwconv_i8_stat: cannot raise the dynamic LDS limit");                                          \
+    hipLaunchKernelGGL((pw_stat_kernel<1, EPI_, SG_>), dim3((unsigned)grid), dim3(kBlock), lds, c.st, c.x, c.wcodes,       \
+                       c.wscale, (const int*)c.wsum, c.bias, g, c.in_stat, (int)c.n, c.in_thr, c.levels, c.lo_neg, kEps,   \
+                       c.out_current_max, c.bn_scale, c.bn_shift, c.act, c.stat_out, (int8_t*)c.x_codes_out, fa);          \
+  }
+#define FQ_PST_FRONT_S(EPI_)                                                                                               \
+  {                                                                                                                        \
+    if (c.front->is_signed) FQ_PST_FRONT(EPI_, true) else FQ_PST_FRONT(EPI_, false)                                        \
+  }
+  if (c.front != nullptr) {
+    FQ_REQUIRE(kt == 1, "fq_pwconv_i8_stat: a front layer needs cin <= 32");
+    if (c.front->epi == kEpiBnRelu) FQ_PST_FRONT_S(kEpiBnRelu)
+    else if (c.front->epi == kEpiBnRelu6) FQ_PST_FRONT_S(kEpiBnRelu6)
+    else FQ_PST_FRONT_S(kEpiRuntime)
+  } else {
+    switch (kt) {
+      FQ_PST_GO(1) FQ_PST_GO(2) FQ_PST_GO(4) FQ_PST_GO(8)
+      default: return fail(FQ_ERR_INVALID, "fq_pwconv_i8_stat: K / 32 = %d is not instantiated", kt);
+    }
+  }
+#undef FQ_PST_FRONT_S
+#undef FQ_PST_FRONT
 #undef FQ_PST_GO
   FQ_LAUNCH_CHECK();
   return FQ_OK;
diff --git a/quantization/mxnet_amd/ops.py b/quantization/mxnet_amd/ops.py
--- a/quantization/mxnet_amd/ops.py
+++ b/quantization/mxnet_amd/ops.py
@@ -523,8 +523,25 @@
                                          (cout == 64 and k == (7, 7) and p == (3, 3)))
 
 
+def front_codes_shape(xshape):
+    n, c, h, w = (int(v) for v in xshape)
+    return (n, c, h * w)
+
+
+def _check_front_codes(t, name, xshape, device):
+    _check(t, name, torch.int8)
+    if len(xshape) != 4 or tuple(t.shape) != front_codes_shape(xshape):
+        raise ValueError("%s must be int8 %s for a depthwise input %s; got %s"
+                         % (name, front_codes_shape(xshape) if len(xshape) == 4 else "(4-d x)", tuple(xshape), tuple(t.shape)))
+    if t.device != device:
+        raise ValueError("%s lives on %s, x on %s" % (name, t.device, device))
+    if t.data_ptr() % 16:
+        raise ValueError("%s must be 16-byte aligned" % name)
+    return t
+
+
 def dwconv3x3(x, w, bias=None, stride=1, in_stat=None, in_thr=None, width=8, flags=0, cur_out=None, bn_scale=None,
-              bn_shift=None, act=None, want_stat=True):
+              bn_shift=None, act=None, want_stat=True, store=True, x_codes_out=None):
     _check(x, "x")
     _check(w, "w")
     if x.dim() != 4 or w.dim() != 4 or tuple(w.shape[1:]) != (1, 3, 3) or w.shape[0] != x.shape[1]:
@@ -535,11 +552,17 @@
             _check(t, name)
     n, c, h, wd = x.shape
     ho, wo = (h - 1) // stride + 1, (wd - 1) // stride + 1
-    y = torch.empty((n, c, ho, wo), dtype=torch.float32, device=x.device)
+    if not store and not want_stat:
+        raise ValueError("dwconv3x3(store=False) leaves nothing but the statistic: want_stat must be set")
+    if x_codes_out is not None:
+        if store:
+            raise ValueError("dwconv3x3 keeps the codes of x only in its statistic pass (store=False)")
+        _check_front_codes(x_codes_out, "x_codes_out", tuple(x.shape), x.device)
+    y = torch.empty((n, c, ho, wo), dtype=torch.float32, device=x.device) if store else None
     stat, zflag = _stat_target(n, x.device, want_stat)
     check_call(_lib_().fq_dwconv3x3(_ptr(x), _ptr(w), _ptr(bias), _ptr(y), n, c, h, wd, int(stride), _ptr(in_stat),
                                     _ptr(in_thr), int(width), int(flags), _ptr(cur_out), _ptr(bn_scale),
-                                    _ptr(bn_shift), _ACTS[act] | zflag, _ptr(stat), _stream(x)))
+                                    _ptr(bn_shift), _ACTS[act] | zflag, _ptr(stat), _stream(x), _ptr(x_codes_out)))
     return y, stat
 
 
@@ -574,8 +597,13 @@
 def pwdw_supported(xshape, cout, stride):
     n, cin, h, w = (int(v) for v in xshape)
     lib = _lib_()
-    return bool(lib.fq_pwconv_i8_stat_supported(n, cin, int(cout), h * w)) and \
+    return bool(lib.fq_pwconv_i8_stat_supported(n, cin, int(cout), h * w, 0, 0)) and \
         bool(lib.fq_pwdw_fused_supported(n, cin, int(cout), h, w, int(stride)))
+
+
+def pwconv_front_supported(xshape, cout):
+    n, cin, h, w = (int(v) for v in xshape)
+    return bool(_lib_().fq_pwconv_i8_stat_supported(n, cin, int(cout), h * w, h, w))
 
 
 def pair_codes_shape(xshape):
@@ -594,7 +622,7 @@
 
 
 def pwconv_i8_stat(x, wcodes, wscale, wsum, bias=None, in_stat=None, in_thr=None, width=8, flags=0, cur_out=None,
-                   bn_scale=None, bn_shift=None, act=None, x_codes_out=None):
+                   bn_scale=None, bn_shift=None, act=None, x_codes_out=None, front=None):
     _check(x, "x")
     _check(wcodes, "wcodes", torch.int8)
     _check(wscale, "wscale")
@@ -612,12 +640,31 @@
         cur_out = torch.empty(1, dtype=torch.float32, device=x.device)
     if x_codes_out is not None:
         _check_pair_codes(x_codes_out, "x_codes_out", x)
+    f_args = (_ptr(None),) * 5 + (0, _ptr(None), _ptr(None), 0, 0, 0, 0)
+    if front is not None:
+        unknown = set(front) - {"x_codes", "w", "bias", "bn_scale", "bn_shift", "act", "in_stat", "in_thr", "width", "flags"}
+        if unknown or x.dim() != 4:
+            raise ValueError("pwconv_i8_stat(front=) wants x (N, Cin, H, W) and the keys of a depthwise call; got %s, %s"
+                             % (tuple(x.shape), sorted(unknown)))
+        fw = _check(front["w"], "front['w']")
+        if tuple(fw.shape) != (cin, 1, 3, 3):
+            raise ValueError("front['w'] must be (%d,1,3,3); got %s" % (cin, tuple(fw.shape)))
+        _check_front_codes(front["x_codes"], "front['x_codes']", tuple(x.shape), x.device)
+        for name in ("bias", "bn_scale", "bn_shift", "in_stat", "in_thr"):
+            if front.get(name) is not None:
+                _check(front[name], "front['%s']" % name)
+        if not pwconv_front_supported(x.shape, cout):
+            raise ValueError("pwconv_i8_stat(front=) does not take x %s -> %d channels: see pwconv_front_supported"
+                             % (tuple(x.shape), cout))
+        f_args = (_ptr(front["x_codes"]), _ptr(fw), _ptr(front.get("bias")), _ptr(front.get("bn_scale")),
+                  _ptr(front.get("bn_shift")), _ACTS[front.get("act")], _ptr(front.get("in_stat")), _ptr(front.get("in_thr")),
+                  int(front.get("width", 8)), int(front.get("flags", 0)), int(x.shape[2]), int(x.shape[3]))
     stat, zflag = _stat_target(n, x.device, True)
     hw = x.numel() // (n * cin)
     check_call(_lib_().fq_pwconv_i8_stat(_ptr(x), _ptr(wcodes), _ptr(wscale), _ptr(wsum), _ptr(bias), n, cin, cin_pad,
                                          wcodes.shape[0], cout, hw, _ptr(in_stat), _ptr(in_thr), int(width), int(flags), _ptr(cur_out),
                                          _ptr(bn_scale), _ptr(bn_shift), _ACTS[act] | zflag, _ptr(stat), _ptr(x_codes_out),
-                                         _stream(x)))
+                                         _stream(x), *f_args))
     return stat
 
 
diff --git a/quantization/mxnet_amd/quantize/convert/convert_conv2d.py b/quantization/mxnet_amd/quantize/convert/convert_conv2d.py
--- a/quantization/mxnet_amd/quantize/convert/convert_conv2d.py
+++ b/quantization/mxnet_amd/quantize/convert/convert_conv2d.py
@@ -29,7 +29,7 @@
 class _InputView(object):
 
     def __init__(self, block, x):
-        self.t = contiguous(x._t)
+        self.t = x._t if getattr(x, "_fq_deferred", None) is not None else contiguous(x._t)
         self.n = self.t.shape[0]
         self.cur, self.side = scalar_slot(block, self.t)
         rows = getattr(block, "_fq_stat_ws", None)
@@ -127,11 +127,46 @@
             return out
         x = NDArray(codes16_to_fake_quant(c16_in))
         plan = {}
-    y, stat = ops.dwconv3x3(contiguous(x._t), contiguous(weight_q._t), None if bias is None else bias._t,
-                            stride=block._kwargs["stride"][0], bn_scale=scale, bn_shift=shift, act=fz["act"], **plan)
+    call = dict(x=contiguous(x._t), w=contiguous(weight_q._t), bias=None if bias is None else bias._t,
+                stride=block._kwargs["stride"][0], bn_scale=scale, bn_shift=shift, act=fz["act"], **plan)
+    front = front_target(block, fz, x, plan) if c16_in is None else None
+    if front is not None:
+        xcodes = torch.empty(ops.front_codes_shape(call["x"].shape), dtype=torch.int8, device=call["x"].device)
+        stat = _dwconv3x3(call, store=False, x_codes_out=xcodes)[1]
+        out = NDArray(_placeholder(tuple(call["x"].shape), call["x"].device))
+        out._fq_stat = stat
+        out._fq_deferred = dict(kind="front", consumer=front, call=call, x_codes=xcodes)
+        return out
+    y, stat = _dwconv3x3(call)
     out = NDArray(y)
     out._fq_stat = stat
     return out
+
+
+def _dwconv3x3(call, **more):
+    kw = dict(call)
+    return ops.dwconv3x3(kw.pop("x"), **kw, **more)
+
+
+def front_target(block, fz, x, plan):
+    from .. import fuse as _fuse
+    nxt = fz.get("front_pw")
+    if nxt is None or not _fuse.PAIR_CODES or not (int(_fuse.PAIR_FRONT) >= 2 or (_fuse.PAIR_FRONT and ops.in_flight())) \
+            or block._kwargs["stride"] != (1, 1) \
+            or block.quantize_args.fake_bn or "in_stat" not in plan or "in_thr" in plan or plan["width"] > 8:
+        return None
+    pz, a = nxt._fq_pw_fused, nxt.quantize_args
+    if not (nxt.enable_quantize and a.quantize_input and nxt.quantize_input and not nxt.quantize_input_offline
+            and a.in_width <= 8 and a.wt_width <= 8 and not getattr(nxt, "_fq_no_int8", False) and not a.fake_bn
+            and getattr(nxt, "_fq_global_stat", None) is None and getattr(nxt, "_fq_residual", None) is None):
+        return None
+    if any(_hooked(b) for b in (block, fz.get("bn"), fz.get("act_block"))):
+        return None
+    if recompute_target(nxt, pz, x, dict(in_stat=None), None) is None or handover_target(nxt) is not None:
+        return None
+    if not ops.pwconv_front_supported(tuple(x._t.shape), nxt._kwargs["num_filter"]):
+        return None
+    return nxt
 
 
 def _weight_rows_per_scale(block, args):
@@ -347,7 +382,12 @@
 
 def _materialise(x):
     d = x._fq_deferred
-    y, stat = ops.pwconv_i8(d["x"], *d["codes"], d["bias"], bn_scale=d["bn"][0], bn_shift=d["bn"][1], act=d["act"], **d["plan"])
+    if d.get("kind") == "front":
+        y, stat = _dwconv3x3(d["call"])
+    else:
+        src = d["x"] if d.get("front") is None else _dwconv3x3(d["front"]["call"])[0]
+        y, stat = ops.pwconv_i8(src, *d["codes"], d["bias"], bn_scale=d["bn"][0], bn_shift=d["bn"][1], act=d["act"],
+                                **d["plan"])
     out = NDArray(y)
     out._fq_stat = stat
     return out
@@ -401,6 +441,12 @@
         and not getattr(block, "_fq_no_int8", False)
     held = _pointwise_weight_codes(block, args, weight_raw, weight_q) if on_codes else None
     on_codes = held is not None
+    front = getattr(x, "_fq_deferred", None)
+    if front is not None:
+        from .. import fuse as _fuse
+        if not (on_codes and fz.get("kind") == "1x1" and _fuse.PAIR_CODES and getattr(block, "_fq_residual", None) is None
+                and handover_target(block) is None and recompute_target(block, fz, x, plan, None) is not None):
+            x, front = _materialise(x), None
     res0 = getattr(block, "_fq_residual", None)
     if res0 is not None and res0.get("short") is not None and not (on_codes and fz.get("kind") == "1x1"):
         res0["t"], res0["short"] = materialise_shortcut_record(res0["short"]), None
@@ -418,7 +464,10 @@
         plan, c16_in = {}, None
     if on_codes:
         codes, scales, rowsum = held
-        x_arg = c16_in if c16_in is not None else contiguous(x._t)
+        if front is not None:
+            x_arg = torch.empty(tuple(x._t.shape), dtype=torch.float32, device=x._t.device)
+        else:
+            x_arg = c16_in if c16_in is not None else contiguous(x._t)
         if fz.get("kind") == "3x3":
             out_codes = None if fz.get("sliced") else handover_target(block)
             y, stat = ops.conv3x3_i8(x_arg, codes, scales, rowsum, None if bias is None else bias._t,
@@ -501,14 +550,20 @@
                 from .. import fuse as _fuse
                 xcodes = torch.empty(ops.pair_codes_shape(x_arg.shape), dtype=torch.int8, device=x_arg.device) \
                     if _fuse.PAIR_CODES else None
+                fkw = {}
+                if front is not None:
+                    c_ = front["call"]
+                    fkw = dict(front=dict(x_codes=front["x_codes"], w=c_["w"], bias=c_["bias"], bn_scale=c_["bn_scale"],
+                                          bn_shift=c_["bn_shift"], act=c_["act"], in_stat=c_["in_stat"], width=c_["width"],
+                                          flags=c_["flags"]))
                 stat = ops.pwconv_i8_stat(x_arg, codes, scales, rowsum, b_, bn_scale=scale, bn_shift=shift, act=fz["act"],
-                                          x_codes_out=xcodes, **plan)
+                                          x_codes_out=xcodes, **fkw, **plan)
                 xs = tuple(x_arg.shape)
                 res_ = NDArray(_placeholder((xs[0], block._kwargs["num_filter"], xs[2], xs[3]), x_arg.device))
                 res_._fq_stat = stat
                 res_._fq_deferred = dict(x=x_arg, codes=(codes, scales, rowsum), bias=b_, bn=(scale, shift), act=fz["act"],
                                          plan=dict(in_stat=plan["in_stat"], width=plan["width"], flags=plan["flags"],
-                                                   cur_out=plan.get("cur_out")), consumer=pair, x_codes=xcodes)
+                                                   cur_out=plan.get("cur_out")), consumer=pair, x_codes=xcodes, front=front)
                 return res_
             out = ops.pwconv_i8(x_arg, codes, scales, rowsum, None if bias is None else bias._t,
                                 bn_scale=scale, bn_shift=shift,
@@ -626,8 +681,12 @@
         raise RuntimeError("a subsampled trunk (fq_pwconv_i8_sub2) reached a block that is not one of its two readers")
 
     deferred = getattr(x, "_fq_deferred", None)
-    if deferred is not None and not (deferred["consumer"] is self and dw is not None and self.enable_quantize
-                                     and args.quantize_input and self.quantize_input and not self.quantize_input_offline):
+    online = self.enable_quantize and args.quantize_input and self.quantize_input and not self.quantize_input_offline
+    if deferred is not None and deferred.get("kind") == "front":
+        if not (deferred["consumer"] is self and pw is not None and online and getattr(self, "_fq_global_stat", None) is None):
+            x = _materialise(x)
+        deferred = None
+    if deferred is not None and not (deferred["consumer"] is self and dw is not None and online):
         x, deferred = _materialise(x), None
 
     weight_q = weight
diff --git a/quantization/mxnet_amd/quantize/fuse.py b/quantization/mxnet_amd/quantize/fuse.py
--- a/quantization/mxnet_amd/quantize/fuse.py
+++ b/quantization/mxnet_amd/quantize/fuse.py
@@ -129,6 +129,7 @@
 RECOMPUTE_MIN_PIXELS = int(_os.environ.get("FQ_RECOMPUTE_MIN_PIXELS", "3136"))
 RECOMPUTE_MAX_CIN = int(_os.environ.get("FQ_RECOMPUTE_MAX_CIN", "128"))
 PAIR_CODES = _os.environ.get("FQ_PWDW_CODES", "1") != "0"
+PAIR_FRONT = int(_os.environ.get("FQ_PWDW_FRONT", "1"))
 SUBSAMPLE = _os.environ.get("FQ_SUBSAMPLE", "1") != "0"
 GAP_FUSE = _os.environ.get("FQ_GAP_FUSE", "1") != "0"
 SHORTCUT_FUSE = _os.environ.get("FQ_SHORTCUT_FUSE", "1") != "0"
@@ -523,6 +524,9 @@
             if hasattr(b, "_fq_dw_fused"):
                 if getattr(nxt, "_fq_pw_fused", None) is not None and nxt._fq_pw_fused.get("kind") == "1x1":
                     fz["next"] = nxt
+                    if b._kwargs["stride"] == (1, 1):
+                        fz["front_pw"] = nxt
+                        nxt._fq_pw_fused["front_dw"] = b
             elif getattr(nxt, "_fq_pw_fused", None) is not None and not nxt._fq_pw_fused.get("sliced"):
                 fz["next"] = nxt
             elif getattr(nxt, "_fq_dw_fused", None) is not None and fz.get("kind") == "1x1":
```
